# alvinliu0/HumanGaussian

Hardware: AMD Instinct MI355X
Metric: rasterize fwd+bwd Gaussians/sec @1024^2, 100k pts (higher is better)
Workload: dtype f32

## Files before the change

### humangaussian_amd/csrc/api.hip

```cpp
#include "hgs_common.h"
#include <stdio.h>
#include <stdlib.h>
#include <string.h>
#include <algorithm>
#include <atomic>
#include <mutex>

#ifdef HGS_TIMELINE
__device__ unsigned long long hgs_tl[HGS_TL_KERNELS][HGS_TL_SLOTS][4];
#endif
#include "preprocess.hip"
#include "binning.hip"
#include "render_fwd.hip"
#include "knn.hip"
#include "mesh.hip"
#include "fields.hip"
#include "bookkeeping.hip"
#include "optim.hip"
#include "lbs.hip"
#include "pose.hip"
#include "step_images.hip"

extern "C" __global__ void hgs_k_render_bwd(View, Layout, const hgs_status*, const SortRec*, const float*,
                                            const float*, const float*, const float*, const float*,
                                            const float*, const float*, float*, uint32_t);
extern "C" __global__ void hgs_k_pair_reduce_em(View, Layout, const hgs_status*, const SortRec*, const float*, float*, uint32_t, uint32_t);
extern "C" __global__ void hgs_k_pair_reduce_ch(View, Layout, const hgs_status*, const SortRec*, const float*, float*, uint32_t, uint32_t);

namespace {

#ifdef HGS_KNOBS
inline int hgs_knob(const char* name, int dflt) { const char* e = getenv(name); return (e && atoi(e) > 0) ? atoi(e) : dflt; }
#else
inline int hgs_knob(const char*, int dflt) { return dflt; }
#endif

#define HGS_CHUNK_ROWS_MIN_VIEWS 3
#ifndef HGS_PRE_BWD_VPAR_MIN_VIEWS
#define HGS_PRE_BWD_VPAR_MIN_VIEWS 2
#endif
constexpr size_t ALIGN = 256;
struct Carver {
  size_t off = 0;
  size_t take(size_t bytes) { const size_t o = off; off = hgs_align_up(off + bytes, ALIGN); return o; }
};
struct ScanShape { unsigned blocks; size_t bsum_bytes; };
inline ScanShape scan_shape(size_t n, size_t elem) {
  const size_t nb = (n + HGS_SCAN_BLOCK - 1) / HGS_SCAN_BLOCK;
  return {(unsigned)nb, (nb + 1) * elem};
}
constexpr size_t HGS_LDS_BINS_MAX = 16384;
#define HGS_BIN_WGS_PER_VIEW_MAX 512
#define HGS_BIN_WGS_TOTAL_MAX 1024
constexpr int HGS_MAX_BIN_WGS_PER_VIEW = HGS_BIN_WGS_PER_VIEW_MAX;
constexpr int HGS_BIN_WGS_TOTAL = HGS_BIN_WGS_TOTAL_MAX;

struct GeomCarve {
  size_t geom, tile_n, tile_start, tile_order, tile_rec, cell_info, items_part, fwd_cells,
      hist, tile_gbase, tile_count, chunk_sums, chunk_base, ctr, status, total;
};

inline int grid_dim(int pixels) { return (pixels + HGS_TILE - 1) / HGS_TILE; }

inline void bin_shape(int B, int P, int& nblk, int& cpw, int& nwg) {
  nblk = (P + HGS_BLOCK - 1) / HGS_BLOCK;
  int want = HGS_BIN_WGS_TOTAL / (B > 0 ? B : 1);
  if (want > HGS_MAX_BIN_WGS_PER_VIEW) want = HGS_MAX_BIN_WGS_PER_VIEW;
  if (want < 1) want = 1;
  cpw = (nblk + want - 1) / want;
  if (cpw < 1) cpw = 1;
  nwg = (nblk + cpw - 1) / cpw;
}

GeomCarve carve_geom(int B, int P, int H, int W) {
  const size_t T = (size_t)grid_dim(W) * grid_dim(H);
  const size_t TT = T * (size_t)B;
  int nblk, cpw, nwg;
  bin_shape(B, P, nblk, cpw, nwg);
  const bool lds = T <= HGS_LDS_BINS_MAX;
  GeomCarve c;
  Carver cv;
  c.geom = cv.take((size_t)B * P * sizeof(GeomRec));
  c.tile_n = cv.take(TT * 4);
  c.tile_start = cv.take(TT * 4);
  c.tile_order = cv.take(TT * 4);
  c.tile_rec = cv.take(TT * 16);
  c.cell_info = cv.take(TT * 16 * sizeof(CellInfo));
  const size_t dcap = hgs_die_cells((int)TT);
  c.items_part = cv.take(HGS_NXCD * 2 * dcap * sizeof(uint4));
  c.fwd_cells = cv.take((size_t)HGS_NXCD * HGS_NFC * dcap * 4);
  c.hist = cv.take(lds ? (size_t)B * nwg * T * 4 : 0);
  c.tile_gbase = cv.take(lds ? (size_t)HGS_ROW_GROUPS * TT * 4 : 0);
  c.tile_count = cv.take(lds ? 0 : TT * 4);
  c.chunk_sums = cv.take((size_t)B * nblk * 4);
  c.chunk_base = cv.take((size_t)B * nblk * 4);
  c.ctr = cv.take(sizeof(Counters));
  c.status = cv.take(sizeof(hgs_status));
  c.total = cv.off;
  return c;
}

struct BinCarve { size_t keys, recs, cell_list, entpair, cstate, items_full, total; };

BinCarve carve_bin(int64_t cap) {
  BinCarve c;
  Carver cv;
  const size_t C = (size_t)(cap > 0 ? cap : 0);
  const size_t NP = C * HGS_PAIRS_PER_ENTRY;
  c.keys = cv.take(C * 8);
  c.recs = cv.take(C * sizeof(SortRec));
  c.cell_list = cv.take(NP * 8);
  c.entpair = cv.take(C * 8);
  c.cstate = cv.take((NP / HGS_SEGLEN + 1) * HGS_CSTATE_FLOATS * sizeof(float));
  c.items_full = cv.take(HGS_NXCD * (NP / HGS_SEGLEN + 1) * sizeof(uint4));
  c.total = cv.off;
  return c;
}

Layout make_layout(void* geom, void* bin, void* img, int B, int P, int H, int W, int64_t cap) {
  const GeomCarve g = carve_geom(B, P, H, W);
  const BinCarve b = carve_bin(cap);
  char* gp = static_cast<char*>(geom);
  char* bp = static_cast<char*>(bin);
  Layout L;
  L.geom = reinterpret_cast<GeomRec*>(gp + g.geom);
  L.tile_n = reinterpret_cast<uint32_t*>(gp + g.tile_n);
  L.tile_start = reinterpret_cast<uint32_t*>(gp + g.tile_start);
  L.tile_order = reinterpret_cast<uint32_t*>(gp + g.tile_order);
  L.tile_rec = reinterpret_cast<uint4*>(gp + g.tile_rec);
  L.cell_info = reinterpret_cast<CellInfo*>(gp + g.cell_info);
  L.items_part = reinterpret_cast<uint4*>(gp + g.items_part);
  L.fwd_cells = reinterpret_cast<uint32_t*>(gp + g.fwd_cells);
  L.hist = reinterpret_cast<uint32_t*>(gp + g.hist);
  L.tile_gbase = reinterpret_cast<uint32_t*>(gp + g.tile_gbase);
  L.tile_count = reinterpret_cast<uint32_t*>(gp + g.tile_count);
  L.chunk_sums = reinterpret_cast<uint32_t*>(gp + g.chunk_sums);
  L.chunk_base = reinterpret_cast<uint32_t*>(gp + g.chunk_base);
  L.ctr = reinterpret_cast<Counters*>(gp + g.ctr);
  L.keys = bp ? reinterpret_cast<unsigned long long*>(bp + b.keys) : nullptr;
  L.recs = bp ? reinterpret_cast<SortRec*>(bp + b.recs) : nullptr;
  L.cell_list = bp ? reinterpret_cast<uint2*>(bp + b.cell_list) : nullptr;
  L.entpair = bp ? reinterpret_cast<uint2*>(bp + b.entpair) : nullptr;
  L.cstate = bp ? reinterpret_cast<float*>(bp + b.cstate) : nullptr;
  L.items_full = bp ? reinterpret_cast<uint4*>(bp + b.items_full) : nullptr;
  L.full_cap = (uint32_t)((size_t)(cap > 0 ? cap : 0) * HGS_PAIRS_PER_ENTRY / HGS_SEGLEN + 1);
  L.n_contrib = static_cast<uint32_t*>(img);
  return L;
}

View make_view(const hgs_settings* s, int B, int P, int M, int64_t cap, int max_tile_hint = 0, int act = 0) {
  View v;
  v.act = act;
  v.pairchunks = B >= HGS_CHUNK_ROWS_MIN_VIEWS ? 1 : 0;
  for (int b = 0; b < HGS_MAX_VIEWS; ++b) {
    const hgs_settings& sb = s[b < B ? b : 0];
    Cam& c = v.cam[b];
    c.viewmatrix = sb.viewmatrix;
    c.projmatrix = sb.projmatrix;
    c.campos = sb.campos;
    c.bg = sb.bg;
    c.tanfovx = sb.tanfovx;
    c.tanfovy = sb.tanfovy;
    c.focal_x = (float)sb.image_width / (2.0f * sb.tanfovx);
    c.focal_y = (float)sb.image_height / (2.0f * sb.tanfovy);
  }
  v.scale_modifier = s->scale_modifier;
  v.W = s->image_width;
  v.H = s->image_height;
  v.grid_x = grid_dim(v.W);
  v.grid_y = grid_dim(v.H);
  v.T = v.grid_x * v.grid_y;
  v.B = B;
  v.TT = B * v.T;
  v.P = P;
  v.M = M;
  v.D = s->sh_degree;
  v.lds_bins = (size_t)v.T <= HGS_LDS_BINS_MAX ? 1 : 0;
  bin_shape(B, P, v.nblk, v.cpw, v.nwg);
  if (!v.lds_bins) { v.cpw = 1; v.nwg = v.nblk; }
  v.entry_capacity = (uint32_t)(cap < 0 ? 0 : (cap > 0xffffffffll ? 0xffffffffll : cap));
  v.max_tile_hint = max_tile_hint;
  return v;
}

inline int hip_rc(hipError_t e) { return e == hipSuccess ? HGS_OK : -(1000 + (int)e); }

inline hipError_t box_init(void* hdr, size_t hdr_bytes, uint32_t* bmin, hipStream_t stream) {
  const hipError_t e = hipMemsetAsync(hdr, 0, hdr_bytes, stream);
  return e != hipSuccess ? e : hipMemsetAsync(bmin, 0xff, 3 * sizeof(uint32_t), stream);
}

#define HGS_LAUNCH_CHECK()                       \
  do {                                           \
    hipError_t e__ = hipGetLastError();          \
    if (e__ != hipSuccess) return hip_rc(e__);   \
  } while (0)

#define HGS_STAGE(k)                                                              \
  do {                                                                            \
    if (stage_events && stage_events[k]) {                                        \
      hipError_t e__ = hipEventRecord(static_cast<hipEvent_t>(stage_events[k]), stream); \
      if (e__ != hipSuccess) return hip_rc(e__);                                  \
    }                                                                             \
  } while (0)

struct SideStream {
  std::mutex mu;
  hipStream_t s = nullptr;
  hipEvent_t fork = nullptr, join = nullptr;
  bool tried = false, ok = false;
};

struct DeviceState {
  std::atomic<int> cus;
  SideStream side;
  std::atomic<int> lds_raised[HGS_PRE_BWD_ROWS];
};
DeviceState g_devices[64];
DeviceState* device_state(hipStream_t stream) {
  int dev = 0;
  if (hipStreamGetDevice(stream, &dev) != hipSuccess || dev < 0 || dev >= 64) { (void)hipGetLastError(); return nullptr; }
  return &g_devices[dev];
}
struct DeviceCurrent {
  int dev, cur = 0;
  bool ok, switched;
  explicit DeviceCurrent(const DeviceState* ds)
      : dev((int)(ds - g_devices)), ok(hipGetDevice(&cur) == hipSuccess), switched(ok && cur != dev) {
    if (switched) ok = hipSetDevice(dev) == hipSuccess;
  }
  ~DeviceCurrent() { if (switched) (void)hipSetDevice(cur); }
};

int cu_count(DeviceState* ds) {
  if (!ds) return 256;
  int cus = ds->cus.load(std::memory_order_relaxed);
  if (cus > 0) return cus;
  if (hipDeviceGetAttribute(&cus, hipDeviceAttributeMultiprocessorCount, (int)(ds - g_devices)) != hipSuccess || cus < 1) cus = 256;
  ds->cus.store(cus, std::memory_order_relaxed);
  return cus;
}

SideStream* side_stream(DeviceState* ds) {
  if (!ds) return nullptr;
  SideStream& t = ds->side;
  std::lock_guard<std::mutex> lk(t.mu);
  if (!t.tried) {
    t.tried = true;
    DeviceCurrent on(ds);
    t.ok = on.ok && hipStreamCreateWithFlags(&t.s, hipStreamNonBlocking) == hipSuccess &&
           hipEventCreateWithFlags(&t.fork, hipEventDisableTiming) == hipSuccess &&
           hipEventCreateWithFlags(&t.join, hipEventDisableTiming) == hipSuccess;
    if (!t.ok) (void)hipGetLastError();
  }
  return t.ok ? &t : nullptr;
}

bool pre_bwd_lds_raised(DeviceState* ds, int row) {
  if (!ds) return false;
  int st = ds->lds_raised[row].load(std::memory_order_relaxed);
  if (st == 0) {
    const PreBwdForm& form = hgs_pre_bwd_forms.row[row];
    DeviceCurrent on(ds);
    if (on.ok && hipFuncSetAttribute(reinterpret_cast<const void*>(form.kernel), hipFuncAttributeMaxDynamicSharedMemorySize, 160 * 1024) == hipSuccess) {
      st = 1;
    } else {
      (void)hipGetLastError();
      st = -1;
      fprintf(stderr, "libhgs_rast: cannot raise the dynamic LDS limit of %s on device %d: "
                      "batches that need more than 64 KB take the (slower) loop form\n", form.name, on.dev);
    }
    ds->lds_raised[row].store(st, std::memory_order_relaxed);
  }
  return st > 0;
}

bool settings_ok(const hgs_settings* s) {
  return s && s->image_height > 0 && s->image_width > 0 && s->bg && s->viewmatrix &&
         s->projmatrix && s->campos && s->sh_degree >= 0 && s->sh_degree <= 3 &&
         s->image_width <= 16 * 65535 && s->image_height <= 16 * 65535;
}

bool batch_ok(const hgs_settings* s, int B) {
  if (!s || B < 1 || B > HGS_MAX_VIEWS) return false;
  for (int b = 0; b < B; ++b) {
    if (!settings_ok(s + b)) return false;
    if (s[b].image_height != s[0].image_height || s[b].image_width != s[0].image_width ||
        s[b].sh_degree != s[0].sh_degree || s[b].scale_modifier != s[0].scale_modifier)
      return false;
  }
  return (size_t)B * grid_dim(s->image_width) * grid_dim(s->image_height) < (1u << 30);
}

}

#ifdef HGS_TIMELINE
extern "C" int hgs_debug_timeline_read(int kernel_id, void* host_dst) {
  if (kernel_id < 0 || kernel_id >= HGS_TL_KERNELS) return -1;
  const size_t bytes = sizeof(unsigned long long) * HGS_TL_SLOTS * 4, off = bytes * (size_t)kernel_id;
  if (hipDeviceSynchronize() != hipSuccess) return -2;
  if (hipMemcpyFromSymbol(host_dst, HIP_SYMBOL(hgs_tl), bytes, off, hipMemcpyDeviceToHost) != hipSuccess) return -3;
  void* p = nullptr;
  if (hipGetSymbolAddress(&p, HIP_SYMBOL(hgs_tl)) != hipSuccess) return -4;
  return hipMemset(static_cast<char*>(p) + off, 0, bytes) == hipSuccess ? 0 : -5;
}
#endif
// ... 5 lines not shown
  if (P == 0) return HGS_OK;
  if (!points || !mean_dist2) return HGS_EINVAL;
  hipStream_t stream = static_cast<hipStream_t>(stream_);
  hipLaunchKernelGGL(hgs_k_knn3, dim3((P + 255) / 256), dim3(256), 0, stream, (int)P, points, mean_dist2,
                     static_cast<const KnnGrid*>(nullptr));
  HGS_LAUNCH_CHECK();
  return HGS_OK;
}

namespace {
struct KnnCarve { size_t grid, cell_of, count, cursor, bsum, sorted, total; uint32_t nc_max; };
KnnCarve carve_knn(int32_t P) {
  KnnCarve c;
  const size_t n = (size_t)(P > 0 ? P : 0);
  const size_t want = std::max<size_t>(64, 2 * n);
  c.nc_max = (uint32_t)std::min<size_t>(want, HGS_KNN_MAX_CELLS);
  Carver cv;
  c.grid = cv.take(sizeof(KnnGrid));
  c.cell_of = cv.take(n * 4);
  c.count = cv.take(((size_t)c.nc_max + 1) * 4);
  c.cursor = cv.take((size_t)c.nc_max * 4);
  c.bsum = cv.take(scan_shape((size_t)c.nc_max + 1, 4).bsum_bytes);
  c.sorted = cv.take(n * 16);
  c.total = cv.off;
  return c;
}
}

size_t hgs_knn_scratch_bytes(int32_t P) { return carve_knn(P).total; }

int hgs_knn_mean_dist2_grid(int32_t P, const float* points, float* mean_dist2, void* scratch, void* stream_) {
  if (P < 0) return HGS_EINVAL;
  if (P == 0) return HGS_OK;
  if (!points || !mean_dist2 || !scratch) return HGS_EINVAL;
  hipStream_t stream = static_cast<hipStream_t>(stream_);
  const KnnCarve c = carve_knn(P);
  char* sp = static_cast<char*>(scratch);
  KnnGrid* G = reinterpret_cast<KnnGrid*>(sp + c.grid);
  uint32_t* cell_of = reinterpret_cast<uint32_t*>(sp + c.cell_of);
  uint32_t* count = reinterpret_cast<uint32_t*>(sp + c.count);
  uint32_t* cursor = reinterpret_cast<uint32_t*>(sp + c.cursor);
  uint32_t* bsum = reinterpret_cast<uint32_t*>(sp + c.bsum);
  float4* sorted = reinterpret_cast<float4*>(sp + c.sorted);
  hipError_t e = box_init(G, sizeof(KnnGrid), G->bmin, stream);
  if (e == hipSuccess) e = hipMemsetAsync(count, 0, ((size_t)c.nc_max + 1) * 4, stream);
  if (e != hipSuccess) return hip_rc(e);
  const unsigned gp = (unsigned)((P + 255) / 256), gc = scan_shape(c.nc_max, 4).blocks;
  hipLaunchKernelGGL(hgs_k_knn_bbox, dim3(gp), dim3(256), 0, stream, (int)P, points, G);
  hipLaunchKernelGGL(hgs_k_knn_grid_setup, dim3(1), dim3(64), 0, stream, (int)P, c.nc_max, G);
  hipLaunchKernelGGL(hgs_k_knn_count, dim3(gp), dim3(256), 0, stream, (int)P, points, (const KnnGrid*)G, cell_of, count);
  hipLaunchKernelGGL(hgs_k_knn_scan1, dim3(gc), dim3(1024), 0, stream, (const KnnGrid*)G, (const uint32_t*)count, bsum);
  hipLaunchKernelGGL(hgs_k_knn_scan2, dim3(1), dim3(1024), 0, stream, (const KnnGrid*)G, bsum);
  hipLaunchKernelGGL(hgs_k_knn_scan3, dim3(gc), dim3(1024), 0, stream, (int)P, G, count, cursor, (const uint32_t*)bsum);
  hipLaunchKernelGGL(hgs_k_knn_scatter, dim3(gp), dim3(256), 0, stream, (int)P, points, (const uint32_t*)cell_of, cursor, sorted);
  hipLaunchKernelGGL(hgs_k_knn_search, dim3(gp), dim3(256), 0, stream, (int)P, (const KnnGrid*)G, (const uint32_t*)count,
                     (const float4*)sorted, mean_dist2);
  hipLaunchKernelGGL(hgs_k_knn3, dim3(gp), dim3(256), 0, stream, (int)P, points, mean_dist2, (const KnnGrid*)G);
  HGS_LAUNCH_CHECK();
  return HGS_OK;
}

int hgs_reduce_view_packs_acc(int32_t world, int64_t P, int32_t F, const float* gathered, const float* acc_in,
                              float* out, void* stream_) {
  if (world < 1 || P < 0 || F < 1) return HGS_EINVAL;
  if (P == 0) return HGS_OK;
  if (!gathered || !out) return HGS_EINVAL;
  hipStream_t stream = static_cast<hipStream_t>(stream_);
  const long long n = (long long)P * F;
  hipLaunchKernelGGL(hgs_k_reduce_view_packs, dim3((unsigned)((n + 255) / 256)), dim3(256), 0, stream,
                     (int)world, n, (int)F, gathered, acc_in, out);
  HGS_LAUNCH_CHECK();
  return HGS_OK;
}

int hgs_reduce_view_packs_unpack(int32_t world, int64_t P, int32_t M, const float* gathered, const float* acc_in,
                                 float* g_means3D, float* g_means2D, float* g_sh, float* g_opac, float* g_scales,
                                 float* g_rot, int32_t* radii, void* stream_) {
  if (world < 1 || P < 0 || M < 0) return HGS_EINVAL;
  if (P == 0) return HGS_OK;
  if (!gathered || !g_means3D || !g_means2D || (M > 0 && !g_sh) || !g_opac || !g_scales || !g_rot || !radii) return HGS_EINVAL;
  hipStream_t stream = static_cast<hipStream_t>(stream_);
  const int F = 15 + 3 * M;
  const long long n = (long long)P * F;
  hipLaunchKernelGGL(hgs_k_reduce_view_packs_unpack, dim3((unsigned)((n + 255) / 256)), dim3(256), 0, stream,
                     (int)world, n, (int)F, (int)M, gathered, acc_in, g_means3D, g_means2D, g_sh, g_opac, g_scales, g_rot, radii);
  HGS_LAUNCH_CHECK();
  return HGS_OK;
}

int hgs_reduce_view_packs(int32_t world, int64_t P, int32_t F, const float* gathered, float* out,
                          void* stream_) {
  return hgs_reduce_view_packs_acc(world, P, F, gathered, nullptr, out, stream_);
}

int hgs_pack_view_contribution(int32_t P, int32_t M, const float* g_means3D, const float* g_means2D,
                               const float* g_sh, const float* g_opac, const float* g_scales,
                               const float* g_rot, const int32_t* radii, float* out, void* stream_) {
  if (P < 0 || M < 0) return HGS_EINVAL;
  if (P == 0) return HGS_OK;
  if (!g_means3D || !g_means2D || (M > 0 && !g_sh) || !g_opac || !g_scales || !g_rot || !radii || !out)
    return HGS_EINVAL;
  hipStream_t stream = static_cast<hipStream_t>(stream_);
  const long long n = (long long)P * (15 + 3 * M);
  hipLaunchKernelGGL(hgs_k_pack_view_contribution, dim3((unsigned)((n + 255) / 256)), dim3(256), 0, stream,
                     (int)P, (int)M, g_means3D, g_means2D, g_sh, g_opac, g_scales, g_rot, radii, out);
  HGS_LAUNCH_CHECK();
  return HGS_OK;
}

int hgs_abi_version(void) { return 17; }

size_t hgs_geom_bytes_batch(int32_t B, int32_t P, int32_t H, int32_t W) {
  if (B < 1 || B > HGS_MAX_VIEWS || P < 0 || H <= 0 || W <= 0) return 0;
  return carve_geom(B, P, H, W).total;
}
size_t hgs_geom_bytes(int32_t P, int32_t H, int32_t W) { return hgs_geom_bytes_batch(1, P, H, W); }
size_t hgs_bin_bytes(int64_t entry_capacity) { return carve_bin(entry_capacity).total; }
size_t hgs_img_bytes_batch(int32_t B, int32_t H, int32_t W) {
  if (B < 1 || B > HGS_MAX_VIEWS || H <= 0 || W <= 0) return 0;
  return hgs_align_up((size_t)B * H * W * 4, ALIGN);
}
size_t hgs_img_bytes(int32_t H, int32_t W) { return hgs_img_bytes_batch(1, H, W); }
size_t hgs_bwd_scratch_bytes(int64_t R) {
  return hgs_align_up((size_t)(R > 0 ? R : 0) * (HGS_ROW_FLOATS + HGS_PAIRS_PER_ENTRY * HGS_PROW_FLOATS) * sizeof(float), ALIGN);
}
size_t hgs_bwd_scratch_bytes_pairs(int64_t R, int64_t pairs) {
  if (R <= 0) return 0;
  if (pairs <= 0 || pairs > R * HGS_PAIRS_PER_ENTRY) return hgs_bwd_scratch_bytes(R);
  return hgs_align_up(((size_t)R * HGS_ROW_FLOATS + (size_t)pairs * HGS_PROW_FLOATS) * sizeof(float), ALIGN);
}

int hgs_forward_batch_act(const hgs_settings* s, int32_t B, int32_t P, int32_t M, const float* means3D,
                          const float* shs, const float* colors_precomp, const float* opacities,
                          const float* scales, const float* rotations, const float* cov3D_precomp,
                          float* out_color, float* out_depth, float* out_alpha, int32_t* radii,
                          void* geom, void* bin, int64_t entry_capacity, void* img,
                          int32_t store_bwd_state, int32_t max_tile_entries_hint, hgs_status* status_host,
                          int32_t status_host_mapped, void* status_event, void* const* stage_events,
                          int32_t activation_flags, void* stream_) {
  return hgs_forward_batch_act_leaf(s, B, P, M, means3D, shs, colors_precomp, opacities, scales, rotations, cov3D_precomp,
                                    out_color, out_depth, out_alpha, radii, geom, bin, entry_capacity, img, store_bwd_state,
                                    max_tile_entries_hint, status_host, status_host_mapped, status_event, stage_events,
                                    activation_flags, nullptr, stream_);
}

int hgs_forward_batch_act_leaf(const hgs_settings* s, int32_t B, int32_t P, int32_t M, const float* means3D,
                               const float* shs, const float* colors_precomp, const float* opacities,
                               const float* scales, const float* rotations, const float* cov3D_precomp,
                               float* out_color, float* out_depth, float* out_alpha, int32_t* radii,
                               void* geom, void* bin, int64_t entry_capacity, void* img,
                               int32_t store_bwd_state, int32_t max_tile_entries_hint, hgs_status* status_host,
                               int32_t status_host_mapped, void* status_event, void* const* stage_events,
                               int32_t activation_flags, float* means2D_leaf, void* stream_) {
  if (activation_flags & ~(7 | HGS_GRAD_SCALE_TRUE_DERIVATIVE | HGS_ANTIALIAS)) return HGS_EINVAL;
  if (!batch_ok(s, B) || P < 0 || !out_color || !out_depth || !out_alpha || !geom || !img ||
      entry_capacity < 0)
    return HGS_EINVAL;
  if (P > 0) {
    if (!means3D || !opacities || !radii) return HGS_EINVAL;
    if ((shs != nullptr) == (colors_precomp != nullptr)) return HGS_ESHAPE;
    const bool has_sr = scales != nullptr && rotations != nullptr;
    if ((scales != nullptr) != (rotations != nullptr)) return HGS_ESHAPE;
    if (has_sr == (cov3D_precomp != nullptr)) return HGS_ESHAPE;
    if (shs && M < (s->sh_degree + 1) * (s->sh_degree + 1)) return HGS_ESHAPE;
    if (entry_capacity > 0 && !bin) return HGS_EINVAL;
    if ((int64_t)B * P >= (1ll << 31) || P >= (1 << 28)) return HGS_EINVAL;
  }
  if (entry_capacity > HGS_MAX_ENTRY_CAPACITY) return HGS_EINVAL;
  hipStream_t stream = static_cast<hipStream_t>(stream_);
  DeviceState* const ds = device_state(stream);
  const int ncu = cu_count(ds);
  const bool aa = (activation_flags & HGS_ANTIALIAS) != 0;
  const View v = make_view(s, B, P, M, entry_capacity, max_tile_entries_hint > 0 ? max_tile_entries_hint : 0,
                           activation_flags & 7);
  const Layout L = make_layout(geom, bin, img, B, P, v.H, v.W, entry_capacity);
  hgs_status* status_dev =
      reinterpret_cast<hgs_status*>(static_cast<char*>(geom) + carve_geom(B, P, v.H, v.W).status);

  HGS_STAGE(0);
  hipError_t e = hipSuccess;
  if (v.nblk == 0) {
    e = hipMemsetAsync(L.ctr, 0, sizeof(Counters), stream);
    if (e != hipSuccess) return hip_rc(e);
  }
  const size_t lds_bytes = (size_t)v.T * 4;
  if (!v.lds_bins) {
    e = hipMemsetAsync(L.tile_count, 0, (size_t)v.TT * 4, stream);
    if (e != hipSuccess) return hip_rc(e);
  }
  if (v.nblk > 0) {
    if (v.lds_bins)
      hipLaunchKernelGGL(aa ? hgs_k_preprocess_fwd_aa : hgs_k_preprocess_fwd, dim3(v.B * v.nwg), dim3(HGS_BLOCK), lds_bytes,
                         stream, v, L, means3D, shs, colors_precomp, opacities, scales, rotations,
                         cov3D_precomp, radii, means2D_leaf);
    else
      hipLaunchKernelGGL(aa ? hgs_k_preprocess_fwd_ga_aa : hgs_k_preprocess_fwd_ga, dim3(v.B * v.nblk), dim3(HGS_BLOCK), 0,
                         stream, v, L, means3D, shs, colors_precomp, opacities, scales, rotations,
                         cov3D_precomp, radii, means2D_leaf);
    HGS_LAUNCH_CHECK();
  }
  HGS_STAGE(1);
  const unsigned bpv = (unsigned)((v.T + HGS_TILES_PER_WG - 1) / HGS_TILES_PER_WG);
  hipLaunchKernelGGL(hgs_k_tiles, dim3(bpv * (unsigned)v.B), dim3(64 * HGS_ROW_GROUPS), 0, stream, v, L);
  HGS_LAUNCH_CHECK();
  HGS_STAGE(2);
  const unsigned order_wgs = (unsigned)((v.TT + HGS_BLOCK - 1) / HGS_BLOCK);
  hgs_status* status_mapped = status_host_mapped ? status_host : nullptr;
  const unsigned nbin = entry_capacity > 0 ? (unsigned)(v.B * (v.lds_bins ? v.nwg : v.nblk)) : 0u;
  if (v.lds_bins && nbin)
    hipLaunchKernelGGL(hgs_k_fill, dim3(nbin + order_wgs), dim3(HGS_BLOCK), lds_bytes, stream, v, L, status_dev,
                       status_mapped, (int)nbin);
  else
    hipLaunchKernelGGL(hgs_k_fill_ga, dim3(nbin + order_wgs), dim3(HGS_BLOCK), 0, stream, v, L, status_dev,
                       status_mapped, (int)nbin);
  HGS_LAUNCH_CHECK();
  if (status_host && !status_host_mapped) {
    e = hipMemcpyAsync(status_host, status_dev, sizeof(hgs_status), hipMemcpyDeviceToHost, stream);
    if (e != hipSuccess) return hip_rc(e);
  }
  if (status_event) {
    e = hipEventRecord(static_cast<hipEvent_t>(status_event), stream);
    if (e != hipSuccess) return hip_rc(e);
  }
  if (entry_capacity > 0) {
    HGS_STAGE(3);
    auto class_grid = [&](int64_t lo) {
      const int64_t g = entry_capacity / lo + 1;
      return (unsigned)(g < v.TT ? g : v.TT);
    };
    const int hint = v.max_tile_hint;
    const bool need_huge = hint <= 0 || hint > 16384, need_large = hint <= 0 || hint > HGS_SORT_LDS_MAX;
    const bool expect_long = hint <= 0 || hint > HGS_SORT_LDS_MAX + HGS_SORT_LDS_MAX / 2 + 64;
    SideStream* side = ((need_huge || need_large) && expect_long) ? side_stream(ds) : nullptr;
    {
      std::unique_lock<std::mutex> side_lk;
      hipStream_t s2 = stream;
      if (side) {
        side_lk = std::unique_lock<std::mutex>(side->mu);
        e = hipEventRecord(side->fork, stream);
        if (e == hipSuccess) e = hipStreamWaitEvent(side->s, side->fork, 0);
        if (e != hipSuccess) return hip_rc(e);
        s2 = side->s;
      }
      if (need_huge) {
        hipLaunchKernelGGL(hgs_k_sort_huge, dim3(class_grid(16384)), dim3(1024), 0, s2, v, L, status_dev);
        HGS_LAUNCH_CHECK();
      }
      if (need_large) {
        hipLaunchKernelGGL(hgs_k_sort_large, dim3(class_grid(HGS_SORT_LDS_MAX)), dim3(1024), 0, s2, v, L, status_dev);
        HGS_LAUNCH_CHECK();
      }
      if (side) {
        e = hipEventRecord(side->join, side->s);
        if (e != hipSuccess) return hip_rc(e);
      }
      const unsigned sort_wgs = std::min<unsigned>(class_grid(1), (unsigned)(hgs_knob("HGS_SORT_WGS_PER_CU", 3) * ncu));
      hipLaunchKernelGGL(v.pairchunks ? hgs_k_sort_lds_ch : hgs_k_sort_lds, dim3(sort_wgs), dim3(HGS_SORT_NT), 0, stream, v, L,
                         status_dev);
      HGS_LAUNCH_CHECK();
      if (side) {
        e = hipStreamWaitEvent(stream, side->join, 0);
        if (e != hipSuccess) return hip_rc(e);
      }
    }
  } else {
    HGS_STAGE(3);
  }
  HGS_STAGE(4);
  {
    const int64_t cells = std::min<int64_t>((int64_t)16 * v.TT, (int64_t)HGS_PAIRS_PER_ENTRY * entry_capacity);
    const int64_t fwd_blocks = (int64_t)hgs_knob("HGS_FWD_BLOCKS_PER_CU", 4) * ncu;
    const unsigned cell_blocks = (unsigned)std::max<int64_t>(4, std::min<int64_t>(fwd_blocks, (cells + 3) / 4) & ~int64_t(3));
    const unsigned bg_blocks = (unsigned)v.TT;
    hipLaunchKernelGGL(store_bwd_state ? hgs_k_render_fwd_store : hgs_k_render_fwd_nostore, dim3(cell_blocks + bg_blocks),
                       dim3(HGS_FWD_THREADS), 0, stream, v, L, cell_blocks, status_dev, status_mapped, L.recs, L.cstate,
                       out_color, out_depth, out_alpha);
  }
  HGS_LAUNCH_CHECK();
  HGS_STAGE(5);
  return HGS_OK;
}

int hgs_forward_batch(const hgs_settings* s, int32_t B, int32_t P, int32_t M, const float* means3D,
                      const float* shs, const float* colors_precomp, const float* opacities,
                      const float* scales, const float* rotations, const float* cov3D_precomp,
                      float* out_color, float* out_depth, float* out_alpha, int32_t* radii,
                      void* geom, void* bin, int64_t entry_capacity, void* img,
                      int32_t store_bwd_state, int32_t max_tile_entries_hint, hgs_status* status_host,
                      int32_t status_host_mapped, void* status_event, void* const* stage_events,
                      void* stream_) {
  return hgs_forward_batch_act(s, B, P, M, means3D, shs, colors_precomp, opacities, scales, rotations, cov3D_precomp,
                               out_color, out_depth, out_alpha, radii, geom, bin, entry_capacity, img, store_bwd_state,
                               max_tile_entries_hint, status_host, status_host_mapped, status_event, stage_events, 0,
                               stream_);
}

int hgs_forward(const hgs_settings* s, int32_t P, int32_t M, const float* means3D,
                const float* shs, const float* colors_precomp, const float* opacities,
                const float* scales, const float* rotations, const float* cov3D_precomp,
                float* out_color, float* out_depth, float* out_alpha, int32_t* radii,
                void* geom, void* bin, int64_t entry_capacity, void* img,
                int32_t store_bwd_state, int32_t max_tile_entries_hint, hgs_status* status_host,
                int32_t status_host_mapped, void* status_event, void* const* stage_events,
                void* stream_) {
  return hgs_forward_batch(s, 1, P, M, means3D, shs, colors_precomp, opacities, scales, rotations,
                           cov3D_precomp, out_color, out_depth, out_alpha, radii, geom, bin, entry_capacity,
                           img, store_bwd_state, max_tile_entries_hint, status_host, status_host_mapped,
                           status_event, stage_events, stream_);
}

}

namespace {
int backward_impl(const hgs_settings* s, int32_t B, int32_t P, int32_t M, const float* means3D,
                           const float* shs, const float* colors_precomp, const float* opacities,
                           const float* scales, const float* rotations, const float* cov3D_precomp,
                           const int32_t* radii, const float* out_color, const float* out_depth,
                           const float* out_alpha, const float* dL_dout_color,
                           const float* dL_dout_depth, const float* dL_dout_alpha, const void* geom,
                           const void* bin, const void* img, const hgs_status* status,
                           int64_t entry_capacity, void* bwd_scratch, float* dL_dmeans3D, float* dL_dmeans2D, float* dL_dshs,
                           float* dL_dcolors_precomp, float* dL_dopacities, float* dL_dscales,
                           float* dL_drotations, float* dL_dcov3D_precomp, void* const* stage_events,
                           int32_t activation_flags, float* pack, int32_t pack_F, void* stream_) {
  (void)radii;
  if (activation_flags & ~(7 | HGS_GRAD_SCALE_TRUE_DERIVATIVE | HGS_ANTIALIAS)) return HGS_EINVAL;
  if ((activation_flags & (HGS_ACT_OPACITY_SIGMOID | HGS_ANTIALIAS)) && P > 0 && !opacities) return HGS_EINVAL;
  if (!batch_ok(s, B) || P < 0 || !geom || !img || entry_capacity < 0 || entry_capacity > HGS_MAX_ENTRY_CAPACITY) return HGS_EINVAL;
  if (status && status->overflow) return HGS_EINVAL;
  if (status && (int64_t)status->reserved[0] != entry_capacity) return HGS_EINVAL;
  if (P == 0) return HGS_OK;
  if (!means3D || !out_color || !out_depth || !out_alpha) return HGS_EINVAL;
  if ((shs != nullptr) == (colors_precomp != nullptr)) return HGS_ESHAPE;
  if ((scales != nullptr) != (rotations != nullptr)) return HGS_ESHAPE;
  if ((scales != nullptr) == (cov3D_precomp != nullptr)) return HGS_ESHAPE;
  if (shs && !dL_dshs) return HGS_EINVAL;
  const bool maybe_entries = status ? status->num_rendered > 0 : entry_capacity > 0;
  if (maybe_entries && (!bin || !bwd_scratch)) return HGS_EINVAL;
  hipStream_t stream = static_cast<hipStream_t>(stream_);
  DeviceState* const ds = device_state(stream);
  const int64_t cap = entry_capacity;
  const View v = make_view(s, B, P, M, cap, 0, activation_flags);
  const Layout L = make_layout(const_cast<void*>(geom), const_cast<void*>(bin),
                               const_cast<void*>(img), B, P, v.H, v.W, cap);
  const hgs_status* status_dev = reinterpret_cast<const hgs_status*>(
      static_cast<const char*>(geom) + carve_geom(B, P, v.H, v.W).status);
  const int64_t X = status ? (int64_t)status->num_rendered : cap;
  const int64_t worst = X * HGS_PAIRS_PER_ENTRY;
  const int64_t pc = (status && status->num_pairs > 0 && (int64_t)status->num_pairs < worst) ? (int64_t)status->num_pairs : worst;
  const uint32_t pair_cap = (uint32_t)(pc > 0xffffffffll ? 0xffffffffll : pc);
  float* rows = static_cast<float*>(bwd_scratch);
  float* pair_rows = rows + (size_t)X * HGS_ROW_FLOATS;
  HGS_STAGE(0);
  if (maybe_entries) {
    const int resident = hgs_knob("HGS_BWD_WAVES_PER_CU", 12) * cu_count(ds);
    hipLaunchKernelGGL(hgs_k_render_bwd, dim3((unsigned)std::max(HGS_NXCD, resident / HGS_BWD_BLOCK_WAVES / HGS_NXCD * HGS_NXCD)), dim3(64 * HGS_BWD_BLOCK_WAVES), 0, stream, v, L, status_dev, L.recs, L.cstate,
                       out_color, out_depth, out_alpha, dL_dout_color, dL_dout_depth, dL_dout_alpha, pair_rows, pair_cap);
    HGS_LAUNCH_CHECK();
    HGS_STAGE(1);
    if (X > 0) {
      const uint32_t R_host = status ? status->num_rendered : 0xffffffffu;
      hipLaunchKernelGGL(v.pairchunks ? hgs_k_pair_reduce_ch : hgs_k_pair_reduce_em, dim3((unsigned)((X + 255) / 256)), dim3(256), 0,
                         stream, v, L, status_dev, L.recs, pair_rows, rows, pair_cap, R_host);
      HGS_LAUNCH_CHECK();
    }
  }
  if (!maybe_entries) HGS_STAGE(1);
  HGS_STAGE(2);
  const int deg = shs ? v.D : 0;
  const int nc = (deg + 1) * (deg + 1);
  const int aa = (activation_flags & HGS_ANTIALIAS) ? 1 : 0;
  const unsigned thr_p = 64u * (unsigned)v.B;
  const size_t lds_p = (size_t)(23 + 3 * nc) * thr_p * sizeof(float);
  const int row_p = hgs_pre_bwd_row(aa, 2, deg);
  const bool vpar_ok = v.B >= HGS_PRE_BWD_VPAR_MIN_VIEWS && thr_p <= (unsigned)hgs_pre_bwd_forms.row[row_p].threads &&
                       (lds_p <= 65536 || pre_bwd_lds_raised(ds, row_p));
  const int mode = v.B == 1 ? 1 : (vpar_ok ? 2 : 0);
  const PreBwdForm& form = hgs_pre_bwd_forms.row[hgs_pre_bwd_row(aa, mode, deg)];
  const unsigned grid = mode == 2 ? (unsigned)((v.P + 63) / 64) : (unsigned)v.nblk, threads = mode == 2 ? thr_p : HGS_BLOCK;
  const size_t lds = mode == 2 ? lds_p : (mode == 1 ? hgs_pre_bwd_stage_bytes(M, deg, shs != nullptr && dL_dshs != nullptr) : 0);
  hipLaunchKernelGGL(form.kernel, dim3(grid), dim3(threads), lds, stream, v, L, status_dev, rows, means3D, shs,
                     colors_precomp, opacities, scales, rotations, cov3D_precomp, dL_dmeans3D, dL_dmeans2D,
                     dL_dshs, dL_dcolors_precomp, dL_dopacities, dL_dscales, dL_drotations,
                     dL_dcov3D_precomp, pack, (int)pack_F);
  HGS_LAUNCH_CHECK();
  HGS_STAGE(3);
  return HGS_OK;
}
}

extern "C" {

int hgs_backward_batch_act(const hgs_settings* s, int32_t B, int32_t P, int32_t M, const float* means3D,
                           const float* shs, const float* colors_precomp, const float* opacities,
                           const float* scales, const float* rotations, const float* cov3D_precomp,
                           const int32_t* radii, const float* out_color, const float* out_depth,
                           const float* out_alpha, const float* dL_dout_color,
                           const float* dL_dout_depth, const float* dL_dout_alpha, const void* geom,
                           const void* bin, const void* img, const hgs_status* status,
                           int64_t entry_capacity, void* bwd_scratch, float* dL_dmeans3D, float* dL_dmeans2D, float* dL_dshs,
                           float* dL_dcolors_precomp, float* dL_dopacities, float* dL_dscales,
                           float* dL_drotations, float* dL_dcov3D_precomp, void* const* stage_events,
                           int32_t activation_flags, void* stream_) {
  return backward_impl(s, B, P, M, means3D, shs, colors_precomp, opacities, scales, rotations, cov3D_precomp, radii, out_color,
                       out_depth, out_alpha, dL_dout_color, dL_dout_depth, dL_dout_alpha, geom, bin, img, status,
                       entry_capacity, bwd_scratch, dL_dmeans3D, dL_dmeans2D, dL_dshs, dL_dcolors_precomp, dL_dopacities,
                       dL_dscales, dL_drotations, dL_dcov3D_precomp, stage_events, activation_flags, nullptr, 0, stream_);
}

int hgs_backward_batch_packed(const hgs_settings* s, int32_t B, int32_t P, int32_t M, const float* means3D,
                              const float* shs, const float* opacities, const float* scales, const float* rotations,
                              const int32_t* radii, const float* out_color, const float* out_depth, const float* out_alpha,
                              const float* dL_dout_color, const float* dL_dout_depth, const float* dL_dout_alpha,
                              const void* geom, const void* bin, const void* img, const hgs_status* status,
                              int64_t entry_capacity, void* bwd_scratch, float* pack, float* dL_dmeans2D_views,
                              void* const* stage_events, int32_t activation_flags, void* stream_) {
  if (!pack || !shs || !scales || !rotations || M < 1) return P == 0 ? HGS_OK : HGS_EINVAL;
  float* marker = pack;
  return backward_impl(s, B, P, M, means3D, shs, nullptr, opacities, scales, rotations, nullptr, radii, out_color, out_depth,
                       out_alpha, dL_dout_color, dL_dout_depth, dL_dout_alpha, geom, bin, img, status, entry_capacity,
                       bwd_scratch, marker, dL_dmeans2D_views, marker, nullptr, marker, marker, marker, nullptr, stage_events,
                       activation_flags, pack, 15 + 3 * M, stream_);
}

int hgs_backward_batch(const hgs_settings* s, int32_t B, int32_t P, int32_t M, const float* means3D,
                       const float* shs, const float* colors_precomp, const float* opacities,
                       const float* scales, const float* rotations, const float* cov3D_precomp,
                       const int32_t* radii, const float* out_color, const float* out_depth,
                       const float* out_alpha, const float* dL_dout_color,
                       const float* dL_dout_depth, const float* dL_dout_alpha, const void* geom,
                       const void* bin, const void* img, const hgs_status* status,
                       int64_t entry_capacity, void* bwd_scratch, float* dL_dmeans3D, float* dL_dmeans2D, float* dL_dshs,
                       float* dL_dcolors_precomp, float* dL_dopacities, float* dL_dscales,
                       float* dL_drotations, float* dL_dcov3D_precomp, void* const* stage_events,
                       void* stream_) {
  return hgs_backward_batch_act(s, B, P, M, means3D, shs, colors_precomp, opacities, scales, rotations, cov3D_precomp,
                                radii, out_color, out_depth, out_alpha, dL_dout_color, dL_dout_depth, dL_dout_alpha,
                                geom, bin, img, status, entry_capacity, bwd_scratch, dL_dmeans3D, dL_dmeans2D, dL_dshs,
                                dL_dcolors_precomp, dL_dopacities, dL_dscales, dL_drotations, dL_dcov3D_precomp,
                                stage_events, 0, stream_);
}

int hgs_backward(const hgs_settings* s, int32_t P, int32_t M, const float* means3D,
                 const float* shs, const float* colors_precomp, const float* opacities,
                 const float* scales, const float* rotations, const float* cov3D_precomp,
                 const int32_t* radii, const float* out_color, const float* out_depth,
                 const float* out_alpha, const float* dL_dout_color,
                 const float* dL_dout_depth, const float* dL_dout_alpha, const void* geom,
                 const void* bin, const void* img, const hgs_status* status,
                 int64_t entry_capacity, void* bwd_scratch, float* dL_dmeans3D, float* dL_dmeans2D, float* dL_dshs,
                 float* dL_dcolors_precomp, float* dL_dopacities, float* dL_dscales,
                 float* dL_drotations, float* dL_dcov3D_precomp, void* const* stage_events,
                 void* stream_) {
  return hgs_backward_batch(s, 1, P, M, means3D, shs, colors_precomp, opacities, scales, rotations,
                            cov3D_precomp, radii, out_color, out_depth, out_alpha, dL_dout_color,
                            dL_dout_depth, dL_dout_alpha, geom, bin, img, status, entry_capacity, bwd_scratch,
                            dL_dmeans3D, dL_dmeans2D, dL_dshs, dL_dcolors_precomp, dL_dopacities, dL_dscales,
                            dL_drotations, dL_dcov3D_precomp, stage_events, stream_);
}

int hgs_densify_stats(int32_t B, int32_t P, const float* dL_dmeans2D, const int32_t* radii, const uint8_t* keep,
                      float* xyz_gradient_accum, float* denom, float* max_radii2D, int32_t* radii_max,
                      uint8_t* visibility, void* stream_) {
  if (B < 1 || P < 0) return HGS_EINVAL;
  if (P == 0) return HGS_OK;
  if (!dL_dmeans2D || !radii || !xyz_gradient_accum || !denom || !max_radii2D) return HGS_EINVAL;
  hipStream_t stream = static_cast<hipStream_t>(stream_);
  hipLaunchKernelGGL(hgs_k_densify_stats, dim3((P + 255) / 256), dim3(256), 0, stream, (int)B, (int)P, dL_dmeans2D,
                     radii, keep, xyz_gradient_accum, denom, max_radii2D, radii_max, visibility);
  HGS_LAUNCH_CHECK();
  return HGS_OK;
}

int hgs_densify_masks(int32_t P, const float* xyz_gradient_accum, const float* denom, const float* scales,
                      int32_t scales_are_log, const float* opacity, int32_t opacity_is_logit,
                      const float* max_radii2D, float grad_threshold, float percent_dense, float extent,
                      float min_opacity, float max_screen_size, float size_thresh, uint8_t* clone_mask,
                      uint8_t* split_mask, uint8_t* prune_mask, uint32_t* counts, void* stream_) {
  if (P < 0) return HGS_EINVAL;
  hipStream_t stream = static_cast<hipStream_t>(stream_);
  if (counts) {
    hipError_t e = hipMemsetAsync(counts, 0, 3 * sizeof(uint32_t), stream);
    if (e != hipSuccess) return hip_rc(e);
  }
  if (P == 0) return HGS_OK;
  if (!xyz_gradient_accum || !denom || !scales || !opacity || (max_screen_size > 0.0f && !max_radii2D)) return HGS_EINVAL;
  hipLaunchKernelGGL(hgs_k_densify_masks, dim3((P + 255) / 256), dim3(256), 0, stream, (int)P, xyz_gradient_accum, denom,
                     scales, (int)scales_are_log, opacity, (int)opacity_is_logit, max_radii2D, grad_threshold,
                     percent_dense, extent, min_opacity, max_screen_size, size_thresh, clone_mask, split_mask, prune_mask,
                     counts);
  HGS_LAUNCH_CHECK();
  return HGS_OK;
}

size_t hgs_compact_scratch_bytes(int32_t P) {
  return hgs_align_up(scan_shape((size_t)(P > 0 ? P : 0), 4).bsum_bytes, ALIGN);
}

int hgs_compact_index(int32_t P, const uint8_t* keep, int32_t* src_of_dst, uint32_t* num_kept, void* scratch,
                      void* stream_) {
  if (P < 0 || !num_kept) return HGS_EINVAL;
  hipStream_t stream = static_cast<hipStream_t>(stream_);
  if (P == 0) {
    hipError_t e = hipMemsetAsync(num_kept, 0, 4, stream);
    return e == hipSuccess ? HGS_OK : hip_rc(e);
  }
  if (!keep || !src_of_dst || !scratch) return HGS_EINVAL;
  const int nb = (int)scan_shape((size_t)P, 4).blocks;
  uint32_t* blocks = static_cast<uint32_t*>(scratch);
  hipLaunchKernelGGL(hgs_k_keep_count, dim3(nb), dim3(1024), 0, stream, (int)P, keep, blocks);
  hipLaunchKernelGGL(hgs_k_keep_scan, dim3(1), dim3(1024), 0, stream, nb, blocks, num_kept);
  hipLaunchKernelGGL(hgs_k_keep_index, dim3(nb), dim3(1024), 0, stream, (int)P, keep, blocks, src_of_dst);
  HGS_LAUNCH_CHECK();
  return HGS_OK;
}

int hgs_gather_rows(int64_t n_out, int32_t row_floats, const int32_t* src_of_dst, const float* src, float* dst,
                    void* stream_) {
  if (n_out < 0 || row_floats < 1) return HGS_EINVAL;
  if (n_out == 0) return HGS_OK;
  if (!src_of_dst || !src || !dst) return HGS_EINVAL;
  hipStream_t stream = static_cast<hipStream_t>(stream_);
  const long long n = (long long)n_out * row_floats;
  hipLaunchKernelGGL(hgs_k_gather_rows, dim3((unsigned)((n + 255) / 256)), dim3(256), 0, stream, n, (int)row_floats,
                     src_of_dst, src, dst);
  HGS_LAUNCH_CHECK();
  return HGS_OK;
}

int hgs_reanchor(int32_t P, const float* vertices, const int32_t* faces, const int32_t* mapping_face,
                 const float* mapping_uvw, const float* mapping_dist, float* xyz, void* stream_) {
  if (P < 0) return HGS_EINVAL;
  if (P == 0) return HGS_OK;
  if (!vertices || !faces || !mapping_face || !mapping_uvw || !mapping_dist || !xyz) return HGS_EINVAL;
// ... 457 lines not shown
```

### humangaussian_amd/csrc/binning.hip

```cpp
#include "hgs_common.h"

extern "C" __global__ void __launch_bounds__(64 * HGS_ROW_GROUPS)
hgs_k_tiles(View v, Layout L) {
  __shared__ uint32_t gt[HGS_ROW_GROUPS][HGS_TILES_PER_WG];
  __shared__ uint32_t start_s[HGS_TILES_PER_WG];
  __shared__ uint32_t cls_s[HGS_NCLS];
  const int tid = threadIdx.x, tl = tid & 63;
  const int rg = __builtin_amdgcn_readfirstlane(tid >> 6);
  const int bpv = (v.T + HGS_TILES_PER_WG - 1) / HGS_TILES_PER_WG;
  const int b = (int)blockIdx.x / bpv;
  const int t = ((int)blockIdx.x % bpv) * HGS_TILES_PER_WG + tl;
  const bool valid = t < v.T;
  const size_t g = (size_t)b * v.T + t;
  if (tid < HGS_NCLS) cls_s[tid] = 0;
  uint32_t run = 0;
  if (v.lds_bins) {
    const int rpg = (v.nwg + HGS_ROW_GROUPS - 1) / HGS_ROW_GROUPS;
    const int r0 = rg * rpg, r1 = min(v.nwg, r0 + rpg);
    if (valid) {
      uint32_t* col = L.hist + (size_t)b * v.nwg * v.T + t;
      constexpr int BR = 16;
      for (int r = r0; r < r1; r += BR) {
        uint32_t c[BR];
#pragma unroll
        for (int k = 0; k < BR; ++k) c[k] = (r + k < r1) ? col[(size_t)(r + k) * v.T] : 0u;
#pragma unroll
        for (int k = 0; k < BR; ++k) {
          if (r + k < r1 && c[k]) col[(size_t)(r + k) * v.T] = run;
          run += c[k];
        }
      }
    }
  } else if (rg == 0 && valid) {
    run = L.tile_count[g];
    L.tile_count[g] = 0;
  }
  gt[rg][tl] = run;
  __syncthreads();
  uint32_t gbase = 0;
#pragma unroll
  for (int k = 0; k < HGS_ROW_GROUPS; ++k) gbase += (k < rg) ? gt[k][tl] : 0u;
  if (rg == 0) {
    uint32_t n = 0;
#pragma unroll
    for (int k = 0; k < HGS_ROW_GROUPS; ++k) n += gt[k][tl];
    if (!valid) n = 0;
    const uint32_t i0 = hgs_wave_incl_scan(n);
    unsigned long long b_eb = 0;
    if (tl == 63 && i0) b_eb = atomicAdd(&L.ctr->alloc_eb, (unsigned long long)i0);
    const uint32_t s0 = (uint32_t)__builtin_amdgcn_readlane((int)(uint32_t)b_eb, 63);
    const uint32_t start = s0 + i0 - n;
    start_s[tl] = start;
    if (valid) {
      L.tile_n[g] = n;
      L.tile_start[g] = start;
    }
    const unsigned long long eb = __ballot(valid && n == 0);
    if (tl == 0 && eb) atomicAdd(&cls_s[0], (uint32_t)__popcll(eb));
    if (valid && n) atomicAdd(&cls_s[32 - __clz(n)], 1u);
    const uint32_t mx = hgs_wave_max_u32(n);
    if (tl == 0 && mx) atomicMax(&L.ctr->max_n, mx);
  }
  __syncthreads();
  if (v.lds_bins && valid) L.tile_gbase[(size_t)rg * v.TT + g] = start_s[tl] + gbase;
  if (tid < HGS_NCLS && cls_s[tid]) atomicAdd(&L.ctr->cls_hist[tid].v, cls_s[tid]);

}

__device__ __forceinline__ uint32_t overflow_from_counters(const View& v, const Layout& L) {
  const uint32_t R = (uint32_t)L.ctr->alloc_eb;
  uint32_t o = (R > v.entry_capacity) ? 1u : 0u;
  if (v.max_tile_hint > 0 && L.ctr->max_n > (uint32_t)v.max_tile_hint) o |= 2u;
  return o;
}

__device__ __forceinline__ void place_tiles(const View& v, const Layout& L, int blk, int nblks,
                                            hgs_status* __restrict__ status,
                                            hgs_status* __restrict__ status_host) {
  __shared__ uint32_t cls_base[HGS_NCLS];
  __shared__ uint32_t cls_cnt[HGS_NCLS];
  const int tid = threadIdx.x, lane = tid & 63;
  if (tid < HGS_NCLS) cls_cnt[tid] = L.ctr->cls_hist[tid].v;
  __syncthreads();
  if (tid == 0) {
    uint32_t acc = 0;
    for (int c = HGS_NCLS - 1; c >= 0; --c) { cls_base[c] = acc; acc += cls_cnt[c]; }
  }
  if (blk == 0 && tid == 64) {
    const unsigned long long a_eb = L.ctr->alloc_eb;
    hgs_status st;
    st.num_rendered = (uint32_t)a_eb;
    st.active_tiles = (uint32_t)v.TT - cls_cnt[0];
    st.num_pairs = 0;
    st.bwd_groups = 0;
    st.overflow = overflow_from_counters(v, L);
    st.reserved[0] = v.entry_capacity;
    st.reserved[1] = L.ctr->max_n;
    st.reserved[2] = 1;
    *status = st;
    if (status_host) {
      volatile uint32_t* hs = reinterpret_cast<volatile uint32_t*>(status_host);
      const uint32_t* sw = reinterpret_cast<const uint32_t*>(&st);
      for (int k = 0; k < 7; ++k) hs[k] = sw[k];
      __threadfence_system();
      hs[7] = 1u;
      __threadfence_system();
    }
  }
  if (tid >= 128 && tid < 192) {
    const int nchunk = v.B * v.nblk;
    const int per_wg = (nchunk + nblks - 1) / nblks;
    const int c_begin = blk * per_wg, c_end = min(nchunk, c_begin + per_wg);
    for (int c0 = c_begin; c0 < c_end; c0 += 64) {
      const int c = c0 + lane;
      const uint32_t sum = (c < c_end) ? L.chunk_sums[c] : 0u;
      const uint32_t inc = hgs_wave_incl_scan(sum);
      uint32_t base = 0;
      if (lane == 63 && inc) base = atomicAdd(&L.ctr->entry_alloc, inc);
      base = (uint32_t)__builtin_amdgcn_readlane((int)base, 63);
      if (c < c_end) L.chunk_base[c] = base + inc - sum;
    }
  }
  __syncthreads();
  const int g = blk * HGS_BLOCK + tid;
  const bool valid = g < v.TT;
  const uint32_t n = valid ? L.tile_n[g] : 0u;
  const int c = (valid && n) ? 32 - __clz(n) : 0;
  int leader_of = 0;
  uint32_t rank = 0, cnt = 0;
  unsigned long long todo = __ballot(valid);
  while (todo) {
    const int leader = (int)__builtin_ctzll(todo);
    const int cl = __builtin_amdgcn_readlane(c, leader);
    const unsigned long long same = __ballot(valid && c == cl);
    if (valid && c == cl) {
      leader_of = leader;
      rank = __builtin_amdgcn_mbcnt_hi((uint32_t)(same >> 32), __builtin_amdgcn_mbcnt_lo((uint32_t)same, 0u));
      cnt = (uint32_t)__popcll(same);
    }
    todo &= ~same;
  }
  uint32_t base = 0;
  if (valid && lane == leader_of) base = atomicAdd(&L.ctr->cls_cur[c].v, cnt);
  base = (uint32_t)__shfl((int)base, leader_of, 64);
  const uint32_t pos = cls_base[c] + base + rank;
  if (!valid) return;
  L.tile_order[pos] = (uint32_t)g;
  L.tile_rec[pos] = make_uint4((uint32_t)g, n, L.tile_start[g], 0u);
}

extern "C" __global__ void __launch_bounds__(HGS_BLOCK)
hgs_k_fill(View v, Layout L, hgs_status* __restrict__ status, hgs_status* __restrict__ status_host, int nbin) {
  extern __shared__ __attribute__((aligned(16))) uint32_t lds_cur[];
  if ((int)blockIdx.x >= nbin) {
    place_tiles(v, L, (int)blockIdx.x - nbin, (int)gridDim.x - nbin, status, status_host);
    return;
  }
  if (overflow_from_counters(v, L)) return;
  const int b = (int)blockIdx.x / v.nwg, lw = (int)blockIdx.x % v.nwg;
  const uint32_t* __restrict__ base_row = L.hist + (size_t)blockIdx.x * v.T;
  const int rpg = (v.nwg + HGS_ROW_GROUPS - 1) / HGS_ROW_GROUPS;
  const uint32_t* __restrict__ grp_row = L.tile_gbase + (size_t)(lw / rpg) * v.TT + (size_t)b * v.T;
  for (int t = threadIdx.x; t < v.T; t += HGS_BLOCK) lds_cur[t] = grp_row[t] + base_row[t];
  __syncthreads();
  const GeomRec* __restrict__ geom = L.geom + (size_t)b * v.P;
  for (int c = 0; c < v.cpw; ++c) {
    const int chunk = lw * v.cpw + c;
    if (chunk >= v.nblk) break;
    const int i = chunk * HGS_BLOCK + threadIdx.x;
    if (i >= v.P) continue;
    const uint4 q2 = reinterpret_cast<const uint4*>(&geom[i])[2];
    const uint32_t depth_bits = q2.y, lo = q2.z, hi = q2.w;
    const int minx = lo & 0xffffu, miny = lo >> 16, maxx = hi & 0xffffu, maxy = hi >> 16;
    const unsigned long long key_hi = (unsigned long long)depth_bits << 32;
    for (int ty = miny; ty < maxy; ++ty)
      for (int tx = minx; tx < maxx; ++tx) {
        const uint32_t slot = atomicAdd(&lds_cur[ty * v.grid_x + tx], 1u);
        L.keys[slot] = key_hi | (uint32_t)i;
      }
  }
}

extern "C" __global__ void __launch_bounds__(HGS_BLOCK)
hgs_k_fill_ga(View v, Layout L, hgs_status* __restrict__ status, hgs_status* __restrict__ status_host, int nbin) {
  if ((int)blockIdx.x >= nbin) {
    place_tiles(v, L, (int)blockIdx.x - nbin, (int)gridDim.x - nbin, status, status_host);
    return;
  }
  if (overflow_from_counters(v, L)) return;
  const int b = (int)blockIdx.x / v.nblk, chunk = (int)blockIdx.x % v.nblk;
  const int i = chunk * HGS_BLOCK + threadIdx.x;
  if (i >= v.P) return;
  const uint4 q2 = reinterpret_cast<const uint4*>(&L.geom[(size_t)b * v.P + i])[2];
  const uint32_t depth_bits = q2.y, lo = q2.z, hi = q2.w;
  const int minx = lo & 0xffffu, miny = lo >> 16, maxx = hi & 0xffffu, maxy = hi >> 16;
  const unsigned long long key_hi = (unsigned long long)depth_bits << 32;
  for (int ty = miny; ty < maxy; ++ty)
    for (int tx = minx; tx < maxx; ++tx) {
      const size_t g = (size_t)b * v.T + ty * v.grid_x + tx;
      const uint32_t slot = L.tile_start[g] + atomicAdd(&L.tile_count[g], 1u);
      L.keys[slot] = key_hi | (uint32_t)i;
    }
}

namespace {

#define HGS_EMIT_RECORD(MASK, G0, G1, G2, OFFSET, CHUNK_BASE, K, TAGGED, CHUNK_ROWS)                                     \
  {                                                                                                                      \
    const uint4 g0 = (G0), g1 = (G1), g2 = (G2);                                                                         \
    const int minx = g2.z & 0xffffu, miny = g2.z >> 16, maxx = g2.w & 0xffffu;                                           \
    const uint32_t entry = (CHUNK_BASE) + (OFFSET) + (uint32_t)((ty - miny) * (maxx - minx) + (tx - minx));              \
    const float mx = __uint_as_float(g0.x), my = __uint_as_float(g0.y);                                                  \
    const float ca = __uint_as_float(g0.z), cb = __uint_as_float(g0.w), cc = __uint_as_float(g1.x);                      \
    MASK = hgs_cell_mask(mx, my, ca, cb, cc, __uint_as_float(g1.y), x0, y0);                                             \
    uint4* dst = reinterpret_cast<uint4*>(&L.recs[start + (K)]);                                                         \
    const float qa = -0.5f * ca * HGS_LOG2E, qb = -cb * HGS_LOG2E, qc = -0.5f * cc * HGS_LOG2E;                          \
    dst[0] = make_uint4(g0.x, g0.y, __float_as_uint(qa), __float_as_uint(qb));                                           \
    dst[1] = make_uint4(__float_as_uint(qc), g1.y, g1.z, g1.w);                                                          \
    dst[2] = make_uint4(g2.x, g2.y, entry, (TAGGED) ? hgs_rec_tag(MASK, (K), n, (CHUNK_ROWS)) : 0u);                     \
    L.entpair[start + (K)].x = hgs_entpair_x(entry, (uint32_t)__popc(MASK));                                             \
  }

struct CellAlloc {
  uint32_t len, nfull, rem, nst, i_len, i_st, i_full, pcls, fcls, frank, die;
  unsigned long long b1, b2, b3, got;
};

__device__ __forceinline__ void hgs_alloc_cell_ranges_issue(const Layout& L, uint32_t order_pos, uint32_t len_of_lane, CellAlloc& a) {
  const int lane = (int)threadIdx.x & 63;
  a.die = order_pos % HGS_NXCD;
  const bool cl = lane < 16;
  a.len = cl ? len_of_lane : 0u;
  a.nfull = a.len / HGS_SEGLEN; a.rem = a.len % HGS_SEGLEN;
  const uint32_t nseg = a.nfull + (a.rem ? 1u : 0u);
  a.nst = nseg ? nseg - 1u : 0u;
  a.i_len = hgs_wave_incl_scan(a.len); a.i_st = hgs_wave_incl_scan(a.nst); a.i_full = hgs_wave_incl_scan(a.nfull);
  a.pcls = a.rem ? hgs_item_class(a.rem) : 0u;
  a.b1 = __ballot(a.pcls == 1u); a.b2 = __ballot(a.pcls == 2u); a.b3 = __ballot(a.pcls == 3u);
  const uint32_t t_len = (uint32_t)__builtin_amdgcn_readlane((int)a.i_len, 63);
  const uint32_t t_st = (uint32_t)__builtin_amdgcn_readlane((int)a.i_st, 63);
  const uint32_t t_full = (uint32_t)__builtin_amdgcn_readlane((int)a.i_full, 63);
  a.fcls = hgs_cell_class(a.len);
  unsigned long long fb_ = 0;
  a.frank = 0;
#pragma unroll
  for (int c = 0; c < HGS_NFC; ++c) {
    const unsigned long long bc = __ballot(cl && a.len && a.fcls == (uint32_t)c);
    if (lane == 3 + c) fb_ = bc;
    if (a.fcls == (uint32_t)c) a.frank = (uint32_t)__popcll(bc & ((1ull << lane) - 1ull));
  }
  const unsigned long long add = lane == 0 ? ((unsigned long long)t_len | ((unsigned long long)t_st << 32))
                               : lane == 1 ? ((unsigned long long)t_full | ((unsigned long long)__popcll(a.b1) << 32))
                               : lane == 2 ? ((unsigned long long)__popcll(a.b2) | ((unsigned long long)__popcll(a.b3) << 32))
                                           : (unsigned long long)__popcll(fb_);
  a.got = 0;
  unsigned long long* ctr = lane == 0 ? &L.ctr->alloc_ps : &L.ctr->sched[a.die][min(lane, 2 + HGS_NFC) - 1];
  if (lane < 3 + HGS_NFC && add) a.got = atomicAdd(ctr, add);
}

__device__ __forceinline__ void hgs_alloc_cell_ranges_finish(const View& v, const Layout& L, int g, const CellAlloc& a,
                                                             uint32_t* cell_base, uint32_t& pair_base_out) {
  int lane = (int)threadIdx.x & 63;
  asm volatile("" : "+v"(lane));
  const bool cl = lane < 16;
  const uint32_t fpos = (uint32_t)__shfl((int)(uint32_t)a.got, 3 + (int)a.fcls, 64) + a.frank;
  const uint32_t got_lo = (uint32_t)a.got, got_hi = (uint32_t)(a.got >> 32);
  const uint32_t pb = (uint32_t)__builtin_amdgcn_readlane((int)got_lo, 0);
  const uint32_t sb = (uint32_t)__builtin_amdgcn_readlane((int)got_hi, 0);
  const uint32_t fb = (uint32_t)__builtin_amdgcn_readlane((int)got_lo, 1);
  const uint32_t p1 = (uint32_t)__builtin_amdgcn_readlane((int)got_hi, 1);
  const uint32_t p2 = (uint32_t)__builtin_amdgcn_readlane((int)got_lo, 2);
  const uint32_t p3 = (uint32_t)__builtin_amdgcn_readlane((int)got_hi, 2);
  if (cl) {
    const uint32_t len = a.len, nfull = a.nfull, rem = a.rem;
    const uint32_t base = pb + a.i_len - len;
    cell_base[lane] = base;
    CellInfo ci;
    ci.base = base; ci.len = len; ci.sbase = sb + a.i_st - a.nst; ci.pbase = pb;
    L.cell_info[(size_t)g * 16 + lane] = ci;
    const uint32_t key = hgs_cell_key((uint32_t)g, (uint32_t)lane);
    const size_t dcap = hgs_die_cells(v.TT);
    if (len) L.fwd_cells[((size_t)a.die * HGS_NFC + a.fcls) * dcap + fpos] = key;
    uint4* full = L.items_full + ((size_t)a.die * L.full_cap + fb + a.i_full - nfull);
    for (uint32_t sgm = 0; sgm < nfull; ++sgm)
      full[sgm] = make_uint4(key, HGS_SEGLEN, base + sgm * HGS_SEGLEN, sgm ? ci.sbase + sgm - 1u : 0xffffffffu);
    if (rem) {
      const unsigned long long below = (1ull << lane) - 1ull;
      uint4* part = L.items_part + (size_t)a.die * 2 * dcap;
      const uint4 it = make_uint4(key, rem, base + nfull * HGS_SEGLEN, nfull ? ci.sbase + nfull - 1u : 0xffffffffu);
      if (a.pcls == 1u) part[p1 + (uint32_t)__popcll(a.b1 & below)] = it;
      else if (a.pcls == 2u) part[dcap - 1 - (p2 + (uint32_t)__popcll(a.b2 & below))] = it;
      else part[dcap + p3 + (uint32_t)__popcll(a.b3 & below)] = it;
    }
  }
  if (lane == 0) pair_base_out = pb;
}

__device__ __forceinline__ void hgs_alloc_cell_ranges(const View& v, const Layout& L, int g, uint32_t order_pos, const uint32_t* cell_tot,
                                                      uint32_t* cell_base, uint32_t& pair_base_out) {
  if (threadIdx.x < 64) {
    CellAlloc a;
    hgs_alloc_cell_ranges_issue(L, order_pos, (threadIdx.x & 63) < 16 ? cell_tot[threadIdx.x & 63] : 0u, a);
    hgs_alloc_cell_ranges_finish(v, L, g, a, cell_base, pair_base_out);
  }
}

template <int MAXCH>
struct GatherLds {
  uint32_t tab[MAXCH][17];
  uint32_t run[17];
  uint32_t cell_tot[16];
  uint32_t cell_base[16];
  uint32_t pair_base;
};

template <int MAXCH>
__device__ __forceinline__ void gather_records(const View& v, const Layout& L, int g, uint32_t order_pos,
                                               uint32_t start, uint32_t n,
                                               unsigned long long* sorted, int nt, GatherLds<MAXCH>& S) {
  const int t = g % v.T;
  const GeomRec* __restrict__ geom = L.geom + (size_t)(g / v.T) * v.P;
  const uint32_t* __restrict__ cbase = L.chunk_base + (size_t)(g / v.T) * v.nblk;
  const int tx = t % v.grid_x, ty = t / v.grid_x;
  const float x0 = (float)(tx * HGS_TILE), y0 = (float)(ty * HGS_TILE);
  const int tid = (int)threadIdx.x, lane = tid & 63;
  const int wv = tid >> 6, nwaves = nt >> 6;
  if (tid < 16) S.cell_tot[tid] = 0;
  if (tid < 17) S.run[tid] = 0;
  __syncthreads();
  constexpr int GU = 4;
  uint32_t mytot = 0;
  for (uint32_t kb0 = 0; kb0 < n; kb0 += (uint32_t)nt * GU) {
    const uint32_t kb = kb0 + threadIdx.x;
    uint32_t idxv[GU];
    uint4 q0[GU], q1[GU], q2[GU];
    uint32_t q3[GU];
#pragma unroll
    for (int u = 0; u < GU; ++u) {
      const uint32_t k = kb + (uint32_t)u * nt;
      idxv[u] = (k < n) ? (uint32_t)sorted[k] : 0u;
    }
#pragma unroll
    for (int u = 0; u < GU; ++u) {
      const uint32_t k = kb + (uint32_t)u * nt;
      if (k < n) {
        const uint4* gp = reinterpret_cast<const uint4*>(&geom[idxv[u]]);
        q0[u] = gp[0]; q1[u] = gp[1]; q2[u] = gp[2]; q3[u] = gp[3].x;
      }
    }
#pragma unroll
    for (int u = 0; u < GU; ++u) {
      const uint32_t k = kb + (uint32_t)u * nt;
      uint32_t mask = 0;
      if (k < n) {
        HGS_EMIT_RECORD(mask, q0[u], q1[u], q2[u], q3[u], cbase[idxv[u] >> 8], k, v.pairchunks, false)
        sorted[k] = (unsigned long long)mask;
      }
#pragma unroll
      for (int c = 0; c < 16; ++c) {
        const unsigned long long bal = __ballot((mask >> c) & 1u);
        if (lane == c) mytot += (uint32_t)__popcll(bal);
      }
    }
  }
  if (lane < 16 && mytot) atomicAdd(&S.cell_tot[lane], mytot);
  __syncthreads();
  hgs_alloc_cell_ranges(v, L, g, order_pos, S.cell_tot, S.cell_base, S.pair_base);
  __syncthreads();
  const uint32_t pair_base = S.pair_base;
  for (uint32_t sc0 = 0; sc0 < n; sc0 += (uint32_t)MAXCH * 64u) {
    const uint32_t nch = min((uint32_t)MAXCH, (n - sc0 + 63u) / 64u);
    for (uint32_t ch = wv; ch < nch; ch += nwaves) {
      const uint32_t k = sc0 + ch * 64u + lane;
      const uint32_t mask = (k < n) ? (uint32_t)sorted[k] : 0u;
      uint32_t mine = 0;
#pragma unroll
      for (int c = 0; c < 16; ++c) {
        const unsigned long long bal = __ballot((mask >> c) & 1u);
        if (lane == c) mine = (uint32_t)__popcll(bal);
      }
      uint32_t tot = mine;
      tot += __builtin_amdgcn_update_dpp(0, (int)tot, HGS_DPP_ROW_SHR(1), 0xf, 0xf, false);
      tot += __builtin_amdgcn_update_dpp(0, (int)tot, HGS_DPP_ROW_SHR(2), 0xf, 0xf, false);
      tot += __builtin_amdgcn_update_dpp(0, (int)tot, HGS_DPP_ROW_SHR(4), 0xf, 0xf, false);
      tot += __builtin_amdgcn_update_dpp(0, (int)tot, HGS_DPP_ROW_SHR(8), 0xf, 0xf, false);
      if (lane < 16) S.tab[ch][lane] = mine;
      if (lane == 15) S.tab[ch][16] = tot;
    }
    __syncthreads();
    for (int col = wv; col < 17; col += nwaves) {
      uint32_t carry = S.run[col];
      for (uint32_t c0 = 0; c0 < nch; c0 += 64u) {
        const uint32_t ch = c0 + lane;
        const uint32_t x = ch < nch ? S.tab[ch][col] : 0u;
        const uint32_t inc = hgs_wave_incl_scan(x);
        if (ch < nch) S.tab[ch][col] = carry + inc - x;
        carry += (uint32_t)__builtin_amdgcn_readlane((int)inc, 63);
      }
      if (lane == 0) S.run[col] = carry;
    }
    __syncthreads();
    for (uint32_t ch = wv; ch < nch; ch += nwaves) {
      const uint32_t k = sc0 + ch * 64u + lane;
      const bool in = k < n;
      const uint32_t mask = in ? (uint32_t)sorted[k] : 0u;
      const uint32_t cnt = (uint32_t)__popc(mask);
      const uint32_t rel = S.tab[ch][16] + hgs_wave_incl_scan(cnt) - cnt;
      if (in) L.entpair[start + k].y = pair_base + rel;
#pragma unroll
      for (int c = 0; c < 16; ++c) {
        const bool bit = (mask >> c) & 1u;
        const unsigned long long bal = __ballot(bit);
        if (bit) {
          const uint32_t rank = S.tab[ch][c] + __builtin_amdgcn_mbcnt_hi((uint32_t)(bal >> 32), __builtin_amdgcn_mbcnt_lo((uint32_t)bal, 0u));
          const uint32_t slot = S.cell_base[c] + rank;
          L.cell_list[slot] = make_uint2(start + k, pair_base + rel + (uint32_t)__popc(mask & ((1u << c) - 1u)));
        }
      }
    }
    __syncthreads();
  }
}

__device__ __forceinline__ uint32_t hgs_spread4(uint32_t nib) {
  return (nib * 0x00204081u) & 0x01010101u;
}
__device__ __forceinline__ uint32_t hgs_bytesum(uint32_t w) { return __builtin_amdgcn_sad_u8(w, 0u, 0u); }

template <int MAXCH>
__device__ __forceinline__ void gather_records_single(const View& v, const Layout& L, int g, uint32_t order_pos,
                                                      uint32_t start, uint32_t n,
                                                      unsigned long long* sorted, int nt, GatherLds<MAXCH>& S) {
  const int t = g % v.T;
  const GeomRec* __restrict__ geom = L.geom + (size_t)(g / v.T) * v.P;
  const uint32_t* __restrict__ cbase = L.chunk_base + (size_t)(g / v.T) * v.nblk;
  const int tx = t % v.grid_x, ty = t / v.grid_x;
  const float x0 = (float)(tx * HGS_TILE), y0 = (float)(ty * HGS_TILE);
  const int tid = (int)threadIdx.x, lane = tid & 63;
  const int wv = tid >> 6, nwaves = nt >> 6;
  const uint32_t nch = (n + 63u) / 64u;
#ifdef HGS_TIMELINE
  const unsigned long long tg0 = wall_clock64();
#define HGS_TG(i) const unsigned long long tg##i = wall_clock64()
#else
#define HGS_TG(i)
#endif
  constexpr int GU = 2;
  for (uint32_t kb0 = 0; kb0 < n; kb0 += (uint32_t)nt * GU) {
    const uint32_t kb = kb0 + threadIdx.x;
    uint32_t idxv[GU];
    uint4 q0[GU], q1[GU], q2[GU];
    uint32_t q3[GU];
#pragma unroll
    for (int u = 0; u < GU; ++u) {
      const uint32_t k = kb + (uint32_t)u * nt;
      idxv[u] = (k < n) ? (uint32_t)sorted[k] : 0u;
    }
#pragma unroll
    for (int u = 0; u < GU; ++u) {
      const uint32_t k = kb + (uint32_t)u * nt;
      if (k < n) {
        const uint4* gp = reinterpret_cast<const uint4*>(&geom[idxv[u]]);
        q0[u] = gp[0]; q1[u] = gp[1]; q2[u] = gp[2]; q3[u] = gp[3].x;
      }
    }
#pragma unroll
    for (int u = 0; u < GU; ++u) {
      const uint32_t k = kb + (uint32_t)u * nt;
      if (kb0 + (uint32_t)u * nt + (uint32_t)(wv * 64) >= n) continue;
      uint32_t mask = 0;
      if (k < n) {
        HGS_EMIT_RECORD(mask, q0[u], q1[u], q2[u], q3[u], cbase[idxv[u] >> 8], k, v.pairchunks, false)
        sorted[k] = (unsigned long long)mask;
      }
      const uint32_t ch = k >> 6;
      uint32_t tot[4];
#pragma unroll
      for (int wd = 0; wd < 4; ++wd) tot[wd] = hgs_wave_incl_scan(hgs_spread4((mask >> (4 * wd)) & 0xfu));
      if (lane == 63) {
        S.tab[ch][0] = tot[0]; S.tab[ch][1] = tot[1]; S.tab[ch][2] = tot[2]; S.tab[ch][3] = tot[3];
        S.tab[ch][16] = hgs_bytesum(tot[0]) + hgs_bytesum(tot[1]) + hgs_bytesum(tot[2]) + hgs_bytesum(tot[3]);
      }
    }
  }
  __syncthreads();
  HGS_TG(1);
  {
    uint32_t pk[(MAXCH + 63) / 64][4];
#pragma unroll
    for (int r = 0; r < (MAXCH + 63) / 64; ++r) {
      const uint32_t ch = (uint32_t)r * 64u + lane;
#pragma unroll
      for (int wd = 0; wd < 4; ++wd) pk[r][wd] = (wv < 5 && ch < nch) ? S.tab[ch][wd] : 0u;
    }
    __syncthreads();
    for (int col = wv; col < 5; col += nwaves) {
      uint32_t carry[4] = {0u, 0u, 0u, 0u};
#pragma unroll
      for (int r = 0; r < (MAXCH + 63) / 64; ++r) {
        const uint32_t ch = (uint32_t)r * 64u + lane;
        if ((uint32_t)r * 64u >= nch) break;
        if (col < 4) {
#pragma unroll
          for (int b = 0; b < 4; ++b) {
            const uint32_t x = (pk[r][col] >> (8 * b)) & 0xffu;
            const uint32_t inc = hgs_wave_incl_scan(x);
            if (ch < nch) S.tab[ch][4 * col + b] = carry[b] + inc - x;
            carry[b] += (uint32_t)__builtin_amdgcn_readlane((int)inc, 63);
          }
        } else {
          const uint32_t x = ch < nch ? S.tab[ch][16] : 0u;
          const uint32_t inc = hgs_wave_incl_scan(x);
          if (ch < nch) S.tab[ch][16] = carry[0] + inc - x;
          carry[0] += (uint32_t)__builtin_amdgcn_readlane((int)inc, 63);
        }
      }
      if (col < 4 && lane < 4) S.cell_tot[4 * col + lane] = lane == 0 ? carry[0] : lane == 1 ? carry[1] : lane == 2 ? carry[2] : carry[3];
    }
  }
  __syncthreads();
  HGS_TG(2);
  hgs_alloc_cell_ranges(v, L, g, order_pos, S.cell_tot, S.cell_base, S.pair_base);
  __syncthreads();
  HGS_TG(3);
  const uint32_t pair_base = S.pair_base;
  for (uint32_t ch = wv; ch < nch; ch += nwaves) {
    const uint32_t k = ch * 64u + lane;
    const bool in = k < n;
    uint32_t mask = in ? (uint32_t)sorted[k] : 0u;
    uint32_t ex[4], before = 0;
#pragma unroll
    for (int wd = 0; wd < 4; ++wd) {
      const uint32_t mine = hgs_spread4((mask >> (4 * wd)) & 0xfu);
      ex[wd] = hgs_wave_incl_scan(mine) - mine;
      before += hgs_bytesum(ex[wd]);
    }
    const uint32_t rel = S.tab[ch][16] + before;
    if (in) L.entpair[start + k].y = pair_base + rel;
    uint32_t r = 0;
    while (mask) {
      const int c = __builtin_ctz(mask);
      mask &= mask - 1u;
      const uint32_t exw = (c < 8) ? (c < 4 ? ex[0] : ex[1]) : (c < 12 ? ex[2] : ex[3]);
      const uint32_t slot = S.cell_base[c] + S.tab[ch][c] + ((exw >> (8 * (c & 3))) & 0xffu);
      L.cell_list[slot] = make_uint2(start + k, pair_base + rel + r);
      ++r;
    }
  }
#ifdef HGS_TIMELINE
  if (threadIdx.x == 0 && blockIdx.x < HGS_TL_SLOTS) {
    const unsigned long long tg4 = wall_clock64();
    auto cl = [](unsigned long long d) { return d > 0xffffull ? 0xffffull : d; };
    hgs_tl[2][blockIdx.x][0] = cl(tg1 - tg0) | (cl(tg2 - tg1) << 16) | (cl(tg3 - tg2) << 32) | (cl(tg4 - tg3) << 48);
  }
#endif
}

template <int NT>
__device__ __forceinline__ void bitonic_sort(unsigned long long* keys, uint32_t n) {
  uint32_t npad = 2;
  while (npad < n) npad <<= 1;
  const uint32_t half = npad >> 1;
  for (uint32_t kk = 2; kk <= npad; kk <<= 1) {
    const uint32_t hk = kk >> 1;
    for (uint32_t i = threadIdx.x; i < half; i += NT) {
      const uint32_t blk = i / hk, off = i - blk * hk;
      const uint32_t lo = blk * kk + off, hi = blk * kk + (kk - 1 - off);
      if (hi < n) {
        const unsigned long long a = keys[lo], c = keys[hi];
        if (a > c) { keys[lo] = c; keys[hi] = a; }
      }
    }
    __syncthreads();
    for (uint32_t j = kk >> 2; j > 0; j >>= 1) {
      for (uint32_t i = threadIdx.x; i < half; i += NT) {
        const uint32_t lo = ((i & ~(j - 1)) << 1) | (i & (j - 1));
        const uint32_t hi = lo | j;
        if (hi < n) {
          const unsigned long long a = keys[lo], c = keys[hi];
          if (a > c) { keys[lo] = c; keys[hi] = a; }
        }
      }
      __syncthreads();
    }
  }
}

typedef unsigned long long u64;

}

#define HGS_SORT_LIGHT 16
#define HGS_RANK_BUCKET_MAX 192
#define HGS_RANK_NB_MAX 2048
#define HGS_SORT_NT 256
#define HGS_SORT_WAVES_PER_EU 3
#define HGS_RANK_GU 2

namespace {

#ifdef HGS_TIMELINE
__shared__ unsigned long long hgs_s_tq[8];
#define HGS_TQ(i) { if (threadIdx.x == 0) hgs_s_tq[(i)] = wall_clock64(); }
#else
#define HGS_TQ(i) {}
#endif

__device__ __forceinline__ void lds_barrier() { asm volatile("s_waitcnt lgkmcnt(0)\n\ts_barrier" ::: "memory"); }

struct __attribute__((aligned(16))) RankLds {
  uint32_t hist[HGS_RANK_NB_MAX + 1];
  uint32_t wtot[16];
  uint32_t tot16[8];
  uint32_t dmin, dmax, maxcnt, pad;
};
static_assert(sizeof(uint32_t) * (HGS_RANK_NB_MAX + 1) >= sizeof(uint16_t) * 4096, "the masks of the longest list fit into the histogram");

template <int NT>
__device__ __forceinline__ void bucket_scan(RankLds& R, uint32_t NB) {
  int tid = (int)threadIdx.x;
  asm volatile("" : "+v"(tid));
  const int lane = tid & 63, wv = tid >> 6;
  const uint32_t PER = NB / (uint32_t)NT;
  uint32_t* __restrict__ h = R.hist + (uint32_t)tid * PER;
  uint32_t c[8];
  auto load_counts = [&]() {
#pragma unroll
    for (int i = 0; i < 8; ++i) c[i] = 0u;
    if (PER == 8u) {
      const uint4 a = *reinterpret_cast<const uint4*>(h), b = *reinterpret_cast<const uint4*>(h + 4);
      c[0] = a.x; c[1] = a.y; c[2] = a.z; c[3] = a.w; c[4] = b.x; c[5] = b.y; c[6] = b.z; c[7] = b.w;
    } else if (PER == 4u) {
      const uint4 a = *reinterpret_cast<const uint4*>(h);
      c[0] = a.x; c[1] = a.y; c[2] = a.z; c[3] = a.w;
    } else if (PER == 2u) {
      const uint2 a = *reinterpret_cast<const uint2*>(h);
      c[0] = a.x; c[1] = a.y;
    } else {
      c[0] = h[0];
    }
  };
  load_counts();
  uint32_t sum = 0, mx = 0;
#pragma unroll
  for (int i = 0; i < 8; ++i) { sum += c[i]; mx = max(mx, c[i]); }
  const uint32_t inc = hgs_wave_incl_scan(sum);
  mx = hgs_wave_max_u32(mx);
  if (lane == 63) R.wtot[wv] = inc;
  if (lane == 0 && mx) atomicMax(&R.maxcnt, mx);
  uint32_t base = inc - sum;
  asm volatile("" : "+v"(base));
  lds_barrier();
  load_counts();
#pragma unroll
  for (int w = 0; w < NT / 64; ++w) base += (w < wv) ? R.wtot[w] : 0u;
  uint32_t e[8];
#pragma unroll
  for (int i = 0; i < 8; ++i) { e[i] = base; base += c[i]; }
  if (PER == 8u) {
    *reinterpret_cast<uint4*>(h) = make_uint4(e[0], e[1], e[2], e[3]);
    *reinterpret_cast<uint4*>(h + 4) = make_uint4(e[4], e[5], e[6], e[7]);
  } else if (PER == 4u) {
    *reinterpret_cast<uint4*>(h) = make_uint4(e[0], e[1], e[2], e[3]);
  } else if (PER == 2u) {
    *reinterpret_cast<uint2*>(h) = make_uint2(e[0], e[1]);
  } else {
    h[0] = e[0];
  }
}

template <int NT, bool CH>
__device__ __forceinline__ void cell_lists_from_masks(const View& v, const Layout& L, uint32_t order_pos, uint32_t start, uint32_t n,
                                                      const uint16_t* __restrict__ masks, GatherLds<64>& S, const CellAlloc& ca,
                                                      unsigned long long* tp) {
  const int tid = (int)threadIdx.x, lane = tid & 63, wv = tid >> 6;
  constexpr int nwaves = NT / 64;
  const uint32_t nch = (n + 63u) / 64u;
  for (uint32_t ch = wv; ch < nch; ch += nwaves) {
    const uint32_t k = ch * 64u + lane;
    const uint32_t mask = (k < n) ? (uint32_t)masks[k] : 0u;
    uint32_t tot[4];
#pragma unroll
    for (int wd = 0; wd < 4; ++wd) tot[wd] = hgs_wave_incl_scan(hgs_spread4((mask >> (4 * wd)) & 0xfu));
    if (lane == 63) {
      S.tab[ch][0] = tot[0]; S.tab[ch][1] = tot[1]; S.tab[ch][2] = tot[2]; S.tab[ch][3] = tot[3];
      S.tab[ch][16] = hgs_bytesum(tot[0]) + hgs_bytesum(tot[1]) + hgs_bytesum(tot[2]) + hgs_bytesum(tot[3]);
    }
  }
  lds_barrier();
  {
    uint32_t pk[4];
    const uint32_t ch = (uint32_t)lane;
#pragma unroll
    for (int wd = 0; wd < 4; ++wd) pk[wd] = (ch < nch) ? S.tab[ch][wd] : 0u;
    lds_barrier();
    for (int col = wv; col < 5; col += nwaves) {
      if (col < 4) {
        const uint32_t word = col == 0 ? pk[0] : col == 1 ? pk[1] : col == 2 ? pk[2] : pk[3];
#pragma unroll
        for (int b = 0; b < 4; ++b) {
          const uint32_t x = (word >> (8 * b)) & 0xffu;
          const uint32_t inc = hgs_wave_incl_scan(x);
          if (ch < nch) S.tab[ch][4 * col + b] = inc - x;
        }
      } else {
        const uint32_t x = ch < nch ? S.tab[ch][16] : 0u;
        const uint32_t inc = hgs_wave_incl_scan(x);
        if (ch < nch) S.tab[ch][16] = inc - x;
      }
    }
  }
#ifdef HGS_TIMELINE
  tp[2] = wall_clock64();
#endif
  if (tid < 64) hgs_alloc_cell_ranges_finish(v, L, (int)L.tile_rec[order_pos].x, ca, S.cell_base, S.pair_base);
  lds_barrier();
#ifdef HGS_TIMELINE
  tp[3] = wall_clock64();
#endif
  const uint32_t pair_base = S.pair_base;
  for (uint32_t ch = wv; ch < nch; ch += nwaves) {
    const uint32_t k = ch * 64u + lane;
    const bool in = k < n;
    const uint32_t mask = in ? (uint32_t)masks[k] : 0u;
    uint32_t ex[4], before = 0;
    uint32_t tot[4];
#pragma unroll
    for (int wd = 0; wd < 4; ++wd) {
      const uint32_t mine = hgs_spread4((mask >> (4 * wd)) & 0xfu);
      const uint32_t inc = hgs_wave_incl_scan(mine);
      ex[wd] = inc - mine;
      if (CH) tot[wd] = (uint32_t)__builtin_amdgcn_readlane((int)inc, 63);
      before += hgs_bytesum(ex[wd]);
    }
    const uint32_t rel_chunk = pair_base + S.tab[ch][16];
    const uint32_t rel = rel_chunk + before;
    if (in) L.entpair[start + k].y = CH ? rel_chunk : rel;
    const uint32_t cb = lane < 16 ? S.cell_base[lane] + S.tab[ch][lane] : 0u;
    uint32_t cp = 0;
#pragma unroll
    for (int c = 0; c < 16; ++c) {
      const uint32_t cbase = (uint32_t)__builtin_amdgcn_readlane((int)cb, c);
      if ((mask >> c) & 1u) {
        const uint32_t exc = (ex[c >> 2] >> (8 * (c & 3))) & 0xffu;
        const uint32_t slot = cbase + exc;
        L.cell_list[slot] = make_uint2(start + k, CH ? rel_chunk + cp + exc : rel + (uint32_t)__popc(mask & ((1u << c) - 1u)));
      }
      if (CH) cp += (tot[c >> 2] >> (8 * (c & 3))) & 0xffu;
    }
  }
}

template <int E, int NT>
__device__ __forceinline__ bool rank_keys(const Layout& L, uint32_t start, uint32_t n, uint32_t NB, const u64 (&keyp)[HGS_RANK_GU],
                                          unsigned long long* pairs, RankLds& R) {
  int tid = (int)threadIdx.x;
  asm volatile("" : "+v"(tid));
  const int lane = tid & 63, wv = tid >> 6;
  u64 key[E];
#pragma unroll
  for (int e = 0; e < E; ++e) {
    if (e < HGS_RANK_GU) key[e] = keyp[e];
    else {
      const uint32_t k = (uint32_t)e * NT + (uint32_t)tid;
      const u64 kv = L.keys[start + min(k, n - 1u)];
      key[e] = (k < n) ? kv : ~0ull;
    }
  }
  {
    uint32_t lo = 0xffffffffu, hi = 0u;
#pragma unroll
    for (int e = 0; e < E; ++e) {
      const uint32_t d = (uint32_t)(key[e] >> 32);
      lo = min(lo, d);
      hi = max(hi, key[e] != ~0ull ? d : 0u);
    }
    hi = hgs_wave_max_u32(hi);
    lo = ~hgs_wave_max_u32(~lo);
    lds_barrier();
    if (lane == 0) { atomicMin(&R.dmin, lo); atomicMax(&R.dmax, hi); }
  }
  lds_barrier();
  HGS_TQ(0)
  const float flo = __uint_as_float(R.dmin);
  const float range = __uint_as_float(R.dmax) - flo;
  const float scale = range > 1e-30f ? (float)NB / range : 0.0f;
  uint32_t bp[E];
#pragma unroll
  for (int e = 0; e < E; ++e) {
    bp[e] = 0u;
    if (key[e] != ~0ull) {
      const float x = (__uint_as_float((uint32_t)(key[e] >> 32)) - flo) * scale;
      const uint32_t bkt = (uint32_t)fminf(x, (float)(NB - 1u));
      bp[e] = bkt | (atomicAdd(&R.hist[bkt], 1u) << 12);
    }
  }
  lds_barrier();
  HGS_TQ(1)
  bucket_scan<NT>(R, NB);
  if (tid == 0) R.hist[NB] = n;
  lds_barrier();
  HGS_TQ(2)
  const bool degenerate = R.maxcnt > (uint32_t)HGS_RANK_BUCKET_MAX;
  if (!degenerate) {
    constexpr int EG = E < 8 ? E : 8;
    uint32_t lmax[E / EG];
#pragma unroll
    for (int h = 0; h < E / EG; ++h) lmax[h] = 0u;
#pragma unroll
    for (int e = 0; e < E; ++e) {
      if (key[e] != ~0ull) {
        const uint32_t j0 = R.hist[bp[e] & 0xfffu], j1 = R.hist[(bp[e] & 0xfffu) + 1u];
        pairs[j0 + (bp[e] >> 12)] = key[e];
        bp[e] = j0 | ((j1 - j0) << 12);
        lmax[e / EG] = max(lmax[e / EG], j1 - j0);
      }
    }
    lds_barrier();
    HGS_TQ(3)
#pragma unroll
    for (int h = 0; h < E / EG; ++h) {
      for (uint32_t sidx = 0; sidx < lmax[h]; ++sidx) {
        u64 other[EG];
#pragma unroll
        for (int e = 0; e < EG; ++e) {
          const uint32_t w = bp[h * EG + e];
          const bool on = sidx < ((w >> 12) & 0xffu);
          other[e] = pairs[on ? (w & 0xfffu) + sidx : 0u];
        }
#pragma unroll
        for (int e = 0; e < EG; ++e) {
          const uint32_t w = bp[h * EG + e];
          const bool on = sidx < ((w >> 12) & 0xffu);
          bp[h * EG + e] = w + ((on && other[e] < key[h * EG + e]) ? (1u << 20) : 0u);
        }
      }
    }
#pragma unroll
    for (int e = 0; e < E; ++e) bp[e] = (bp[e] & 0xfffu) + (bp[e] >> 20);
  } else {
#pragma unroll
    for (int e = 0; e < E; ++e) {
      const uint32_t k = (uint32_t)e * NT + (uint32_t)tid;
      if (k < n) pairs[k] = key[e];
    }
    __syncthreads();
    bitonic_sort<NT>(pairs, n);
#pragma unroll
    for (int e = 0; e < E; ++e) {
      const uint32_t k = (uint32_t)e * NT + (uint32_t)tid;
      key[e] = (k < n) ? pairs[k] : ~0ull;
      bp[e] = k;
    }
  }
  lds_barrier();
#pragma unroll
  for (int e = 0; e < E; ++e) {
    const uint32_t k = (uint32_t)e * NT + (uint32_t)tid;
    if (k < n) pairs[k] = (key[e] & 0xffffffffull) | ((u64)bp[e] << 32);
  }
  return degenerate;
}

template <int NT, bool SORTED = false>
__device__ __forceinline__ bool rank_keys_stream(const Layout& L, uint32_t start, uint32_t n, uint32_t NB,
                                                 unsigned long long* pairs, RankLds& R) {
  const int tid = (int)threadIdx.x, lane = tid & 63, wv = tid >> 6;
  constexpr int JB = NT >= 1024 ? 14 : 12;
  constexpr uint32_t JM = (1u << JB) - 1u;
  const unsigned long long* __restrict__ keys = L.keys + start;
  const uint32_t last = n - 1u;
  {
    uint32_t lo = 0xffffffffu, hi = 0u;
#pragma unroll 4
    for (uint32_t k = tid; k < n; k += NT) {
      const uint32_t d = (uint32_t)(keys[k] >> 32);
      lo = min(lo, d); hi = max(hi, d);
    }
    hi = hgs_wave_max_u32(hi);
    lo = ~hgs_wave_max_u32(~lo);
    lds_barrier();
    if (lane == 0) { atomicMin(&R.dmin, lo); atomicMax(&R.dmax, hi); }
  }
  lds_barrier();
  const float flo = __uint_as_float(R.dmin);
  const float range = __uint_as_float(R.dmax) - flo;
  const float scale = range > 1e-30f ? (float)NB / range : 0.0f;
  const float bmax = (float)(NB - 1u);
  auto bucket_of = [&](u64 key) { return (uint32_t)fminf((__uint_as_float((uint32_t)(key >> 32)) - flo) * scale, bmax); };
#pragma unroll 4
  for (uint32_t k = tid; k < n; k += NT) atomicAdd(&R.hist[bucket_of(keys[k])], 1u);
  lds_barrier();
  bucket_scan<NT>(R, NB);
  lds_barrier();
  const bool degenerate = R.maxcnt > (uint32_t)HGS_RANK_BUCKET_MAX;
  uint32_t rk[16];
  if (!degenerate) {
#pragma unroll 4
    for (uint32_t k = tid; k < n; k += NT) {
      const u64 key = keys[k];
      pairs[atomicAdd(&R.hist[bucket_of(key)], 1u)] = key;
    }
    lds_barrier();
#pragma unroll
    for (int e0 = 0; e0 < 16; e0 += 4) {
      if ((uint32_t)e0 * NT >= n) break;
      u64 key[4];
      uint32_t w[4], lmax = 0;
#pragma unroll
      for (int e = 0; e < 4; ++e) {
        const uint32_t k = (uint32_t)(e0 + e) * NT + (uint32_t)tid;
        key[e] = keys[min(k, last)];
      }
#pragma unroll
      for (int e = 0; e < 4; ++e) {
        const uint32_t k = (uint32_t)(e0 + e) * NT + (uint32_t)tid;
        const uint32_t b = bucket_of(key[e]);
        const uint32_t j1 = R.hist[b], j0 = b ? R.hist[b - 1u] : 0u;
        const uint32_t len = k < n ? j1 - j0 : 0u;
        w[e] = j0 | (len << JB);
        lmax = max(lmax, len);
      }
      for (uint32_t sidx = 0; sidx < lmax; ++sidx) {
        u64 other[4];
#pragma unroll
        for (int e = 0; e < 4; ++e) {
          const bool on = sidx < ((w[e] >> JB) & 0xffu);
          other[e] = pairs[on ? (w[e] & JM) + sidx : 0u];
        }
#pragma unroll
        for (int e = 0; e < 4; ++e) {
          const bool on = sidx < ((w[e] >> JB) & 0xffu);
          w[e] += (on && other[e] < key[e]) ? (1u << (JB + 8)) : 0u;
        }
      }
#pragma unroll
      for (int e = 0; e < 4; ++e) rk[e0 + e] = (w[e] & JM) + (w[e] >> (JB + 8));
    }
    lds_barrier();
#pragma unroll
    for (int e = 0; e < 16; ++e) {
      const uint32_t k = (uint32_t)e * NT + (uint32_t)tid;
      if (k < n) {
        if (SORTED) pairs[rk[e]] = keys[k];
        else pairs[k] = (keys[k] & 0xffffffffull) | ((u64)rk[e] << 32);
      }
    }
    if (SORTED) lds_barrier();
  } else {
    for (uint32_t k = tid; k < n; k += NT) pairs[k] = keys[k];
    __syncthreads();
    bitonic_sort<NT>(pairs, n);
    if (!SORTED) {
      for (uint32_t k = tid; k < n; k += NT) pairs[k] = (pairs[k] & 0xffffffffull) | ((u64)k << 32);
      lds_barrier();
    }
  }
  return degenerate;
}

template <int NT, bool CH>
__device__ __forceinline__ void rank_sort_tile(const View& v, const Layout& L, uint32_t order_pos, int g, uint32_t start, uint32_t n,
                                               unsigned long long* pairs, RankLds& R, GatherLds<64>& S, bool& degenerate_out,
                                               unsigned long long* tp) {
  const int tid = (int)threadIdx.x, lane = tid & 63;
  constexpr int GU = HGS_RANK_GU;
  const int t = g % v.T;
  const GeomRec* __restrict__ geom = L.geom + (size_t)(g / v.T) * v.P;
  const uint32_t* __restrict__ cbase = L.chunk_base + (size_t)(g / v.T) * v.nblk;
  const int tx = t % v.grid_x, ty = t / v.grid_x;
  const float x0 = (float)(tx * HGS_TILE), y0 = (float)(ty * HGS_TILE);
  uint32_t NB = 256u;
  while (NB < 2u * n && NB < (uint32_t)HGS_RANK_NB_MAX) NB <<= 1;
  for (uint32_t i = tid; i <= NB; i += NT) R.hist[i] = 0u;
  if (tid < 8) R.tot16[tid] = 0u;
  if (tid == 0) { R.dmin = 0xffffffffu; R.dmax = 0u; R.maxcnt = 0u; }
  u64 keyp[GU];
#pragma unroll
  for (int u = 0; u < GU; ++u) {
    const uint32_t k = (uint32_t)u * NT + (uint32_t)tid;
    const u64 kv = L.keys[start + min(k, n - 1u)];
    keyp[u] = (k < n) ? kv : ~0ull;
  }
  uint4 Aa[GU], Ab[GU], Ac[GU], Ba[GU], Bb[GU], Bc[GU];
  uint32_t Aoff[GU], Acb[GU], Boff[GU], Bcb[GU];
  u64 Apr[GU], Bpr[GU];
#define HGS_RANK_ISSUE(X, u, PR)                                                              \
  {                                                                                           \
    const u64 pr__ = (PR);                                                                    \
    const uint32_t idx__ = pr__ == ~0ull ? 0u : (uint32_t)pr__;                               \
    const uint4* gp__ = reinterpret_cast<const uint4*>(&geom[idx__]);                         \
    X##a[u] = gp__[0]; X##b[u] = gp__[1]; X##c[u] = gp__[2]; X##off[u] = gp__[3].x;           \
    X##cb[u] = cbase[idx__ >> 8];                                                             \
    X##pr[u] = pr__;                                                                          \
  }
  bool degenerate;
  const bool early = n <= 8u * NT;
  if (early) {
#pragma unroll
    for (int u = 0; u < GU; ++u) HGS_RANK_ISSUE(A, u, keyp[u]);
    if (n <= 2u * NT) degenerate = rank_keys<2, NT>(L, start, n, NB, keyp, pairs, R);
    else if (n <= 4u * NT) degenerate = rank_keys<4, NT>(L, start, n, NB, keyp, pairs, R);
    else degenerate = rank_keys<8, NT>(L, start, n, NB, keyp, pairs, R);
  } else {
    degenerate = rank_keys_stream<NT>(L, start, n, NB, pairs, R);
  }
  degenerate_out = degenerate;
#ifdef HGS_TIMELINE
  tp[0] = wall_clock64();
#endif
  uint16_t* __restrict__ masks = reinterpret_cast<uint16_t*>(R.hist);
  uint32_t acc[4] = {0u, 0u, 0u, 0u};
#define HGS_RANK_ROUND(X, r)                       \
  _Pragma("unroll") for (int u = 0; u < GU; ++u) {                                            \
    const uint32_t k__ = ((r) * (uint32_t)GU + (uint32_t)u) * NT + (uint32_t)tid;             \
    HGS_RANK_ISSUE(X, u, (k__ < n) ? pairs[k__] : ~0ull);                                     \
  }
#define HGS_RANK_CONSUME(X)                                                                   \
  _Pragma("unroll") for (int u = 0; u < GU; ++u) {                                            \
    if (X##pr[u] != ~0ull) {                                                                  \
      const uint32_t k = (uint32_t)(X##pr[u] >> 32);                                          \
      uint32_t mask;                                                                          \
      HGS_EMIT_RECORD(mask, X##a[u], X##b[u], X##c[u], X##off[u], X##cb[u], k, CH, true)    \
      masks[k] = (uint16_t)mask;                                                              \
      _Pragma("unroll") for (int wd = 0; wd < 4; ++wd) acc[wd] += hgs_spread4((mask >> (4 * wd)) & 0xfu); \
    }                                                                                         \
  }
  if (degenerate || !early) {
    HGS_RANK_ROUND(A, 0u)
  } else {
#pragma unroll
    for (int u = 0; u < GU; ++u) {
      const uint32_t k = (uint32_t)u * NT + (uint32_t)tid;
      Apr[u] = (k < n) ? pairs[k] : ~0ull;
    }
  }
  const uint32_t per_round = (uint32_t)GU * NT;
  for (uint32_t r = 0; r * per_round < n; r += 2u) {
    const bool hb = (r + 1u) * per_round < n, ha = (r + 2u) * per_round < n;
    if (hb) { HGS_RANK_ROUND(B, r + 1u) }
    HGS_RANK_CONSUME(A)
    if (r < 4u) HGS_TQ(4 + r)
    if (ha) { HGS_RANK_ROUND(A, r + 2u) }
    if (hb) { HGS_RANK_CONSUME(B) }
    if (r < 3u) HGS_TQ(5 + r)
  }
#undef HGS_RANK_ISSUE
#undef HGS_RANK_ROUND
#undef HGS_RANK_CONSUME
  {
    uint32_t w16[8];
#pragma unroll
    for (int wd = 0; wd < 4; ++wd) { w16[2 * wd] = acc[wd] & 0x00ff00ffu; w16[2 * wd + 1] = (acc[wd] >> 8) & 0x00ff00ffu; }
#pragma unroll
    for (int i = 0; i < 8; ++i) w16[i] = hgs_wave_incl_scan(w16[i]);
    if (lane == 63) {
#pragma unroll
      for (int i = 0; i < 8; ++i) if (w16[i]) atomicAdd(&R.tot16[i], w16[i]);
    }
  }
  lds_barrier();
#ifdef HGS_TIMELINE
  tp[1] = wall_clock64();
#endif
  CellAlloc ca;
  if (tid < 64) {
    const int c = lane & 15;
    const uint32_t word = R.tot16[2 * (c >> 2) + (c & 1)];
    hgs_alloc_cell_ranges_issue(L, order_pos, (word >> (16 * ((c >> 1) & 1))) & 0xffffu, ca);
  }
  cell_lists_from_masks<NT, CH>(v, L, order_pos, start, n, masks, S, ca, tp);
}

template <int NT, bool CH>
__device__ __forceinline__ void sort_rank_body(const View& v, const Layout& L, const hgs_status* __restrict__ status,
                                               unsigned long long* pairs, RankLds& R, GatherLds<64>& S) {
  if (status->overflow) return;
  const uint32_t active = status->active_tiles;
  const uint32_t G = gridDim.x, ncu = G / 3u, na = min(active, G);
  const bool remap = HGS_SORT_LIGHT > 0 && G == 3u * ncu && status->reserved[1] >= 768u &&
                     na >= 2u * ncu + 3u * (uint32_t)HGS_SORT_LIGHT;
  for (uint32_t b0 = blockIdx.x; b0 < active; b0 += gridDim.x) {
    uint32_t b = b0;
    if (remap && b0 < na) {
      constexpr uint32_t H = (uint32_t)HGS_SORT_LIGHT;
      if (b0 >= ncu && b0 < ncu + H) b = na - 1u - (b0 - ncu);
      else if (b0 >= 2u * ncu && b0 < 2u * ncu + H) b = na - 1u - H - (b0 - 2u * ncu);
      else if (b0 >= na - 2u * H) { const uint32_t j = na - 1u - b0; b = j < H ? ncu + j : 2u * ncu + (j - H); }
    }
    const uint4 tr = L.tile_rec[b];
    const int g = (int)tr.x;
    const uint32_t n = tr.y, start = tr.z;
    if (n == 0 || n > (uint32_t)HGS_SORT_LDS_MAX) continue;
#ifdef HGS_TIMELINE
    const unsigned long long tp0 = wall_clock64();
#endif
    bool degenerate;
    unsigned long long tp[4] = {0, 0, 0, 0};
    rank_sort_tile<NT, CH>(v, L, b, g, start, n, pairs, R, S, degenerate, tp);
#ifdef HGS_TIMELINE
    if (threadIdx.x == 0 && b < HGS_TL_SLOTS) {
      const unsigned long long tpe = wall_clock64();
      auto cl = [](unsigned long long d) { return d > 0xffffull ? 0xffffull : d; };
      hgs_tl[5][b][0] = tp0;
      hgs_tl[5][b][1] = tpe;
      hgs_tl[5][b][2] = degenerate ? 1 : 0;
      hgs_tl[5][b][3] = ((unsigned long long)1 << 32) | n;
      hgs_tl[2][b][0] = cl(tp[0] - tp0) | (cl(tp[1] - tp[0]) << 16) | (cl(tp[2] - tp[1]) << 32) | (cl(tp[3] - tp[2]) << 48);
      hgs_tl[2][b][1] = cl(tpe - tp[3]);
      hgs_tl[2][b][2] = cl(hgs_s_tq[0] - tp0) | (cl(hgs_s_tq[1] - hgs_s_tq[0]) << 16) | (cl(hgs_s_tq[2] - hgs_s_tq[1]) << 32) | (cl(hgs_s_tq[3] - hgs_s_tq[2]) << 48);
      hgs_tl[2][b][3] = cl(hgs_s_tq[4] - tp[0]) | (cl(hgs_s_tq[5] - tp[0]) << 16) | (cl(hgs_s_tq[6] - tp[0]) << 32) | (cl(hgs_s_tq[7] - tp[0]) << 48);
    }
#endif
    lds_barrier();
  }
}
#undef HGS_EMIT_RECORD
}

static_assert(16 * HGS_SORT_NT >= 4096, "the rank sort takes every list of the LDS class");
#define HGS_SORT_LDS_KERNEL(NAME, CH)                                                                                  \
  extern "C" __global__ void __launch_bounds__(HGS_SORT_NT) __attribute__((amdgpu_waves_per_eu(HGS_SORT_WAVES_PER_EU, HGS_SORT_WAVES_PER_EU))) \
  NAME(View v, Layout L, const hgs_status* __restrict__ status) {                                                      \
    __shared__ unsigned long long pairs[4096];                                                                         \
    __shared__ GatherLds<64> S;                                                                                        \
    __shared__ RankLds R;                                                                                              \
    HGS_TL_BEGIN();                                                                                                    \
    sort_rank_body<HGS_SORT_NT, CH>(v, L, status, pairs, R, S);                                                        \
    HGS_TL_END(3, 0u);                                                                                                 \
  }
HGS_SORT_LDS_KERNEL(hgs_k_sort_lds, false)
HGS_SORT_LDS_KERNEL(hgs_k_sort_lds_ch, true)

extern "C" __global__ void __launch_bounds__(1024)
hgs_k_sort_large(View v, Layout L, const hgs_status* __restrict__ status) {
  __shared__ unsigned long long keys[16384];
  __shared__ GatherLds<256> S;
  if (status->overflow) return;
  const uint32_t b = blockIdx.x;
  if (b >= status->active_tiles) return;
  const int t = (int)L.tile_order[b];
  const uint32_t start = L.tile_start[t];
  const uint32_t n = L.tile_n[t];
  if (n <= (uint32_t)HGS_SORT_LDS_MAX || n > 16384u) return;
  {
    __shared__ RankLds R;
    const uint32_t NB = (uint32_t)HGS_RANK_NB_MAX;
    for (uint32_t i = threadIdx.x; i <= NB; i += 1024) R.hist[i] = 0u;
    if (threadIdx.x == 0) { R.dmin = 0xffffffffu; R.dmax = 0u; R.maxcnt = 0u; }
    rank_keys_stream<1024, true>(L, start, n, NB, keys, R);
    __syncthreads();
  }
  gather_records_single<256>(v, L, t, b, start, n, keys, 1024, S);
}

extern "C" __global__ void __launch_bounds__(1024)
hgs_k_sort_huge(View v, Layout L, const hgs_status* __restrict__ status) {
  if (status->overflow) return;
  const uint32_t b = blockIdx.x;
  if (b >= status->active_tiles) return;
  const int t = (int)L.tile_order[b];
  const uint32_t start = L.tile_start[t];
  const uint32_t n = L.tile_n[t];
  if (n <= 16384u) return;
  __shared__ GatherLds<256> S;
  bitonic_sort<1024>(L.keys + start, n);
  gather_records<256>(v, L, t, b, start, n, L.keys + start, 1024, S);
}
```

### humangaussian_amd/csrc/entryrec.h

```cpp
#pragma once
#include <stddef.h>
#include <stdint.h>

#include "../../include/hgs_rast.h"
#include "cellmask.h"

struct __attribute__((aligned(16))) SortRec {
  float mx, my;
  float qa, qb, qc;
  float op, r, g, b, depth;
  uint32_t entry;
  uint32_t tag;
};
#define HGS_REC_WORDS ((uint32_t)(sizeof(SortRec) / sizeof(uint32_t)))
#define HGS_REC_F4 ((int)(sizeof(SortRec) / 16))
#define HGS_REC_TAG_WORD ((uint32_t)(offsetof(SortRec, tag) / sizeof(uint32_t)))
static_assert(sizeof(SortRec) == 48, "a record is three 16 B words");
static_assert(offsetof(SortRec, entry) == 40 && offsetof(SortRec, tag) == 44, "entry id and tag close the record's third word");

#define HGS_CHUNK_RECS 64u
#define HGS_TAG_MASK_BITS 16
#define HGS_TAG_POS_SHIFT 16
#define HGS_TAG_COUNT_SHIFT 22
#define HGS_TAG_ROWS_SHIFT 28
#define HGS_TAG_CHUNK_BITS 6
#define HGS_TAG_CHUNK_FIELD ((1u << HGS_TAG_CHUNK_BITS) - 1u)
static_assert(HGS_TAG_MASK_BITS == HGS_CELLS_PER_TILE, "one mask bit per cell");
static_assert(HGS_CHUNK_RECS == 1u << HGS_TAG_CHUNK_BITS, "position and count - 1 of a 64-record chunk fit their 6-bit fields");
static_assert(HGS_TAG_POS_SHIFT >= HGS_TAG_MASK_BITS && HGS_TAG_COUNT_SHIFT >= HGS_TAG_POS_SHIFT + HGS_TAG_CHUNK_BITS &&
              HGS_TAG_ROWS_SHIFT >= HGS_TAG_COUNT_SHIFT + HGS_TAG_CHUNK_BITS && HGS_TAG_ROWS_SHIFT < 32,
              "the four tag fields do not overlap");

HGS_HD uint32_t hgs_rec_tag(uint32_t mask, uint32_t k, uint32_t n, bool chunk_rows) {
  const uint32_t left = n - (k & ~(HGS_CHUNK_RECS - 1u));
  return (mask & 0xffffu) | ((k & (HGS_CHUNK_RECS - 1u)) << HGS_TAG_POS_SHIFT) |
         (((left < HGS_CHUNK_RECS ? left : HGS_CHUNK_RECS) - 1u) << HGS_TAG_COUNT_SHIFT) | (chunk_rows ? 1u << HGS_TAG_ROWS_SHIFT : 0u);
}
HGS_HD uint32_t hgs_tag_mask(uint32_t tag) { return tag & 0xffffu; }
HGS_HD uint32_t hgs_tag_pos(uint32_t tag) { return (tag >> HGS_TAG_POS_SHIFT) & HGS_TAG_CHUNK_FIELD; }
HGS_HD uint32_t hgs_tag_count(uint32_t tag) { return ((tag >> HGS_TAG_COUNT_SHIFT) & HGS_TAG_CHUNK_FIELD) + 1u; }
HGS_HD bool hgs_tag_chunk_rows(uint32_t tag) { return ((tag >> HGS_TAG_ROWS_SHIFT) & 1u) != 0u; }

#define HGS_PAIRS_PER_ENTRY 16
#define HGS_ENTRY_BITS 27
#define HGS_ENTRY_MASK ((1u << HGS_ENTRY_BITS) - 1u)
static_assert(HGS_MAX_ENTRY_CAPACITY == 1ll << HGS_ENTRY_BITS, "the ABI's capacity limit is what the entry field holds");
static_assert(HGS_PAIRS_PER_ENTRY < (1 << (32 - HGS_ENTRY_BITS)), "the pair count fits above the entry id");
static_assert(HGS_PAIRS_PER_ENTRY == HGS_CELLS_PER_TILE, "an entry has at most one pair per cell");

HGS_HD uint32_t hgs_entpair_x(uint32_t entry, uint32_t pairs) { return entry | (pairs << HGS_ENTRY_BITS); }
HGS_HD uint32_t hgs_entpair_entry(uint32_t x) { return x & HGS_ENTRY_MASK; }
HGS_HD uint32_t hgs_entpair_pairs(uint32_t x) { return x >> HGS_ENTRY_BITS; }

#define HGS_CELL_KEY_BITS 4
static_assert(HGS_CELLS_PER_TILE == 1 << HGS_CELL_KEY_BITS, "the cell index is the key's low bits");
HGS_HD uint32_t hgs_cell_key(uint32_t g, uint32_t c) { return g * (uint32_t)HGS_CELLS_PER_TILE + c; }
HGS_HD int hgs_cell_key_tile(uint32_t key) { return (int)(key >> HGS_CELL_KEY_BITS); }
HGS_HD int hgs_cell_key_cell(uint32_t key) { return (int)(key & ((1u << HGS_CELL_KEY_BITS) - 1u)); }
```

### humangaussian_amd/csrc/hgs_common.h

```cpp
#pragma once
#include <hip/hip_runtime.h>
#include <stdint.h>

#include "../../include/hgs_rast.h"
#include "cellmask.h"
#include "entryrec.h"

#define HGS_TILE 16
#define HGS_TILE_PIX 256
#define HGS_BLOCK 256
#define HGS_ROW_GROUPS 16
#define HGS_TILES_PER_WG 64
#define HGS_RB 16
#define HGS_ROW_F4 (HGS_RB * HGS_REC_F4 + 1)
#define HGS_BWD_BLOCK_WAVES 12
#define HGS_SEGLEN 128
#define HGS_NEAR_Z 0.2f
#define HGS_ALPHA_MIN (1.0f / 255.0f)
#define HGS_ALPHA_MAX 0.99f
#define HGS_T_EPS 0.0001f
#define HGS_CSTATE_FLOATS (6 * 16)
#define HGS_ROW_FLOATS 12
#define HGS_GROW_F4 (HGS_ROW_FLOATS / 4)
#define HGS_PROW_FLOATS 10
#define HGS_PROW_F2 (HGS_PROW_FLOATS / 2)
#define HGS_SORT_LDS_MAX 4096
#define HGS_NCLS 33
#define HGS_NXCD 8
#define HGS_NFC 11

struct __attribute__((aligned(16))) GeomRec {
  float mx, my;
  float ca, cb, cc;
  float op;
  float r, g, b;
  float depth;
  uint32_t rect_lo;
  uint32_t rect_hi;
  uint32_t offset;
  int32_t radius;
  uint32_t clamped;
  uint32_t flags;
};

#define HGS_LOG2E 1.4426950408889634f

struct __attribute__((aligned(16))) CellInfo {
  uint32_t base;
  uint32_t len;
  uint32_t sbase;
  uint32_t pbase;
};

struct __attribute__((aligned(128))) CounterLine { uint32_t v; };
struct __attribute__((aligned(128))) Counters {
  unsigned long long alloc_eb;
  __attribute__((aligned(128))) uint32_t entry_alloc;
  __attribute__((aligned(128))) uint32_t max_n;
  CounterLine cls_hist[HGS_NCLS];
  CounterLine cls_cur[HGS_NCLS];
  __attribute__((aligned(128))) unsigned long long alloc_ps;
  __attribute__((aligned(128))) unsigned long long sched[HGS_NXCD][16];
};
static_assert(2 + HGS_NFC <= 16, "a die's row of work counters is one 128 B line");

__host__ __device__ __forceinline__ uint32_t hgs_item_class(uint32_t cnt) {
  return cnt >= HGS_SEGLEN ? 0u : (cnt >= (2u * HGS_SEGLEN + 2u) / 3u ? 1u : (cnt >= (HGS_SEGLEN + 2u) / 3u ? 2u : 3u));
}

__host__ __device__ __forceinline__ uint32_t hgs_cell_class(uint32_t len) {
  const uint32_t nb = (len + HGS_RB - 1) / HGS_RB;
  return nb >= 33u ? 0u : nb >= 25u ? 1u : nb >= 17u ? 2u : nb >= 13u ? 3u : nb >= 9u ? 4u : nb >= 7u ? 5u : nb >= 5u ? 6u : 11u - nb;
}

struct Layout {
  GeomRec* geom;
  uint32_t* tile_n;
  uint32_t* tile_start;
  uint32_t* tile_order;
  uint4* tile_rec;
  uint32_t* hist;
  uint32_t* tile_gbase;
  uint32_t* tile_count;
  uint32_t* chunk_sums;
  uint32_t* chunk_base;
  CellInfo* cell_info;
  uint32_t* fwd_cells;
  uint4* items_part;
  Counters* ctr;
  unsigned long long* keys;
  SortRec* recs;
  uint2* cell_list;
  uint2* entpair;
  float* cstate;
  uint32_t full_cap;
  uint4* items_full;
  uint32_t* n_contrib;
};

__host__ __device__ __forceinline__ size_t hgs_die_cells(int TT) { return (size_t)16 * (size_t)((TT + HGS_NXCD - 1) / HGS_NXCD); }

struct Cam {
  const float* viewmatrix;
  const float* projmatrix;
  const float* campos;
  const float* bg;
  float tanfovx, tanfovy, focal_x, focal_y;
};

struct View {
  Cam cam[HGS_MAX_VIEWS];
  float scale_modifier;
  int32_t W, H, grid_x, grid_y, T;
  int32_t B, TT;
  int32_t P, M, D, nblk;
  int32_t cpw, nwg, lds_bins;
  uint32_t entry_capacity;
  int32_t max_tile_hint;
  int32_t act;
  int32_t pairchunks;
};

static inline size_t hgs_align_up(size_t v, size_t a) { return (v + a - 1) / a * a; }

__device__ __forceinline__ int hgs_cell_of(int w, int j) { return (((w >> 1) << 1) + (j >> 1)) * 4 + ((w & 1) << 1) + (j & 1); }
#define HGS_FWD_THREADS 256

__device__ __forceinline__ bool hgs_eval_alpha(float dx, float dy, float qa, float qb,
                                               float qc, float op, float& G, float& alpha,
                                               float& m2, float& m3) {
  m2 = __builtin_fmaf(qa, dx, qb * dy);
  m3 = qc * dy;
  const float p2 = __builtin_fmaf(dx, m2, m3 * dy);
  G = __builtin_amdgcn_exp2f(p2);
  const float og = op * G;
  alpha = fminf(HGS_ALPHA_MAX, og);
  return (p2 <= 0.0f) && (og >= HGS_ALPHA_MIN);
}

#define HGS_DPP_ROW_SHR(n) (0x110 + (n))
#define HGS_DPP_ROW_BCAST15 0x142
#define HGS_DPP_ROW_BCAST31 0x143
#define HGS_DPP_QUAD_PERM(a, b, c, d) ((a) | ((b) << 2) | ((c) << 4) | ((d) << 6))
#define HGS_DPP_ROW_MIRROR 0x140
#define HGS_DPP_ROW_HALF_MIRROR 0x141
#define HGS_DPP_ROW_ROR(n) (0x120 + (n))

__device__ __forceinline__ uint32_t hgs_wave_incl_scan(uint32_t v) {
  int x = (int)v;
  x += __builtin_amdgcn_update_dpp(0, x, HGS_DPP_ROW_SHR(1), 0xf, 0xf, false);
  x += __builtin_amdgcn_update_dpp(0, x, HGS_DPP_ROW_SHR(2), 0xf, 0xf, false);
  x += __builtin_amdgcn_update_dpp(0, x, HGS_DPP_ROW_SHR(4), 0xf, 0xf, false);
  x += __builtin_amdgcn_update_dpp(0, x, HGS_DPP_ROW_SHR(8), 0xf, 0xf, false);
  x += __builtin_amdgcn_update_dpp(0, x, HGS_DPP_ROW_BCAST15, 0xa, 0xf, false);
  x += __builtin_amdgcn_update_dpp(0, x, HGS_DPP_ROW_BCAST31, 0xc, 0xf, false);
  return (uint32_t)x;
}

__device__ __forceinline__ uint32_t hgs_wave_max_u32(uint32_t v) {
  int x = (int)v;
  x = (int)max((uint32_t)x, (uint32_t)__builtin_amdgcn_update_dpp(0, x, HGS_DPP_ROW_SHR(1), 0xf, 0xf, false));
  x = (int)max((uint32_t)x, (uint32_t)__builtin_amdgcn_update_dpp(0, x, HGS_DPP_ROW_SHR(2), 0xf, 0xf, false));
  x = (int)max((uint32_t)x, (uint32_t)__builtin_amdgcn_update_dpp(0, x, HGS_DPP_ROW_SHR(4), 0xf, 0xf, false));
  x = (int)max((uint32_t)x, (uint32_t)__builtin_amdgcn_update_dpp(0, x, HGS_DPP_ROW_SHR(8), 0xf, 0xf, false));
  x = (int)max((uint32_t)x, (uint32_t)__builtin_amdgcn_update_dpp(0, x, HGS_DPP_ROW_BCAST15, 0xa, 0xf, false));
  x = (int)max((uint32_t)x, (uint32_t)__builtin_amdgcn_update_dpp(0, x, HGS_DPP_ROW_BCAST31, 0xc, 0xf, false));
  return (uint32_t)__builtin_amdgcn_readlane(x, 63);
}

template <int NT>
__device__ __forceinline__ uint32_t hgs_block_excl_scan(uint32_t v, uint32_t* wtot,
                                                        uint32_t& total) {
  const int lane = threadIdx.x & 63, w = threadIdx.x >> 6;
  const uint32_t incl = hgs_wave_incl_scan(v);
  __syncthreads();
  if (lane == 63) wtot[w] = incl;
  __syncthreads();
  uint32_t base = 0, tot = 0;
#pragma unroll
  for (int k = 0; k < NT / 64; ++k) {
    const uint32_t t = wtot[k];
    if (k < w) base += t;
    tot += t;
  }
  total = tot;
  return base + incl - v;
}

#include "gridscan.h"

#ifdef HGS_TIMELINE
#define HGS_TL_KERNELS 6
#define HGS_TL_SLOTS (1 << 17)
#define HGS_TL_BEGIN() const unsigned long long tl_t0__ = wall_clock64()
#define HGS_TL_END(KID, TAG)                                                                        \
  do {                                                                                              \
    const unsigned long long tl_t1__ = wall_clock64();                                              \
    const uint32_t tl_slot__ = blockIdx.x * (blockDim.x >> 6) + (threadIdx.x >> 6);                 \
    if ((threadIdx.x & 63) == 0 && tl_slot__ < HGS_TL_SLOTS) {                                      \
      const uint32_t hw__ = __builtin_amdgcn_s_getreg((31 << 11) | 4);                              \
      const uint32_t xcc__ = __builtin_amdgcn_s_getreg((31 << 11) | 20);                            \
      hgs_tl[KID][tl_slot__][0] = tl_t0__;                                                          \
      hgs_tl[KID][tl_slot__][1] = tl_t1__;                                                          \
      hgs_tl[KID][tl_slot__][2] = ((unsigned long long)xcc__ << 32) | hw__;                         \
      hgs_tl[KID][tl_slot__][3] = (unsigned long long)(TAG);                                        \
    }                                                                                               \
  } while (0)
#define HGS_TLI_DECL() unsigned long long tli_max__ = 0, tli_t__ = 0; uint32_t tli_it__ = 0, tli_n__ = 0
#define HGS_TLI_BEGIN() tli_t__ = wall_clock64()
#define HGS_TLI_END(IT, CLS)                                                                        \
  do {                                                                                              \
    const unsigned long long d__ = wall_clock64() - tli_t__;                                        \
    ++tli_n__;                                                                                      \
    if (d__ > tli_max__) { tli_max__ = d__; tli_it__ = ((uint32_t)(IT) << 4) | (uint32_t)((CLS) + 1); } \
  } while (0)
#define HGS_TLI_TAG() ((tli_max__ << 40) | ((unsigned long long)tli_n__ << 28) | (tli_it__ & 0xfffffffu))
#else
#define HGS_TL_BEGIN() do {} while (0)
#define HGS_TL_END(KID, TAG) do {} while (0)
#define HGS_TLI_DECL() do {} while (0)
#define HGS_TLI_BEGIN() do {} while (0)
#define HGS_TLI_END(IT, CLS) do {} while (0)
#define HGS_TLI_TAG() 1u
#endif
```

### humangaussian_amd/csrc/preprocess.hip

```cpp
#include "hgs_common.h"

namespace {

__device__ __constant__ const float SH_C0 = 0.28209479177387814f;
__device__ __constant__ const float SH_C1 = 0.4886025119029199f;
__device__ __constant__ const float SH_C2[5] = {1.0925484305920792f, -1.0925484305920792f,
                                                0.31539156525252005f, -1.0925484305920792f,
                                                0.5462742152960396f};
__device__ __constant__ const float SH_C3[7] = {-0.5900435899266435f, 2.890611442640554f,
                                                -0.4570457994644658f, 0.3731763325901154f,
                                                -0.4570457994644658f, 1.445305721320277f,
                                                -0.5900435899266435f};

struct Cov3 { float c0, c1, c2, c3, c4, c5; };

struct RotScale {
  float R00, R01, R02, R10, R11, R12, R20, R21, R22;
  float sx, sy, sz;
};

__device__ __forceinline__ float act_opacity(float raw, int act) {
  return (act & HGS_ACT_OPACITY_SIGMOID) ? 1.0f / (1.0f + expf(-raw)) : raw;
}
__device__ __forceinline__ void act_scale(const float* __restrict__ scales, int i, int act, float& s0, float& s1, float& s2) {
// ... 260 lines not shown
    rec.g = colors_precomp[3 * i + 1];
    rec.b = colors_precomp[3 * i + 2];
  } else {
    const float* cp = cam.campos;
    const float ddx = x - cp[0], ddy = y - cp[1], ddz = z - cp[2];
    const float n = sqrtf(ddx * ddx + ddy * ddy + ddz * ddz);
    float col[3];
    if (sh_block_vectorisable(v.M)) {
      float sh48[48];
      load_sh_block(shs + (size_t)i * v.M * 3, v.M, sh48);
      eval_sh(v.D, sh48, ddx / n, ddy / n, ddz / n, col);
    } else {
      eval_sh(v.D, shs + (size_t)i * v.M * 3, ddx / n, ddy / n, ddz / n, col);
    }
    uint32_t cl = 0;
#pragma unroll
    for (int ch = 0; ch < 3; ++ch) {
      col[ch] = col[ch] + 0.5f;
      if (col[ch] < 0.0f) { cl |= (1u << ch); col[ch] = 0.0f; }
    }
    rec.r = col[0]; rec.g = col[1]; rec.b = col[2];
    rec.clamped = cl;
  }
  return (uint32_t)tight_area;
}

__device__ __forceinline__ void store_geom(GeomRec* dstp, const GeomRec& rec) {
  uint4* dst = reinterpret_cast<uint4*>(dstp);
  const uint4* src = reinterpret_cast<const uint4*>(&rec);
  dst[0] = src[0]; dst[1] = src[1]; dst[2] = src[2]; dst[3] = src[3];
}

}

__device__ __forceinline__ uint32_t chunk_prefix(uint32_t tt, uint32_t* wtot, uint32_t* chunk_sum) {
  uint32_t total;
  const uint32_t ex = hgs_block_excl_scan<HGS_BLOCK>(tt, wtot, total);
  if (threadIdx.x == 0) *chunk_sum = total;
  return ex;
}

__device__ __forceinline__ void zero_counters(const Layout& L) {
  if (blockIdx.x == 0)
    for (uint32_t i = threadIdx.x; i < sizeof(Counters) / 4; i += blockDim.x) reinterpret_cast<uint32_t*>(L.ctr)[i] = 0u;
}

template <bool AA>
__device__ __forceinline__ void preprocess_fwd_body(
    const View& v, const Layout& L, const float* __restrict__ means3D, const float* __restrict__ shs,
    const float* __restrict__ colors_precomp, const float* __restrict__ opacities, const float* __restrict__ scales,
    const float* __restrict__ rotations, const float* __restrict__ cov3D_precomp, int32_t* __restrict__ radii,
    float* __restrict__ zero_leaf) {
  extern __shared__ __attribute__((aligned(16))) uint32_t lds_hist[];
  __shared__ uint32_t wtot[HGS_BLOCK / 64];
  zero_counters(L);
  const int b = (int)blockIdx.x / v.nwg, lw = (int)blockIdx.x % v.nwg;
  const Cam cam = v.cam[b];
  for (int t = threadIdx.x; t < v.T; t += HGS_BLOCK) lds_hist[t] = 0u;
  __syncthreads();
  const int gxm = v.grid_x;
  for (int c = 0; c < v.cpw; ++c) {
    const int chunk = lw * v.cpw + c;
    if (chunk >= v.nblk) break;
    const int i = chunk * HGS_BLOCK + threadIdx.x;
    uint32_t tt = 0;
    if (i < v.P) {
      GeomRec rec;
      tt = preprocess_one<AA>(v, cam, i, means3D, shs, colors_precomp, opacities, scales, rotations,
                              cov3D_precomp, rec);
      radii[(size_t)b * v.P + i] = rec.radius;
      if (zero_leaf) {
        float* z = zero_leaf + ((size_t)b * v.P + i) * 3;
        z[0] = 0.0f; z[1] = 0.0f; z[2] = 0.0f;
      }
      store_geom(&L.geom[(size_t)b * v.P + i], rec);
      if (tt) {
        const int minx = rec.rect_lo & 0xffffu, miny = rec.rect_lo >> 16;
        const int maxx = rec.rect_hi & 0xffffu, maxy = rec.rect_hi >> 16;
        for (int ty = miny; ty < maxy; ++ty)
          for (int tx = minx; tx < maxx; ++tx) atomicAdd(&lds_hist[ty * gxm + tx], 1u);
      }
    }
    const uint32_t off = chunk_prefix(tt, wtot, &L.chunk_sums[(size_t)b * v.nblk + chunk]);
    if (i < v.P && tt) L.geom[(size_t)b * v.P + i].offset = off;
  }
  __syncthreads();
  uint32_t* row = L.hist + (size_t)blockIdx.x * v.T;
  for (int t = threadIdx.x; t < v.T; t += HGS_BLOCK) row[t] = lds_hist[t];
}

template <bool AA>
__device__ __forceinline__ void preprocess_fwd_ga_body(
    const View& v, const Layout& L, const float* __restrict__ means3D, const float* __restrict__ shs,
    const float* __restrict__ colors_precomp, const float* __restrict__ opacities, const float* __restrict__ scales,
    const float* __restrict__ rotations, const float* __restrict__ cov3D_precomp, int32_t* __restrict__ radii,
    float* __restrict__ zero_leaf) {
  __shared__ uint32_t wtot[HGS_BLOCK / 64];
  zero_counters(L);
  const int b = (int)blockIdx.x / v.nblk, chunk = (int)blockIdx.x % v.nblk;
  const Cam cam = v.cam[b];
  const int i = chunk * HGS_BLOCK + threadIdx.x;
  uint32_t tt = 0;
  if (i < v.P) {
    GeomRec rec;
    tt = preprocess_one<AA>(v, cam, i, means3D, shs, colors_precomp, opacities, scales, rotations,
                            cov3D_precomp, rec);
    radii[(size_t)b * v.P + i] = rec.radius;
    if (zero_leaf) {
      float* z = zero_leaf + ((size_t)b * v.P + i) * 3;
      z[0] = 0.0f; z[1] = 0.0f; z[2] = 0.0f;
    }
    store_geom(&L.geom[(size_t)b * v.P + i], rec);
    if (tt) {
      const int minx = rec.rect_lo & 0xffffu, miny = rec.rect_lo >> 16;
      const int maxx = rec.rect_hi & 0xffffu, maxy = rec.rect_hi >> 16;
      uint32_t* cnt = L.tile_count + (size_t)b * v.T;
      for (int ty = miny; ty < maxy; ++ty)
        for (int tx = minx; tx < maxx; ++tx) atomicAdd(&cnt[ty * v.grid_x + tx], 1u);
    }
  }
  const uint32_t off = chunk_prefix(tt, wtot, &L.chunk_sums[blockIdx.x]);
  if (i < v.P && tt) L.geom[(size_t)b * v.P + i].offset = off;
}

#define HGS_PRE_FWD_KERNEL(NAME, BODY, AA)                                                                       \
  extern "C" __global__ void __launch_bounds__(HGS_BLOCK) NAME(                                                  \
      View v, Layout L, const float* __restrict__ means3D, const float* __restrict__ shs,                        \
      const float* __restrict__ colors_precomp, const float* __restrict__ opacities,                             \
      const float* __restrict__ scales, const float* __restrict__ rotations,                                     \
      const float* __restrict__ cov3D_precomp, int32_t* __restrict__ radii, float* __restrict__ zero_leaf) {     \
    BODY<AA>(v, L, means3D, shs, colors_precomp, opacities, scales, rotations, cov3D_precomp, radii, zero_leaf);   \
  }
HGS_PRE_FWD_KERNEL(hgs_k_preprocess_fwd, preprocess_fwd_body, false)
HGS_PRE_FWD_KERNEL(hgs_k_preprocess_fwd_ga, preprocess_fwd_ga_body, false)
HGS_PRE_FWD_KERNEL(hgs_k_preprocess_fwd_aa, preprocess_fwd_body, true)
HGS_PRE_FWD_KERNEL(hgs_k_preprocess_fwd_ga_aa, preprocess_fwd_ga_body, true)

namespace {

template <int DEG, int MODE, int AA>
__device__ __forceinline__ void preprocess_bwd_body(
    const View& v, const Layout& L, const hgs_status* __restrict__ status,
    const float* __restrict__ grad_rows, const float* __restrict__ means3D,
    const float* __restrict__ shs, const float* __restrict__ colors_precomp,
    const float* __restrict__ opacities_raw,
    const float* __restrict__ scales, const float* __restrict__ rotations,
    const float* __restrict__ cov3D_precomp, float* __restrict__ dL_dmeans3D,
    float* __restrict__ dL_dmeans2D, float* __restrict__ dL_dshs, float* __restrict__ dL_dcolors,
    float* __restrict__ dL_dopac, float* __restrict__ dL_dscales, float* __restrict__ dL_drots,
    float* __restrict__ dL_dcov3D, float* __restrict__ pack, int pack_F) {
  constexpr int NC = (DEG + 1) * (DEG + 1);
  constexpr bool SINGLE = MODE != 0;
  constexpr bool VPAR = MODE == 2;
  constexpr int NV = 23 + 3 * NC;
  extern __shared__ float red[];
  int i = blockIdx.x * HGS_BLOCK + threadIdx.x, bview = 0, il = threadIdx.x;
  if (VPAR) {
    il = (int)threadIdx.x & 63;
    bview = __builtin_amdgcn_readfirstlane((int)threadIdx.x >> 6);
    i = blockIdx.x * 64 + il;
  }
  const bool mine = (i < v.P) && (bview < v.B);
  const bool staged = MODE == 1 && DEG > 0 && dL_dshs != nullptr && shs != nullptr && hgs_sh_staged(v.M) &&
                      (int)(blockIdx.x + 1) * HGS_BLOCK <= v.P && pack == nullptr;
  if (staged) {
    stage_sh_chunk(shs, v.M, (int)blockIdx.x * HGS_BLOCK, HGS_BLOCK, red);
    __syncthreads();
  }
  if (!VPAR && !mine) return;
  if (!mine) i = 0;
  if (bview >= v.B) bview = 0;
  const bool ok = status->overflow == 0;
  const bool aa = AA == 1 || (AA == 2 && (v.act & HGS_ANTIALIAS) != 0);

  float x, y, z;
  Cov3 s;
  RotScale rs;
  float4 q = make_float4(0.f, 0.f, 0.f, 0.f);
  float q_inv_norm = 1.0f;
  const bool want_sh = dL_dshs != nullptr && shs != nullptr;
  float sh48[48];
  auto load_inputs = [&]() {
    x = means3D[3 * i + 0]; y = means3D[3 * i + 1]; z = means3D[3 * i + 2];
    if (cov3D_precomp) {
      const float* c = cov3D_precomp + 6 * (size_t)i;
      s.c0 = c[0]; s.c1 = c[1]; s.c2 = c[2]; s.c3 = c[3]; s.c4 = c[4]; s.c5 = c[5];
    } else {
      rs = make_rotscale(scales, rotations, i, v.scale_modifier, v.act);
      s = cov3d_from(rs);
      q = act_rotation(rotations, i, v.act, q_inv_norm);
    }
    if (DEG > 0 && want_sh) {
      if (staged) {
        load_sh_row_lds(red + (int)threadIdx.x * (hgs_sh_row_f4(v.M) * 4), v.M, sh48);
      } else if (sh_block_vectorisable(v.M)) {
        load_sh_block(shs + (size_t)i * v.M * 3, v.M, sh48);
      } else {
        const float* shp = shs + (size_t)i * v.M * 3;
#pragma unroll
        for (int k = 3; k < 48; ++k) sh48[k] = (k < 3 * NC) ? shp[k] : 0.f;
      }
    }
  };
  if (SINGLE) load_inputs();

  float a_mean[3] = {0.f, 0.f, 0.f}, a_sc[3] = {0.f, 0.f, 0.f}, a_rot[4] = {0.f, 0.f, 0.f, 0.f};
  float a_cov[6] = {0.f, 0.f, 0.f, 0.f, 0.f, 0.f}, a_col[3] = {0.f, 0.f, 0.f}, a_op = 0.f;
  float a_sh[3 * NC];
#pragma unroll
  for (int k = 0; k < 3 * NC; ++k) a_sh[k] = 0.f;
  float a_m2x = 0.f, a_m2y = 0.f, a_rad = 0.f;

  const int b_begin = VPAR ? bview : 0;
  const int b_end = SINGLE ? b_begin + 1 : v.B;
  for (int b = b_begin; b < b_end; ++b) {
    if (!SINGLE) {
      asm volatile("" ::: "memory");
      load_inputs();
    }
    const Cam cam = v.cam[b];
    const float* __restrict__ V = cam.viewmatrix;
    const float* __restrict__ PM = cam.projmatrix;
    const GeomRec g = L.geom[(size_t)b * v.P + i];
    float gmx = 0.f, gmy = 0.f;
    if ((g.radius > 0) && ok && mine) {
      float gA = 0.f, gB = 0.f, gC = 0.f, gop = 0.f, gr = 0.f, gg = 0.f, gb = 0.f, gdep = 0.f;
      const int rw = (int)(g.rect_hi & 0xffffu) - (int)(g.rect_lo & 0xffffu);
      const int rh = (int)(g.rect_hi >> 16) - (int)(g.rect_lo >> 16);
      const int tt = rw * rh;
      const float4* rows = reinterpret_cast<const float4*>(grad_rows) +
                           HGS_GROW_F4 * (size_t)(L.chunk_base[(size_t)b * v.nblk + (i >> 8)] + g.offset);
#define HGS_ROWS_UNROLL_MANY 4
      constexpr int RU = SINGLE ? 1 : HGS_ROWS_UNROLL_MANY;
      for (int k0 = 0; k0 < tt; k0 += RU) {
        float4 r0[RU], r1[RU], r2[RU];
#pragma unroll
        for (int u = 0; u < RU; ++u) {
          const int k = min(k0 + u, tt - 1);
          r0[u] = rows[HGS_GROW_F4 * k + 0]; r1[u] = rows[HGS_GROW_F4 * k + 1]; r2[u] = rows[HGS_GROW_F4 * k + 2];
        }
#pragma unroll
        for (int u = 0; u < RU; ++u) {
          if (k0 + u < tt) {
            gmx += r0[u].x; gmy += r0[u].y; gA += r0[u].z; gB += r0[u].w;
            gC += r1[u].x; gop += r1[u].y; gr += r1[u].z; gg += r1[u].w;
            gb += r2[u].x; gdep += r2[u].y;
          }
        }
      }
      if (!aa) a_op += gop;
      a_col[0] += gr; a_col[1] += gg; a_col[2] += gb;

      Proj2D pj;
      view_point(V, x, y, z, pj.tx0, pj.ty0, pj.tz);
      project_cov(cam, V, s, pj);

      const float a = pj.a, bq_ = pj.b, c = pj.c;
      const float inv2 = 1.0f / (pj.det * pj.det);
      float dLa = inv2 * (-c * c * gA + bq_ * c * gB - bq_ * bq_ * gC);
      float dLb = inv2 * (2.0f * bq_ * c * gA - (pj.det + 2.0f * bq_ * bq_) * gB + 2.0f * a * bq_ * gC);
      float dLc = inv2 * (-bq_ * bq_ * gA + a * bq_ * gB - a * a * gC);
      if (aa) {
        const float ratio = aa_ratio(pj), rho = aa_rho(ratio);
        a_op += gop * rho;
        if (ratio > HGS_AA_MIN_RATIO) {
          const float k = gop * act_opacity(opacities_raw[i], v.act) / (2.0f * rho * pj.det);
          dLa += k * (pj.c0 - ratio * c);
          dLc += k * (pj.a0 - ratio * a);
          dLb += -2.0f * k * bq_ * (1.0f - ratio);
        }
      }

      const float M0[3] = {pj.M00, pj.M01, pj.M02}, M1[3] = {pj.M10, pj.M11, pj.M12};
      float dcov[6];
      dcov[0] = dLa * M0[0] * M0[0] + dLb * M0[0] * M1[0] + dLc * M1[0] * M1[0];
      dcov[3] = dLa * M0[1] * M0[1] + dLb * M0[1] * M1[1] + dLc * M1[1] * M1[1];
      dcov[5] = dLa * M0[2] * M0[2] + dLb * M0[2] * M1[2] + dLc * M1[2] * M1[2];
      dcov[1] = 2.f * dLa * M0[0] * M0[1] + dLb * (M0[0] * M1[1] + M0[1] * M1[0]) + 2.f * dLc * M1[0] * M1[1];
      dcov[2] = 2.f * dLa * M0[0] * M0[2] + dLb * (M0[0] * M1[2] + M0[2] * M1[0]) + 2.f * dLc * M1[0] * M1[2];
      dcov[4] = 2.f * dLa * M0[1] * M0[2] + dLb * (M0[1] * M1[2] + M0[2] * M1[1]) + 2.f * dLc * M1[1] * M1[2];
#pragma unroll
      for (int k = 0; k < 6; ++k) a_cov[k] += dcov[k];

      const float u[3] = {pj.u0, pj.u1, pj.u2}, w[3] = {pj.w0, pj.w1, pj.w2};
      float dM0[3], dM1[3];
#pragma unroll
      for (int k = 0; k < 3; ++k) {
        dM0[k] = 2.f * dLa * u[k] + dLb * w[k];
        dM1[k] = 2.f * dLc * w[k] + dLb * u[k];
      }
      const float dJ00 = dM0[0] * V[0] + dM0[1] * V[4] + dM0[2] * V[8];
      const float dJ02 = dM0[0] * V[2] + dM0[1] * V[6] + dM0[2] * V[10];
      const float dJ11 = dM1[0] * V[1] + dM1[1] * V[5] + dM1[2] * V[9];
      const float dJ12 = dM1[0] * V[2] + dM1[1] * V[6] + dM1[2] * V[10];
      const float tzi = 1.0f / pj.tz, tz2 = tzi * tzi, tz3 = tz2 * tzi;
      const float fx = cam.focal_x, fy = cam.focal_y;
      float dt[3];
      dt[0] = pj.clx ? 0.f : -fx * tz2 * dJ02;
      dt[1] = pj.cly ? 0.f : -fy * tz2 * dJ12;
      dt[2] = -fx * tz2 * dJ00 - fy * tz2 * dJ11 + 2.f * fx * pj.tx * tz3 * dJ02 +
              2.f * fy * pj.ty * tz3 * dJ12;
      dt[2] += gdep;
      float dmean[3] = {0.f, 0.f, 0.f};
#pragma unroll
      for (int bq = 0; bq < 3; ++bq)
        dmean[bq] += V[4 * bq + 0] * dt[0] + V[4 * bq + 1] * dt[1] + V[4 * bq + 2] * dt[2];

      const float dpx = gmx * 0.5f * (float)v.W, dpy = gmy * 0.5f * (float)v.H;
      const float hx = PM[0] * x + PM[4] * y + PM[8] * z + PM[12];
      const float hy = PM[1] * x + PM[5] * y + PM[9] * z + PM[13];
      const float hw = PM[3] * x + PM[7] * y + PM[11] * z + PM[15];
      const float pw = 1.0f / (hw + 0.0000001f);
      const float dhx = dpx * pw, dhy = dpy * pw;
      const float dhw = -(dpx * hx + dpy * hy) * pw * pw;
#pragma unroll
      for (int bq = 0; bq < 3; ++bq)
        dmean[bq] += PM[4 * bq + 0] * dhx + PM[4 * bq + 1] * dhy + PM[4 * bq + 3] * dhw;

      if (!cov3D_precomp) {
        const float G00 = dcov[0], G11 = dcov[3], G22 = dcov[5];
        const float G01 = 0.5f * dcov[1], G02 = 0.5f * dcov[2], G12 = 0.5f * dcov[4];
        const float Lm[3][3] = {{rs.R00 * rs.sx, rs.R01 * rs.sy, rs.R02 * rs.sz},
                                {rs.R10 * rs.sx, rs.R11 * rs.sy, rs.R12 * rs.sz},
                                {rs.R20 * rs.sx, rs.R21 * rs.sy, rs.R22 * rs.sz}};
        const float Gm[3][3] = {{G00, G01, G02}, {G01, G11, G12}, {G02, G12, G22}};
        const float Rm[3][3] = {{rs.R00, rs.R01, rs.R02}, {rs.R10, rs.R11, rs.R12},
                                {rs.R20, rs.R21, rs.R22}};
        const float sv[3] = {rs.sx, rs.sy, rs.sz};
        float D[3][3];
#pragma unroll
        for (int k = 0; k < 3; ++k) {
          float ds = 0.f;
#pragma unroll
          for (int ii = 0; ii < 3; ++ii) {
            const float dLik = 2.f * (Gm[ii][0] * Lm[0][k] + Gm[ii][1] * Lm[1][k] + Gm[ii][2] * Lm[2][k]);
            ds += dLik * Rm[ii][k];
            D[ii][k] = dLik * sv[k];
          }
          a_sc[k] += (v.act & HGS_GRAD_SCALE_TRUE_DERIVATIVE) ? ds * v.scale_modifier : ds;
        }
        const float r = q.x, qx = q.y, qy = q.z, qz = q.w;
        a_rot[0] += 2.f * (-qz * D[0][1] + qy * D[0][2] + qz * D[1][0] - qx * D[1][2] - qy * D[2][0] + qx * D[2][1]);
        a_rot[1] += 2.f * (qy * D[0][1] + qz * D[0][2] + qy * D[1][0] - 2.f * qx * D[1][1] - r * D[1][2] +
                           qz * D[2][0] + r * D[2][1] - 2.f * qx * D[2][2]);
        a_rot[2] += 2.f * (-2.f * qy * D[0][0] + qx * D[0][1] + r * D[0][2] + qx * D[1][0] + qz * D[1][2] -
                           r * D[2][0] + qz * D[2][1] - 2.f * qy * D[2][2]);
        a_rot[3] += 2.f * (-2.f * qz * D[0][0] - r * D[0][1] + qx * D[0][2] + r * D[1][0] - 2.f * qz * D[1][1] +
                           qy * D[1][2] + qx * D[2][0] + qy * D[2][1]);
      }

      if (want_sh) {
        float draw[3];
        draw[0] = (g.clamped & 1u) ? 0.f : gr;
        draw[1] = (g.clamped & 2u) ? 0.f : gg;
        draw[2] = (g.clamped & 4u) ? 0.f : gb;
        const float* cp = cam.campos;
        const float ox = x - cp[0], oy = y - cp[1], oz = z - cp[2];
        const float n = sqrtf(ox * ox + oy * oy + oz * oz);
        const float dx = ox / n, dy = oy / n, dz = oz / n;
        float basis[NC];
        basis[0] = SH_C0;
        float ddir[3] = {0.f, 0.f, 0.f};
        if constexpr (DEG > 0) {
          basis[1] = -SH_C1 * dy; basis[2] = SH_C1 * dz; basis[3] = -SH_C1 * dx;
#pragma unroll
          for (int ch = 0; ch < 3; ++ch) {
            ddir[0] += draw[ch] * (-SH_C1 * sh48[9 + ch]);
            ddir[1] += draw[ch] * (-SH_C1 * sh48[3 + ch]);
            ddir[2] += draw[ch] * (SH_C1 * sh48[6 + ch]);
          }
        }
        if constexpr (DEG > 1) {
          const float xx = dx * dx, yy = dy * dy, zz = dz * dz;
          const float xy = dx * dy, yz = dy * dz, xz = dx * dz;
          basis[4] = SH_C2[0] * xy; basis[5] = SH_C2[1] * yz;
          basis[6] = SH_C2[2] * (2.f * zz - xx - yy);
          basis[7] = SH_C2[3] * xz; basis[8] = SH_C2[4] * (xx - yy);
#pragma unroll
          for (int ch = 0; ch < 3; ++ch) {
            const float s4 = sh48[12 + ch], s5 = sh48[15 + ch], s6 = sh48[18 + ch], s7 = sh48[21 + ch], s8 = sh48[24 + ch];
            ddir[0] += draw[ch] * (SH_C2[0] * dy * s4 + SH_C2[2] * -2.f * dx * s6 + SH_C2[3] * dz * s7 + SH_C2[4] * 2.f * dx * s8);
            ddir[1] += draw[ch] * (SH_C2[0] * dx * s4 + SH_C2[1] * dz * s5 + SH_C2[2] * -2.f * dy * s6 + SH_C2[4] * -2.f * dy * s8);
            ddir[2] += draw[ch] * (SH_C2[1] * dy * s5 + SH_C2[2] * 4.f * dz * s6 + SH_C2[3] * dx * s7);
          }
          if constexpr (DEG > 2) {
            basis[9] = SH_C3[0] * dy * (3.f * xx - yy);
            basis[10] = SH_C3[1] * xy * dz;
            basis[11] = SH_C3[2] * dy * (4.f * zz - xx - yy);
            basis[12] = SH_C3[3] * dz * (2.f * zz - 3.f * xx - 3.f * yy);
            basis[13] = SH_C3[4] * dx * (4.f * zz - xx - yy);
            basis[14] = SH_C3[5] * dz * (xx - yy);
            basis[15] = SH_C3[6] * dx * (xx - 3.f * yy);
#pragma unroll
            for (int ch = 0; ch < 3; ++ch) {
              const float s9 = sh48[27 + ch], s10 = sh48[30 + ch], s11 = sh48[33 + ch], s12 = sh48[36 + ch];
              const float s13 = sh48[39 + ch], s14 = sh48[42 + ch], s15 = sh48[45 + ch];
              ddir[0] += draw[ch] * (SH_C3[0] * s9 * 6.f * xy + SH_C3[1] * s10 * yz + SH_C3[2] * s11 * -2.f * xy +
                                     SH_C3[3] * s12 * -6.f * xz + SH_C3[4] * s13 * (4.f * zz - 3.f * xx - yy) +
                                     SH_C3[5] * s14 * 2.f * xz + SH_C3[6] * s15 * 3.f * (xx - yy));
              ddir[1] += draw[ch] * (SH_C3[0] * s9 * 3.f * (xx - yy) + SH_C3[1] * s10 * xz +
                                     SH_C3[2] * s11 * (4.f * zz - xx - 3.f * yy) + SH_C3[3] * s12 * -6.f * yz +
// ... 50 lines not shown
    const int nthr = (int)blockDim.x;
#pragma unroll
    for (int k = 0; k < NV; ++k) red[k * nthr + threadIdx.x] = vals[k];
    __syncthreads();
    if (bview != 0 || !mine) return;
#pragma unroll
    for (int k = 0; k < NV; ++k) vals[k] = 0.f;
#pragma unroll 1
    for (int bb = 0; bb < v.B; ++bb) {
      const float* col = red + bb * 64 + il;
#pragma unroll
      for (int k = 0; k < NV - 1; ++k) vals[k] += col[k * nthr];
      vals[NV - 1] = fmaxf(vals[NV - 1], col[(NV - 1) * nthr]);
    }
    {
      int vi = 0;
#pragma unroll
      for (int k = 0; k < 3; ++k) a_mean[k] = vals[vi++];
#pragma unroll
      for (int k = 0; k < 3; ++k) a_sc[k] = vals[vi++];
#pragma unroll
      for (int k = 0; k < 4; ++k) a_rot[k] = vals[vi++];
#pragma unroll
      for (int k = 0; k < 6; ++k) a_cov[k] = vals[vi++];
#pragma unroll
      for (int k = 0; k < 3; ++k) a_col[k] = vals[vi++];
      a_op = vals[vi++];
#pragma unroll
      for (int k = 0; k < 3 * NC; ++k) a_sh[k] = vals[vi++];
      a_m2x = vals[vi++]; a_m2y = vals[vi++]; a_rad = vals[vi++];
    }
  }
  if (pack) {
    float* __restrict__ row = pack + (size_t)i * pack_F;
    row[0] = a_mean[0]; row[1] = a_mean[1]; row[2] = a_mean[2];
    row[3] = a_m2x; row[4] = a_m2y; row[5] = 0.f;
    if (dL_dshs) {
#pragma unroll
      for (int k = 0; k < 3 * NC; ++k)
        if (k < 3 * v.M) row[6 + k] = a_sh[k];
      for (int k = 3 * NC; k < 3 * v.M; ++k) row[6 + k] = 0.f;
    }
    float* __restrict__ tail = row + 6 + 3 * v.M;
    float gop = a_op;
    if (v.act & HGS_ACT_OPACITY_SIGMOID) {
      const float y = act_opacity(opacities_raw[i], v.act);
      gop = gop * ((1.0f - y) * y);
    }
    tail[0] = gop;
    if (dL_dscales) {
      if (v.act & HGS_ACT_SCALE_EXP) {
        float s0, s1, s2;
        act_scale(scales, i, v.act, s0, s1, s2);
        a_sc[0] *= s0; a_sc[1] *= s1; a_sc[2] *= s2;
      }
      tail[1] = a_sc[0]; tail[2] = a_sc[1]; tail[3] = a_sc[2];
    }
    if (dL_drots) {
      if (!SINGLE && !cov3D_precomp) q = act_rotation(rotations, i, v.act, q_inv_norm);
      if (v.act & HGS_ACT_ROTATION_NORMALIZE) {
        const float dot = q.x * a_rot[0] + q.y * a_rot[1] + q.z * a_rot[2] + q.w * a_rot[3];
        a_rot[0] = (a_rot[0] - q.x * dot) * q_inv_norm;
        a_rot[1] = (a_rot[1] - q.y * dot) * q_inv_norm;
        a_rot[2] = (a_rot[2] - q.z * dot) * q_inv_norm;
        a_rot[3] = (a_rot[3] - q.w * dot) * q_inv_norm;
      }
      tail[4] = a_rot[0]; tail[5] = a_rot[1]; tail[6] = a_rot[2]; tail[7] = a_rot[3];
    }
    tail[8] = a_rad;
    return;
  }

  if (dL_dshs && staged) {
    float* row = red + (int)threadIdx.x * (hgs_sh_row_f4(v.M) * 4);
#pragma unroll
    for (int k = 0; k < 3 * NC; ++k)
      if (k < 3 * v.M) row[k] = a_sh[k];
    for (int k = 3 * NC; k < 3 * v.M; ++k) row[k] = 0.f;
    __syncthreads();
    unstage_sh_chunk(dL_dshs, v.M, (int)blockIdx.x * HGS_BLOCK, red);
  } else if (dL_dshs) {
    float* out = dL_dshs + (size_t)i * v.M * 3;
    if (sh_block_vectorisable(v.M)) {
      float4* o4 = reinterpret_cast<float4*>(out);
      const int nq = (v.M * 3) >> 2;
#pragma unroll
      for (int qd = 0; qd < 12; ++qd)
        if (qd < nq) {
          float4 t;
          t.x = (4 * qd + 0 < 3 * NC) ? a_sh[(4 * qd + 0) % (3 * NC)] : 0.f;
          t.y = (4 * qd + 1 < 3 * NC) ? a_sh[(4 * qd + 1) % (3 * NC)] : 0.f;
          t.z = (4 * qd + 2 < 3 * NC) ? a_sh[(4 * qd + 2) % (3 * NC)] : 0.f;
          t.w = (4 * qd + 3 < 3 * NC) ? a_sh[(4 * qd + 3) % (3 * NC)] : 0.f;
          o4[qd] = t;
        }
    } else {
#pragma unroll
      for (int k = 0; k < 3 * NC; ++k)
        if (k < 3 * v.M) out[k] = a_sh[k];
      for (int k = 3 * NC; k < 3 * v.M; ++k) out[k] = 0.f;
    }
  }
  if (dL_dmeans3D) {
    dL_dmeans3D[3 * i + 0] = a_mean[0]; dL_dmeans3D[3 * i + 1] = a_mean[1]; dL_dmeans3D[3 * i + 2] = a_mean[2];
  }
  if (dL_dcolors) {
    dL_dcolors[3 * i + 0] = a_col[0]; dL_dcolors[3 * i + 1] = a_col[1]; dL_dcolors[3 * i + 2] = a_col[2];
  }
  if (dL_dopac) {
    float g = a_op;
    if (v.act & HGS_ACT_OPACITY_SIGMOID) {
      const float y = act_opacity(opacities_raw[i], v.act);
      g = g * ((1.0f - y) * y);
    }
    dL_dopac[i] = g;
  }
  if (dL_dscales) {
    if (v.act & HGS_ACT_SCALE_EXP) {
      float s0, s1, s2;
      act_scale(scales, i, v.act, s0, s1, s2);
      a_sc[0] *= s0; a_sc[1] *= s1; a_sc[2] *= s2;
    }
    dL_dscales[3 * i + 0] = a_sc[0]; dL_dscales[3 * i + 1] = a_sc[1]; dL_dscales[3 * i + 2] = a_sc[2];
  }
  if (dL_drots) {
    if (!SINGLE && !cov3D_precomp) q = act_rotation(rotations, i, v.act, q_inv_norm);
    if (v.act & HGS_ACT_ROTATION_NORMALIZE) {
      const float dot = q.x * a_rot[0] + q.y * a_rot[1] + q.z * a_rot[2] + q.w * a_rot[3];
      a_rot[0] = (a_rot[0] - q.x * dot) * q_inv_norm;
      a_rot[1] = (a_rot[1] - q.y * dot) * q_inv_norm;
      a_rot[2] = (a_rot[2] - q.z * dot) * q_inv_norm;
      a_rot[3] = (a_rot[3] - q.w * dot) * q_inv_norm;
    }
    reinterpret_cast<float4*>(dL_drots)[i] = make_float4(a_rot[0], a_rot[1], a_rot[2], a_rot[3]);
  }
  if (dL_dcov3D) {
    float* o = dL_dcov3D + 6 * (size_t)i;
#pragma unroll
    for (int k = 0; k < 6; ++k) o[k] = a_cov[k];
  }
}

}

#define HGS_PRE_BWD_FORMS(X)                                                                                              \
  X(0, 0, 0, hgs_k_preprocess_bwd_d0, HGS_BLOCK)                             \
  X(1, 0, 0, hgs_k_preprocess_bwd_d1, HGS_BLOCK)                                                                          \
  X(2, 0, 0, hgs_k_preprocess_bwd_d2, HGS_BLOCK)                                                                          \
  X(3, 0, 2, hgs_k_preprocess_bwd_d3, HGS_BLOCK)            \
  X(0, 1, 0, hgs_k_preprocess_bwd_s0, HGS_BLOCK)                                                             \
  X(1, 1, 0, hgs_k_preprocess_bwd_s1, HGS_BLOCK)                                                                          \
  X(2, 1, 0, hgs_k_preprocess_bwd_s2, HGS_BLOCK)                                                                          \
  X(3, 1, 0, hgs_k_preprocess_bwd_s3, HGS_BLOCK)                                                                          \
  X(0, 2, 0, hgs_k_preprocess_bwd_p0, 1024)                \
  X(1, 2, 0, hgs_k_preprocess_bwd_p1, 1024)                 \
  X(2, 2, 0, hgs_k_preprocess_bwd_p2, 512)                                                                                \
  X(3, 2, 0, hgs_k_preprocess_bwd_p3, 512)                                                                                \
       \
  X(0, 0, 1, hgs_k_preprocess_bwd_d0_aa, HGS_BLOCK)                                                                       \
  X(1, 0, 1, hgs_k_preprocess_bwd_d1_aa, HGS_BLOCK)                                                                       \
  X(2, 0, 1, hgs_k_preprocess_bwd_d2_aa, HGS_BLOCK)                                                                       \
  X(0, 1, 1, hgs_k_preprocess_bwd_s0_aa, HGS_BLOCK)                                                                       \
  X(1, 1, 1, hgs_k_preprocess_bwd_s1_aa, HGS_BLOCK)                                                                       \
  X(2, 1, 1, hgs_k_preprocess_bwd_s2_aa, HGS_BLOCK)                                                                       \
  X(3, 1, 1, hgs_k_preprocess_bwd_s3_aa, HGS_BLOCK)                                                                       \
  X(0, 2, 1, hgs_k_preprocess_bwd_p0_aa, 1024)                                                                            \
  X(1, 2, 1, hgs_k_preprocess_bwd_p1_aa, 1024)                                                                            \
  X(2, 2, 1, hgs_k_preprocess_bwd_p2_aa, 512)                                                                             \
  X(3, 2, 1, hgs_k_preprocess_bwd_p3_aa, 512)

#define HGS_PRE_BWD_KERNEL(DEG, MODE, AA, NAME, THREADS)                                                 \
  extern "C" __global__ void __launch_bounds__(THREADS) NAME(                                       \
      View v, Layout L, const hgs_status* __restrict__ status, const float* __restrict__ grad_rows, \
      const float* __restrict__ means3D, const float* __restrict__ shs,                             \
      const float* __restrict__ colors_precomp, const float* __restrict__ opacities_raw,            \
      const float* __restrict__ scales,                                                             \
      const float* __restrict__ rotations, const float* __restrict__ cov3D_precomp,                 \
      float* __restrict__ dL_dmeans3D, float* __restrict__ dL_dmeans2D, float* __restrict__ dL_dshs, \
      float* __restrict__ dL_dcolors, float* __restrict__ dL_dopac, float* __restrict__ dL_dscales,  \
      float* __restrict__ dL_drots, float* __restrict__ dL_dcov3D, float* __restrict__ pack, int pack_F) { \
    preprocess_bwd_body<DEG, MODE, AA>(v, L, status, grad_rows, means3D, shs, colors_precomp, opacities_raw, scales, \
                             rotations, cov3D_precomp, dL_dmeans3D, dL_dmeans2D, dL_dshs,           \
                             dL_dcolors, dL_dopac, dL_dscales, dL_drots, dL_dcov3D, pack, pack_F);  \
  }
HGS_PRE_BWD_FORMS(HGS_PRE_BWD_KERNEL)
#undef HGS_PRE_BWD_KERNEL

namespace {
using PreBwdKernel = void (*)(View, Layout, const hgs_status*, const float*, const float*, const float*, const float*,
                              const float*, const float*, const float*, const float*, float*, float*, float*, float*,
                              float*, float*, float*, float*, float*, int);
struct PreBwdForm { PreBwdKernel kernel; const char* name; int threads; };
constexpr int HGS_PRE_BWD_ROWS = 24;
constexpr int hgs_pre_bwd_row(int aa, int mode, int deg) { return deg + 4 * mode + 12 * aa; }
struct PreBwdForms { PreBwdForm row[HGS_PRE_BWD_ROWS]; };
__host__ constexpr PreBwdForms hgs_make_pre_bwd_forms() {
  PreBwdForms t{};
#define HGS_PRE_BWD_ROW(DEG, MODE, AA, NAME, THREADS)                                      \
  if (AA != 1) t.row[hgs_pre_bwd_row(0, MODE, DEG)] = PreBwdForm{NAME, #NAME, THREADS};    \
  if (AA != 0) t.row[hgs_pre_bwd_row(1, MODE, DEG)] = PreBwdForm{NAME, #NAME, THREADS};
  HGS_PRE_BWD_FORMS(HGS_PRE_BWD_ROW)
#undef HGS_PRE_BWD_ROW
  return t;
}
constexpr PreBwdForms hgs_pre_bwd_forms = hgs_make_pre_bwd_forms();
__host__ constexpr bool hgs_pre_bwd_forms_complete() {
  for (int r = 0; r < HGS_PRE_BWD_ROWS; ++r)
    if (hgs_pre_bwd_forms.row[r].kernel == nullptr) return false;
  return true;
}
static_assert(hgs_pre_bwd_forms_complete(), "a (filter, mode, degree) combination without a kernel");
#define HGS_PRE_BWD_CHECK(DEG, MODE, AA, NAME, THREADS)                                                              \
  static_assert(MODE != 2 || ((THREADS) % 64 == 0 && (THREADS) <= 1024), #NAME ": a wave per view, <= 1024 threads"); \
  static_assert(MODE != 2 || (23 + 3 * (DEG + 1) * (DEG + 1)) * (THREADS) * 4 <= 160 * 1024, #NAME ": exchange buffer > LDS");
HGS_PRE_BWD_FORMS(HGS_PRE_BWD_CHECK)
#undef HGS_PRE_BWD_CHECK
}

extern "C" __global__ void __launch_bounds__(HGS_BLOCK)
hgs_k_mark_visible(const float* __restrict__ V, int P, const float* __restrict__ means3D,
                   uint8_t* __restrict__ present) {
  const int i = blockIdx.x * HGS_BLOCK + threadIdx.x;
  if (i >= P) return;
  const float x = means3D[3 * i + 0], y = means3D[3 * i + 1], z = means3D[3 * i + 2];
  const float tz = V[2] * x + V[6] * y + V[10] * z + V[14];
  present[i] = tz > HGS_NEAR_Z ? 1 : 0;
}
```

### include/hgs_rast.h

```cpp
#ifndef HGS_RAST_H
#define HGS_RAST_H

#include <stddef.h>
#include <stdint.h>

#ifdef __cplusplus
extern "C" {
#endif

#define HGS_MAX_VIEWS 16
#define HGS_MAX_ENTRY_CAPACITY (1ll << 27)

#define HGS_OK 0
#define HGS_EINVAL (-1)
#define HGS_ESHAPE (-2)

typedef struct hgs_settings {
  int32_t image_height;
  int32_t image_width;
  float tanfovx;
  float tanfovy;
  const float* bg;
  float scale_modifier;
  const float* viewmatrix;
  const float* projmatrix;
  int32_t sh_degree;
  const float* campos;
  int32_t prefiltered;
  int32_t debug;
} hgs_settings;

typedef struct hgs_status {
  uint32_t num_rendered;
  uint32_t active_tiles;
  uint32_t num_pairs;
  uint32_t bwd_groups;
  uint32_t overflow;
  uint32_t reserved[3];
} hgs_status;

size_t hgs_geom_bytes(int32_t P, int32_t image_height, int32_t image_width);
size_t hgs_bin_bytes(int64_t entry_capacity);
size_t hgs_img_bytes(int32_t image_height, int32_t image_width);
size_t hgs_bwd_scratch_bytes(int64_t num_rendered);
size_t hgs_bwd_scratch_bytes_pairs(int64_t num_rendered, int64_t num_pairs);
size_t hgs_geom_bytes_batch(int32_t B, int32_t P, int32_t image_height, int32_t image_width);
size_t hgs_img_bytes_batch(int32_t B, int32_t image_height, int32_t image_width);

#define HGS_FWD_STAGES 6
#define HGS_BWD_STAGES 4

int hgs_forward(const hgs_settings* s, int32_t P, int32_t M,
                const float* means3D, const float* shs, const float* colors_precomp,
                const float* opacities, const float* scales, const float* rotations,
                const float* cov3D_precomp,
                float* out_color, float* out_depth, float* out_alpha, int32_t* radii,
                void* geom, void* bin, int64_t entry_capacity, void* img,
                int32_t store_bwd_state, int32_t max_tile_entries_hint,
                hgs_status* status_host, int32_t status_host_mapped, void* status_event,
                void* const* stage_events, void* stream);

int hgs_forward_batch(const hgs_settings* views, int32_t B, int32_t P, int32_t M,
                      const float* means3D, const float* shs, const float* colors_precomp,
                      const float* opacities, const float* scales, const float* rotations,
                      const float* cov3D_precomp,
                      float* out_color, float* out_depth, float* out_alpha, int32_t* radii,
                      void* geom, void* bin, int64_t entry_capacity, void* img,
                      int32_t store_bwd_state, int32_t max_tile_entries_hint,
                      hgs_status* status_host, int32_t status_host_mapped, void* status_event,
                      void* const* stage_events, void* stream);

int hgs_backward_batch(const hgs_settings* views, int32_t B, int32_t P, int32_t M,
                       const float* means3D, const float* shs, const float* colors_precomp,
                       const float* opacities, const float* scales, const float* rotations,
                       const float* cov3D_precomp, const int32_t* radii,
                       const float* out_color, const float* out_depth, const float* out_alpha,
                       const float* dL_dout_color, const float* dL_dout_depth,
                       const float* dL_dout_alpha,
                       const void* geom, const void* bin, const void* img,
                       const hgs_status* status, int64_t entry_capacity, void* bwd_scratch,
                       float* dL_dmeans3D, float* dL_dmeans2D, float* dL_dshs,
                       float* dL_dcolors_precomp, float* dL_dopacities, float* dL_dscales,
                       float* dL_drotations, float* dL_dcov3D_precomp,
                       void* const* stage_events, void* stream);

#define HGS_ACT_OPACITY_SIGMOID 1
#define HGS_ACT_SCALE_EXP 2
#define HGS_ACT_ROTATION_NORMALIZE 4
#define HGS_GRAD_SCALE_TRUE_DERIVATIVE 8
#define HGS_ANTIALIAS 16
int hgs_forward_batch_act(const hgs_settings* views, int32_t B, int32_t P, int32_t M,
                          const float* means3D, const float* shs, const float* colors_precomp,
                          const float* opacities, const float* scales, const float* rotations,
                          const float* cov3D_precomp,
                          float* out_color, float* out_depth, float* out_alpha, int32_t* radii,
                          void* geom, void* bin, int64_t entry_capacity, void* img,
                          int32_t store_bwd_state, int32_t max_tile_entries_hint,
                          hgs_status* status_host, int32_t status_host_mapped, void* status_event,
                          void* const* stage_events, int32_t activation_flags, void* stream);
int hgs_forward_batch_act_leaf(const hgs_settings* views, int32_t B, int32_t P, int32_t M,
                               const float* means3D, const float* shs, const float* colors_precomp,
                               const float* opacities, const float* scales, const float* rotations,
                               const float* cov3D_precomp,
                               float* out_color, float* out_depth, float* out_alpha, int32_t* radii,
                               void* geom, void* bin, int64_t entry_capacity, void* img,
                               int32_t store_bwd_state, int32_t max_tile_entries_hint,
                               hgs_status* status_host, int32_t status_host_mapped, void* status_event,
                               void* const* stage_events, int32_t activation_flags, float* means2D_leaf, void* stream);
int hgs_backward_batch_act(const hgs_settings* views, int32_t B, int32_t P, int32_t M,
                           const float* means3D, const float* shs, const float* colors_precomp,
                           const float* opacities, const float* scales, const float* rotations,
                           const float* cov3D_precomp, const int32_t* radii,
                           const float* out_color, const float* out_depth, const float* out_alpha,
                           const float* dL_dout_color, const float* dL_dout_depth,
                           const float* dL_dout_alpha,
                           const void* geom, const void* bin, const void* img,
                           const hgs_status* status, int64_t entry_capacity, void* bwd_scratch,
                           float* dL_dmeans3D, float* dL_dmeans2D, float* dL_dshs,
                           float* dL_dcolors_precomp, float* dL_dopacities, float* dL_dscales,
                           float* dL_drotations, float* dL_dcov3D_precomp,
                           void* const* stage_events, int32_t activation_flags, void* stream);

int hgs_backward(const hgs_settings* s, int32_t P, int32_t M,
                 const float* means3D, const float* shs, const float* colors_precomp,
                 const float* opacities, const float* scales, const float* rotations,
                 const float* cov3D_precomp, const int32_t* radii,
                 const float* out_color, const float* out_depth, const float* out_alpha,
                 const float* dL_dout_color, const float* dL_dout_depth,
                 const float* dL_dout_alpha,
                 const void* geom, const void* bin, const void* img,
                 const hgs_status* status, int64_t entry_capacity, void* bwd_scratch,
                 float* dL_dmeans3D, float* dL_dmeans2D, float* dL_dshs,
                 float* dL_dcolors_precomp, float* dL_dopacities, float* dL_dscales,
                 float* dL_drotations, float* dL_dcov3D_precomp,
                 void* const* stage_events, void* stream);

int hgs_mark_visible(const hgs_settings* s, int32_t P, const float* means3D,
                     uint8_t* present, void* stream);

int hgs_knn_mean_dist2(int32_t P, const float* points, float* mean_dist2, void* stream);
size_t hgs_knn_scratch_bytes(int32_t P);
int hgs_knn_mean_dist2_grid(int32_t P, const float* points, float* mean_dist2, void* scratch, void* stream);

int hgs_reduce_view_packs(int32_t world, int64_t P, int32_t F, const float* gathered, float* out,
                          void* stream);
int hgs_reduce_view_packs_acc(int32_t world, int64_t P, int32_t F, const float* gathered, const float* acc_in,
                              float* out, void* stream);

int hgs_pack_view_contribution(int32_t P, int32_t M, const float* g_means3D, const float* g_means2D,
                               const float* g_sh, const float* g_opac, const float* g_scales,
                               const float* g_rot, const int32_t* radii, float* out, void* stream);

int hgs_backward_batch_packed(const hgs_settings* views, int32_t B, int32_t P, int32_t M, const float* means3D,
                              const float* shs, const float* opacities, const float* scales, const float* rotations,
                              const int32_t* radii, const float* out_color, const float* out_depth, const float* out_alpha,
                              const float* dL_dout_color, const float* dL_dout_depth, const float* dL_dout_alpha,
                              const void* geom, const void* bin, const void* img, const hgs_status* status,
                              int64_t entry_capacity, void* bwd_scratch, float* pack, float* dL_dmeans2D_views,
                              void* const* stage_events, int32_t activation_flags, void* stream);
int hgs_reduce_view_packs_unpack(int32_t world, int64_t P, int32_t M, const float* gathered, const float* acc_in,
                                 float* g_means3D, float* g_means2D, float* g_sh, float* g_opac, float* g_scales,
                                 float* g_rot, int32_t* radii, void* stream);

int hgs_densify_stats(int32_t B, int32_t P, const float* dL_dmeans2D, const int32_t* radii, const uint8_t* keep,
                      float* xyz_gradient_accum, float* denom, float* max_radii2D, int32_t* radii_max,
                      uint8_t* visibility, void* stream);

int hgs_densify_masks(int32_t P, const float* xyz_gradient_accum, const float* denom, const float* scales,
                      int32_t scales_are_log, const float* opacity, int32_t opacity_is_logit,
                      const float* max_radii2D, float grad_threshold, float percent_dense, float extent,
                      float min_opacity, float max_screen_size, float size_thresh, uint8_t* clone_mask,
                      uint8_t* split_mask, uint8_t* prune_mask, uint32_t* counts, void* stream);

size_t hgs_compact_scratch_bytes(int32_t P);
int hgs_compact_index(int32_t P, const uint8_t* keep, int32_t* src_of_dst, uint32_t* num_kept, void* scratch,
                      void* stream);
int hgs_gather_rows(int64_t n_out, int32_t row_floats, const int32_t* src_of_dst, const float* src, float* dst,
                    void* stream);

int hgs_reanchor(int32_t P, const float* vertices, const int32_t* faces, const int32_t* mapping_face,
                 const float* mapping_uvw, const float* mapping_dist, float* xyz, void* stream);

#define HGS_ADAM_MAX_TENSORS 16
typedef struct hgs_adam_tensor {
  float* param;
  const float* grad;
  float* exp_avg;
  float* exp_avg_sq;
  int64_t rows;
  int32_t row_floats;
  float step_size, bc2_sqrt, w1, beta2, w2, eps;
} hgs_adam_tensor;
typedef struct hgs_adam_args {
  int32_t num_tensors;
  int64_t visible_rows;
  const uint8_t* visible;
  hgs_adam_tensor t[HGS_ADAM_MAX_TENSORS];
  uint32_t block_start[HGS_ADAM_MAX_TENSORS + 1];
} hgs_adam_args;
int hgs_adam_step(const hgs_adam_args* args, void* stream);

#define HGS_LBS_MAX_JOINTS 64
#define HGS_LBS_FRAME_TILE 8
typedef struct hgs_lbs_args {
  int32_t V, J, F, K;
  int32_t weight_width;
  int32_t posedirs_stride;
  const float* v_shaped;
  const float* J_rest;
  const int32_t* parents;
  const float* posedirs;
  const int32_t* weight_joint;
  const float* weight_value;
  const float* poses;
  const float* transl;
  float centre[3];
  float scale;
  void* workspace;
  float* vertices;
  float* joints;
} hgs_lbs_args;
size_t hgs_lbs_workspace_bytes(int32_t J, int32_t F);
int hgs_lbs_pose(const hgs_lbs_args* args, void* stream);

#define HGS_POSE_OPENPOSE 0
#define HGS_POSE_HUMANSD 1
#define HGS_POSE_MAX_LIMBS 17
#define HGS_POSE_MAX_COLOURS 18
#define HGS_POSE_RECORD_INTS 8
#define HGS_POSE_MAX_DIM 4096
typedef struct hgs_pose_args {
  int32_t style;
  int32_t B, K, H, W;
  int32_t limb_width;
  int32_t uint8_out;
  int32_t num_limbs;
  const float* points;
  const float* mvp;
  const uint8_t* occlusion;
  void* image;
  float* kp;
  int32_t* records;
  int32_t limb[HGS_POSE_MAX_LIMBS][3];
// ... 91 lines not shown
```

Before: 661.2 million.

## Add entry-indexed pair table and gather-based backward reduction for single view

Adds an opt-in row-gather mode, used for single-view, SH-degree-0 inputs. The sort writes entry pairs indexed by entry id, and a new preprocess-backward kernel gathers each Gaussian's per-pair gradient rows directly through LDS windows. This replaces the separate pair-reduce kernel and its intermediate rows buffer. It adds LDS staging, block scans and extra barriers, and it runs only when the caller sets the new HGS_ROW_GATHER flag.

```diff
diff --git a/humangaussian_amd/csrc/api.hip b/humangaussian_amd/csrc/api.hip
--- a/humangaussian_amd/csrc/api.hip
+++ b/humangaussian_amd/csrc/api.hip
@@ -148,10 +148,12 @@
   return L;
 }
 
-View make_view(const hgs_settings* s, int B, int P, int M, int64_t cap, int max_tile_hint = 0, int act = 0) {
+View make_view(const hgs_settings* s, int B, int P, int M, int64_t cap, bool has_shs, bool row_gather, int max_tile_hint = 0, int act = 0) {
   View v;
   v.act = act;
   v.pairchunks = B >= HGS_CHUNK_ROWS_MIN_VIEWS ? 1 : 0;
+  v.enttab = (row_gather && B == 1 && (!has_shs || s->sh_degree == 0)) ? 1 : 0;
+  v.pair_cap = 0;
   for (int b = 0; b < HGS_MAX_VIEWS; ++b) {
     const hgs_settings& sb = s[b < B ? b : 0];
     Cam& c = v.cam[b];
@@ -463,7 +465,7 @@
                                int32_t store_bwd_state, int32_t max_tile_entries_hint, hgs_status* status_host,
                                int32_t status_host_mapped, void* status_event, void* const* stage_events,
                                int32_t activation_flags, float* means2D_leaf, void* stream_) {
-  if (activation_flags & ~(7 | HGS_GRAD_SCALE_TRUE_DERIVATIVE | HGS_ANTIALIAS)) return HGS_EINVAL;
+  if (activation_flags & ~(7 | HGS_GRAD_SCALE_TRUE_DERIVATIVE | HGS_ANTIALIAS | HGS_ROW_GATHER)) return HGS_EINVAL;
   if (!batch_ok(s, B) || P < 0 || !out_color || !out_depth || !out_alpha || !geom || !img ||
       entry_capacity < 0)
     return HGS_EINVAL;
@@ -482,8 +484,8 @@
   DeviceState* const ds = device_state(stream);
   const int ncu = cu_count(ds);
   const bool aa = (activation_flags & HGS_ANTIALIAS) != 0;
-  const View v = make_view(s, B, P, M, entry_capacity, max_tile_entries_hint > 0 ? max_tile_entries_hint : 0,
-                           activation_flags & 7);
+  const View v = make_view(s, B, P, M, entry_capacity, shs != nullptr, (activation_flags & HGS_ROW_GATHER) != 0,
+                           max_tile_entries_hint > 0 ? max_tile_entries_hint : 0, activation_flags & 7);
   const Layout L = make_layout(geom, bin, img, B, P, v.H, v.W, entry_capacity);
   hgs_status* status_dev =
       reinterpret_cast<hgs_status*>(static_cast<char*>(geom) + carve_geom(B, P, v.H, v.W).status);
@@ -566,8 +568,8 @@
         if (e != hipSuccess) return hip_rc(e);
       }
       const unsigned sort_wgs = std::min<unsigned>(class_grid(1), (unsigned)(hgs_knob("HGS_SORT_WGS_PER_CU", 3) * ncu));
-      hipLaunchKernelGGL(v.pairchunks ? hgs_k_sort_lds_ch : hgs_k_sort_lds, dim3(sort_wgs), dim3(HGS_SORT_NT), 0, stream, v, L,
-                         status_dev);
+      hipLaunchKernelGGL(v.pairchunks ? hgs_k_sort_lds_ch : (v.enttab ? hgs_k_sort_lds_et : hgs_k_sort_lds), dim3(sort_wgs),
+                         dim3(HGS_SORT_NT), 0, stream, v, L, status_dev);
       HGS_LAUNCH_CHECK();
       if (side) {
         e = hipStreamWaitEvent(stream, side->join, 0);
@@ -635,7 +637,7 @@
                            float* dL_drotations, float* dL_dcov3D_precomp, void* const* stage_events,
                            int32_t activation_flags, float* pack, int32_t pack_F, void* stream_) {
   (void)radii;
-  if (activation_flags & ~(7 | HGS_GRAD_SCALE_TRUE_DERIVATIVE | HGS_ANTIALIAS)) return HGS_EINVAL;
+  if (activation_flags & ~(7 | HGS_GRAD_SCALE_TRUE_DERIVATIVE | HGS_ANTIALIAS | HGS_ROW_GATHER)) return HGS_EINVAL;
   if ((activation_flags & (HGS_ACT_OPACITY_SIGMOID | HGS_ANTIALIAS)) && P > 0 && !opacities) return HGS_EINVAL;
   if (!batch_ok(s, B) || P < 0 || !geom || !img || entry_capacity < 0 || entry_capacity > HGS_MAX_ENTRY_CAPACITY) return HGS_EINVAL;
   if (status && status->overflow) return HGS_EINVAL;
@@ -651,7 +653,7 @@
   hipStream_t stream = static_cast<hipStream_t>(stream_);
   DeviceState* const ds = device_state(stream);
   const int64_t cap = entry_capacity;
-  const View v = make_view(s, B, P, M, cap, 0, activation_flags);
+  View v = make_view(s, B, P, M, cap, shs != nullptr, (activation_flags & HGS_ROW_GATHER) != 0, 0, activation_flags & ~HGS_ROW_GATHER);
   const Layout L = make_layout(const_cast<void*>(geom), const_cast<void*>(bin),
                                const_cast<void*>(img), B, P, v.H, v.W, cap);
   const hgs_status* status_dev = reinterpret_cast<const hgs_status*>(
@@ -662,6 +664,7 @@
   const uint32_t pair_cap = (uint32_t)(pc > 0xffffffffll ? 0xffffffffll : pc);
   float* rows = static_cast<float*>(bwd_scratch);
   float* pair_rows = rows + (size_t)X * HGS_ROW_FLOATS;
+  v.pair_cap = pair_cap;
   HGS_STAGE(0);
   if (maybe_entries) {
     const int resident = hgs_knob("HGS_BWD_WAVES_PER_CU", 12) * cu_count(ds);
@@ -669,7 +672,7 @@
                        out_color, out_depth, out_alpha, dL_dout_color, dL_dout_depth, dL_dout_alpha, pair_rows, pair_cap);
     HGS_LAUNCH_CHECK();
     HGS_STAGE(1);
-    if (X > 0) {
+    if (X > 0 && !v.enttab) {
       const uint32_t R_host = status ? status->num_rendered : 0xffffffffu;
       hipLaunchKernelGGL(v.pairchunks ? hgs_k_pair_reduce_ch : hgs_k_pair_reduce_em, dim3((unsigned)((X + 255) / 256)), dim3(256), 0,
                          stream, v, L, status_dev, L.recs, pair_rows, rows, pair_cap, R_host);
@@ -686,11 +689,12 @@
   const int row_p = hgs_pre_bwd_row(aa, 2, deg);
   const bool vpar_ok = v.B >= HGS_PRE_BWD_VPAR_MIN_VIEWS && thr_p <= (unsigned)hgs_pre_bwd_forms.row[row_p].threads &&
                        (lds_p <= 65536 || pre_bwd_lds_raised(ds, row_p));
-  const int mode = v.B == 1 ? 1 : (vpar_ok ? 2 : 0);
+  const int mode = v.enttab ? 3 : (v.B == 1 ? 1 : (vpar_ok ? 2 : 0));
   const PreBwdForm& form = hgs_pre_bwd_forms.row[hgs_pre_bwd_row(aa, mode, deg)];
-  const unsigned grid = mode == 2 ? (unsigned)((v.P + 63) / 64) : (unsigned)v.nblk, threads = mode == 2 ? thr_p : HGS_BLOCK;
+  const unsigned grid = mode >= 2 ? (unsigned)((v.P + 63) / 64) : (unsigned)v.nblk;
+  const unsigned threads = mode == 2 ? thr_p : (mode == 3 ? (unsigned)form.threads : HGS_BLOCK);
   const size_t lds = mode == 2 ? lds_p : (mode == 1 ? hgs_pre_bwd_stage_bytes(M, deg, shs != nullptr && dL_dshs != nullptr) : 0);
-  hipLaunchKernelGGL(form.kernel, dim3(grid), dim3(threads), lds, stream, v, L, status_dev, rows, means3D, shs,
+  hipLaunchKernelGGL(form.kernel, dim3(grid), dim3(threads), lds, stream, v, L, status_dev, mode == 3 ? pair_rows : rows, means3D, shs,
                      colors_precomp, opacities, scales, rotations, cov3D_precomp, dL_dmeans3D, dL_dmeans2D,
                      dL_dshs, dL_dcolors_precomp, dL_dopacities, dL_dscales, dL_drotations,
                      dL_dcov3D_precomp, pack, (int)pack_F);
diff --git a/humangaussian_amd/csrc/binning.hip b/humangaussian_amd/csrc/binning.hip
--- a/humangaussian_amd/csrc/binning.hip
+++ b/humangaussian_amd/csrc/binning.hip
@@ -98,6 +98,7 @@
     st.reserved[1] = L.ctr->max_n;
     st.reserved[2] = 1;
     *status = st;
+    L.ctr->enttab = v.enttab ? 1u : 0u;
     if (status_host) {
       volatile uint32_t* hs = reinterpret_cast<volatile uint32_t*>(status_host);
       const uint32_t* sw = reinterpret_cast<const uint32_t*>(&st);
@@ -205,7 +206,7 @@
 
 namespace {
 
-#define HGS_EMIT_RECORD(MASK, G0, G1, G2, OFFSET, CHUNK_BASE, K, TAGGED, CHUNK_ROWS)                                     \
+#define HGS_EMIT_RECORD(MASK, ENTRY, G0, G1, G2, OFFSET, CHUNK_BASE, K, TAGGED, CHUNK_ROWS, ET)                          \
   {                                                                                                                      \
     const uint4 g0 = (G0), g1 = (G1), g2 = (G2);                                                                         \
     const int minx = g2.z & 0xffffu, miny = g2.z >> 16, maxx = g2.w & 0xffffu;                                           \
@@ -218,7 +219,8 @@
     dst[0] = make_uint4(g0.x, g0.y, __float_as_uint(qa), __float_as_uint(qb));                                           \
     dst[1] = make_uint4(__float_as_uint(qc), g1.y, g1.z, g1.w);                                                          \
     dst[2] = make_uint4(g2.x, g2.y, entry, (TAGGED) ? hgs_rec_tag(MASK, (K), n, (CHUNK_ROWS)) : 0u);                     \
-    L.entpair[start + (K)].x = hgs_entpair_x(entry, (uint32_t)__popc(MASK));                                             \
+    L.entpair[(ET) ? entry : start + (K)].x = hgs_entpair_x(entry, (uint32_t)__popc(MASK));                              \
+    ENTRY = entry;                                                                                                       \
   }
 
 struct CellAlloc {
@@ -351,10 +353,10 @@
 #pragma unroll
     for (int u = 0; u < GU; ++u) {
       const uint32_t k = kb + (uint32_t)u * nt;
-      uint32_t mask = 0;
+      uint32_t mask = 0, eid = 0;
       if (k < n) {
-        HGS_EMIT_RECORD(mask, q0[u], q1[u], q2[u], q3[u], cbase[idxv[u] >> 8], k, v.pairchunks, false)
-        sorted[k] = (unsigned long long)mask;
+        HGS_EMIT_RECORD(mask, eid, q0[u], q1[u], q2[u], q3[u], cbase[idxv[u] >> 8], k, v.pairchunks, false, v.enttab != 0)
+        sorted[k] = hgs_mask_slot(mask, eid);
       }
 #pragma unroll
       for (int c = 0; c < 16; ++c) {
@@ -372,7 +374,7 @@
     const uint32_t nch = min((uint32_t)MAXCH, (n - sc0 + 63u) / 64u);
     for (uint32_t ch = wv; ch < nch; ch += nwaves) {
       const uint32_t k = sc0 + ch * 64u + lane;
-      const uint32_t mask = (k < n) ? (uint32_t)sorted[k] : 0u;
+      const uint32_t mask = (k < n) ? hgs_mask_slot_mask(sorted[k]) : 0u;
       uint32_t mine = 0;
 #pragma unroll
       for (int c = 0; c < 16; ++c) {
@@ -403,10 +405,11 @@
     for (uint32_t ch = wv; ch < nch; ch += nwaves) {
       const uint32_t k = sc0 + ch * 64u + lane;
       const bool in = k < n;
-      const uint32_t mask = in ? (uint32_t)sorted[k] : 0u;
+      const unsigned long long slot_k = in ? sorted[k] : 0ull;
+      const uint32_t mask = hgs_mask_slot_mask(slot_k);
       const uint32_t cnt = (uint32_t)__popc(mask);
       const uint32_t rel = S.tab[ch][16] + hgs_wave_incl_scan(cnt) - cnt;
-      if (in) L.entpair[start + k].y = pair_base + rel;
+      if (in) L.entpair[v.enttab ? hgs_mask_slot_entry(slot_k) : start + k].y = pair_base + rel;
 #pragma unroll
       for (int c = 0; c < 16; ++c) {
         const bool bit = (mask >> c) & 1u;
@@ -468,10 +471,10 @@
     for (int u = 0; u < GU; ++u) {
       const uint32_t k = kb + (uint32_t)u * nt;
       if (kb0 + (uint32_t)u * nt + (uint32_t)(wv * 64) >= n) continue;
-      uint32_t mask = 0;
+      uint32_t mask = 0, eid = 0;
       if (k < n) {
-        HGS_EMIT_RECORD(mask, q0[u], q1[u], q2[u], q3[u], cbase[idxv[u] >> 8], k, v.pairchunks, false)
-        sorted[k] = (unsigned long long)mask;
+        HGS_EMIT_RECORD(mask, eid, q0[u], q1[u], q2[u], q3[u], cbase[idxv[u] >> 8], k, v.pairchunks, false, v.enttab != 0)
+        sorted[k] = hgs_mask_slot(mask, eid);
       }
       const uint32_t ch = k >> 6;
       uint32_t tot[4];
@@ -527,7 +530,8 @@
   for (uint32_t ch = wv; ch < nch; ch += nwaves) {
     const uint32_t k = ch * 64u + lane;
     const bool in = k < n;
-    uint32_t mask = in ? (uint32_t)sorted[k] : 0u;
+    const unsigned long long slot_k = in ? sorted[k] : 0ull;
+    uint32_t mask = hgs_mask_slot_mask(slot_k);
     uint32_t ex[4], before = 0;
 #pragma unroll
     for (int wd = 0; wd < 4; ++wd) {
@@ -536,7 +540,7 @@
       before += hgs_bytesum(ex[wd]);
     }
     const uint32_t rel = S.tab[ch][16] + before;
-    if (in) L.entpair[start + k].y = pair_base + rel;
+    if (in) L.entpair[v.enttab ? hgs_mask_slot_entry(slot_k) : start + k].y = pair_base + rel;
     uint32_t r = 0;
     while (mask) {
       const int c = __builtin_ctz(mask);
@@ -669,9 +673,9 @@
   }
 }
 
-template <int NT, bool CH>
+template <int NT, bool CH, bool ET>
 __device__ __forceinline__ void cell_lists_from_masks(const View& v, const Layout& L, uint32_t order_pos, uint32_t start, uint32_t n,
-                                                      const uint16_t* __restrict__ masks, GatherLds<64>& S, const CellAlloc& ca,
+                                                      uint16_t* __restrict__ masks, GatherLds<64>& S, const CellAlloc& ca,
                                                       unsigned long long* tp) {
   const int tid = (int)threadIdx.x, lane = tid & 63, wv = tid >> 6;
   constexpr int nwaves = NT / 64;
@@ -735,7 +739,7 @@
     }
     const uint32_t rel_chunk = pair_base + S.tab[ch][16];
     const uint32_t rel = rel_chunk + before;
-    if (in) L.entpair[start + k].y = CH ? rel_chunk : rel;
+    if (!ET && in) L.entpair[start + k].y = CH ? rel_chunk : rel;
     const uint32_t cb = lane < 16 ? S.cell_base[lane] + S.tab[ch][lane] : 0u;
     uint32_t cp = 0;
 #pragma unroll
@@ -748,8 +752,10 @@
       }
       if (CH) cp += (tot[c >> 2] >> (8 * (c & 3))) & 0xffu;
     }
-  }
-}
+    if (ET && in) masks[k] = (uint16_t)(rel - pair_base);
+  }
+}
+static_assert(HGS_PAIRS_PER_ENTRY * (HGS_SORT_LDS_MAX - 1) < 65536, "an entry's first pair row, relative to its tile's, fits the mask's 16 bits");
 
 template <int E, int NT>
 __device__ __forceinline__ bool rank_keys(const Layout& L, uint32_t start, uint32_t n, uint32_t NB, const u64 (&keyp)[HGS_RANK_GU],
@@ -959,7 +965,7 @@
   return degenerate;
 }
 
-template <int NT, bool CH>
+template <int NT, bool CH, bool ET>
 __device__ __forceinline__ void rank_sort_tile(const View& v, const Layout& L, uint32_t order_pos, int g, uint32_t start, uint32_t n,
                                                unsigned long long* pairs, RankLds& R, GatherLds<64>& S, bool& degenerate_out,
                                                unsigned long long* tp) {
@@ -1016,13 +1022,14 @@
     const uint32_t k__ = ((r) * (uint32_t)GU + (uint32_t)u) * NT + (uint32_t)tid;             \
     HGS_RANK_ISSUE(X, u, (k__ < n) ? pairs[k__] : ~0ull);                                     \
   }
-#define HGS_RANK_CONSUME(X)                                                                   \
+#define HGS_RANK_CONSUME(X, r)      \
   _Pragma("unroll") for (int u = 0; u < GU; ++u) {                                            \
     if (X##pr[u] != ~0ull) {                                                                  \
       const uint32_t k = (uint32_t)(X##pr[u] >> 32);                                          \
-      uint32_t mask;                                                                          \
-      HGS_EMIT_RECORD(mask, X##a[u], X##b[u], X##c[u], X##off[u], X##cb[u], k, CH, true)    \
+      uint32_t mask, eid;                                                                     \
+      HGS_EMIT_RECORD(mask, eid, X##a[u], X##b[u], X##c[u], X##off[u], X##cb[u], k, CH, true, ET)    \
       masks[k] = (uint16_t)mask;                                                              \
+      if (ET) pairs[((r) * (uint32_t)GU + (uint32_t)u) * NT + (uint32_t)tid] = hgs_rank_slot(eid, k); \
       _Pragma("unroll") for (int wd = 0; wd < 4; ++wd) acc[wd] += hgs_spread4((mask >> (4 * wd)) & 0xfu); \
     }                                                                                         \
   }
@@ -1039,10 +1046,10 @@
   for (uint32_t r = 0; r * per_round < n; r += 2u) {
     const bool hb = (r + 1u) * per_round < n, ha = (r + 2u) * per_round < n;
     if (hb) { HGS_RANK_ROUND(B, r + 1u) }
-    HGS_RANK_CONSUME(A)
+    HGS_RANK_CONSUME(A, r)
     if (r < 4u) HGS_TQ(4 + r)
     if (ha) { HGS_RANK_ROUND(A, r + 2u) }
-    if (hb) { HGS_RANK_CONSUME(B) }
+    if (hb) { HGS_RANK_CONSUME(B, r + 1u) }
     if (r < 3u) HGS_TQ(5 + r)
   }
 #undef HGS_RANK_ISSUE
@@ -1069,10 +1076,18 @@
     const uint32_t word = R.tot16[2 * (c >> 2) + (c & 1)];
     hgs_alloc_cell_ranges_issue(L, order_pos, (word >> (16 * ((c >> 1) & 1))) & 0xffffu, ca);
   }
-  cell_lists_from_masks<NT, CH>(v, L, order_pos, start, n, masks, S, ca, tp);
-}
-
-template <int NT, bool CH>
+  cell_lists_from_masks<NT, CH, ET>(v, L, order_pos, start, n, masks, S, ca, tp);
+  if (ET) {
+    lds_barrier();
+    const uint32_t pair_base = S.pair_base;
+    for (uint32_t k = tid; k < n; k += NT) {
+      const u64 sl = pairs[k];
+      L.entpair[hgs_rank_slot_entry(sl)].y = pair_base + (uint32_t)masks[hgs_rank_slot_rank(sl)];
+    }
+  }
+}
+
+template <int NT, bool CH, bool ET>
 __device__ __forceinline__ void sort_rank_body(const View& v, const Layout& L, const hgs_status* __restrict__ status,
                                                unsigned long long* pairs, RankLds& R, GatherLds<64>& S) {
   if (status->overflow) return;
@@ -1097,7 +1112,7 @@
 #endif
     bool degenerate;
     unsigned long long tp[4] = {0, 0, 0, 0};
-    rank_sort_tile<NT, CH>(v, L, b, g, start, n, pairs, R, S, degenerate, tp);
+    rank_sort_tile<NT, CH, ET>(v, L, b, g, start, n, pairs, R, S, degenerate, tp);
 #ifdef HGS_TIMELINE
     if (threadIdx.x == 0 && b < HGS_TL_SLOTS) {
       const unsigned long long tpe = wall_clock64();
@@ -1119,18 +1134,19 @@
 }
 
 static_assert(16 * HGS_SORT_NT >= 4096, "the rank sort takes every list of the LDS class");
-#define HGS_SORT_LDS_KERNEL(NAME, CH)                                                                                  \
+#define HGS_SORT_LDS_KERNEL(NAME, CH, ET)                                                                                \
   extern "C" __global__ void __launch_bounds__(HGS_SORT_NT) __attribute__((amdgpu_waves_per_eu(HGS_SORT_WAVES_PER_EU, HGS_SORT_WAVES_PER_EU))) \
   NAME(View v, Layout L, const hgs_status* __restrict__ status) {                                                      \
     __shared__ unsigned long long pairs[4096];                                                                         \
     __shared__ GatherLds<64> S;                                                                                        \
     __shared__ RankLds R;                                                                                              \
     HGS_TL_BEGIN();                                                                                                    \
-    sort_rank_body<HGS_SORT_NT, CH>(v, L, status, pairs, R, S);                                                        \
+    sort_rank_body<HGS_SORT_NT, CH, ET>(v, L, status, pairs, R, S);                                                       \
     HGS_TL_END(3, 0u);                                                                                                 \
   }
-HGS_SORT_LDS_KERNEL(hgs_k_sort_lds, false)
-HGS_SORT_LDS_KERNEL(hgs_k_sort_lds_ch, true)
+HGS_SORT_LDS_KERNEL(hgs_k_sort_lds, false, false)
+HGS_SORT_LDS_KERNEL(hgs_k_sort_lds_ch, true, false)
+HGS_SORT_LDS_KERNEL(hgs_k_sort_lds_et, false, true)
 
 extern "C" __global__ void __launch_bounds__(1024)
 hgs_k_sort_large(View v, Layout L, const hgs_status* __restrict__ status) {
diff --git a/humangaussian_amd/csrc/entryrec.h b/humangaussian_amd/csrc/entryrec.h
--- a/humangaussian_amd/csrc/entryrec.h
+++ b/humangaussian_amd/csrc/entryrec.h
@@ -52,6 +52,24 @@
 HGS_HD uint32_t hgs_entpair_entry(uint32_t x) { return x & HGS_ENTRY_MASK; }
 HGS_HD uint32_t hgs_entpair_pairs(uint32_t x) { return x >> HGS_ENTRY_BITS; }
 
+#define HGS_SLOT_ENTRY_SHIFT 16
+static_assert(HGS_SLOT_ENTRY_SHIFT >= HGS_TAG_MASK_BITS && HGS_SLOT_ENTRY_SHIFT + HGS_ENTRY_BITS <= 64, "mask and entry id share a 64-bit slot");
+HGS_HD uint64_t hgs_mask_slot(uint32_t mask, uint32_t entry) { return (uint64_t)(mask & 0xffffu) | ((uint64_t)entry << HGS_SLOT_ENTRY_SHIFT); }
+HGS_HD uint32_t hgs_mask_slot_mask(uint64_t s) { return (uint32_t)s & 0xffffu; }
+HGS_HD uint32_t hgs_mask_slot_entry(uint64_t s) { return (uint32_t)(s >> HGS_SLOT_ENTRY_SHIFT) & HGS_ENTRY_MASK; }
+HGS_HD uint64_t hgs_rank_slot(uint32_t entry, uint32_t rank) { return (uint64_t)entry | ((uint64_t)rank << 32); }
+HGS_HD uint32_t hgs_rank_slot_entry(uint64_t s) { return (uint32_t)s; }
+HGS_HD uint32_t hgs_rank_slot_rank(uint64_t s) { return (uint32_t)(s >> 32); }
+
+#define HGS_GATHER_WINDOW 128u
+#define HGS_GATHER_ROWS 352u
+HGS_HD void hgs_window_span(uint32_t first, uint32_t count, uint32_t w0, uint32_t wn, uint32_t& lo, uint32_t& hi) {
+  lo = first > w0 ? first : w0;
+  const uint32_t e1 = first + count, e2 = w0 + wn;
+  hi = e1 < e2 ? e1 : e2;
+  if (count == 0u) hi = lo;
+}
+
 #define HGS_CELL_KEY_BITS 4
 static_assert(HGS_CELLS_PER_TILE == 1 << HGS_CELL_KEY_BITS, "the cell index is the key's low bits");
 HGS_HD uint32_t hgs_cell_key(uint32_t g, uint32_t c) { return g * (uint32_t)HGS_CELLS_PER_TILE + c; }
diff --git a/humangaussian_amd/csrc/hgs_common.h b/humangaussian_amd/csrc/hgs_common.h
--- a/humangaussian_amd/csrc/hgs_common.h
+++ b/humangaussian_amd/csrc/hgs_common.h
@@ -57,6 +57,7 @@
   unsigned long long alloc_eb;
   __attribute__((aligned(128))) uint32_t entry_alloc;
   __attribute__((aligned(128))) uint32_t max_n;
+  uint32_t enttab;
   CounterLine cls_hist[HGS_NCLS];
   CounterLine cls_cur[HGS_NCLS];
   __attribute__((aligned(128))) unsigned long long alloc_ps;
@@ -119,6 +120,8 @@
   int32_t max_tile_hint;
   int32_t act;
   int32_t pairchunks;
+  int32_t enttab;
+  uint32_t pair_cap;
 };
 
 static inline size_t hgs_align_up(size_t v, size_t a) { return (v + a - 1) / a * a; }
diff --git a/humangaussian_amd/csrc/preprocess.hip b/humangaussian_amd/csrc/preprocess.hip
--- a/humangaussian_amd/csrc/preprocess.hip
+++ b/humangaussian_amd/csrc/preprocess.hip
@@ -436,6 +436,7 @@
   constexpr int NC = (DEG + 1) * (DEG + 1);
   constexpr bool SINGLE = MODE != 0;
   constexpr bool VPAR = MODE == 2;
+  constexpr bool GATHER = MODE == 3;
   constexpr int NV = 23 + 3 * NC;
   extern __shared__ float red[];
   int i = blockIdx.x * HGS_BLOCK + threadIdx.x, bview = 0, il = threadIdx.x;
@@ -444,6 +445,12 @@
     bview = __builtin_amdgcn_readfirstlane((int)threadIdx.x >> 6);
     i = blockIdx.x * 64 + il;
   }
+  int gwave = 0;
+  if (GATHER) {
+    il = (int)threadIdx.x & 63;
+    gwave = __builtin_amdgcn_readfirstlane((int)threadIdx.x >> 6);
+    i = blockIdx.x * 64 + il;
+  }
   const bool mine = (i < v.P) && (bview < v.B);
   const bool staged = MODE == 1 && DEG > 0 && dL_dshs != nullptr && shs != nullptr && hgs_sh_staged(v.M) &&
                       (int)(blockIdx.x + 1) * HGS_BLOCK <= v.P && pack == nullptr;
@@ -451,7 +458,7 @@
     stage_sh_chunk(shs, v.M, (int)blockIdx.x * HGS_BLOCK, HGS_BLOCK, red);
     __syncthreads();
   }
-  if (!VPAR && !mine) return;
+  if (!VPAR && !GATHER && !mine) return;
   if (!mine) i = 0;
   if (bview >= v.B) bview = 0;
   const bool ok = status->overflow == 0;
@@ -486,7 +493,92 @@
       }
     }
   };
-  if (SINGLE) load_inputs();
+  if (SINGLE && gwave == 0) load_inputs();
+
+  float gs0 = 0.f, gs1 = 0.f, gs2 = 0.f, gs3 = 0.f, gs4 = 0.f, gs5 = 0.f, gs6 = 0.f, gs7 = 0.f, gs8 = 0.f, gs9 = 0.f;
+  if constexpr (GATHER) {
+    constexpr uint32_t GT = 128;
+    constexpr uint32_t GW = HGS_GATHER_WINDOW;
+    constexpr uint32_t RC = HGS_GATHER_ROWS;
+    constexpr int NL = (int)((RC * HGS_PROW_F2 + GT - 1) / GT);
+    static_assert(GW == GT, "a window is one table slot per thread");
+    __shared__ uint2 s_ent[GW];
+    __shared__ __attribute__((aligned(8))) float s_esum[GW * HGS_PROW_FLOATS];
+    __shared__ uint32_t s_rowmap[RC];
+    __shared__ float2 s_rows[RC * HGS_PROW_F2];
+    __shared__ uint32_t s_wtot[GT / 64];
+    const uint32_t tid = threadIdx.x;
+    const uint4 gq2 = reinterpret_cast<const uint4*>(&L.geom[i])[2], gq3 = reinterpret_cast<const uint4*>(&L.geom[i])[3];
+    const uint32_t rect_n = ((gq2.w & 0xffffu) - (gq2.z & 0xffffu)) * ((gq2.w >> 16) - (gq2.z >> 16));
+    const uint32_t tt_me = (mine && ok && (int)gq3.y > 0) ? rect_n : 0u;
+    const uint32_t e_me = L.chunk_base[i >> 8] + gq3.x;
+    const uint32_t e_lo = ~hgs_wave_max_u32(tt_me ? ~e_me : 0u), e_hi = hgs_wave_max_u32(tt_me ? e_me + tt_me : 0u);
+    const uint32_t E = e_hi > e_lo ? e_hi - e_lo : 0u;
+    const uint32_t first_me = tt_me ? e_me - e_lo : 0u;
+    const bool poisoned = (uint32_t)L.ctr->alloc_ps > v.pair_cap || L.ctr->enttab != 1u;
+    const float2* __restrict__ prow = reinterpret_cast<const float2*>(grad_rows);
+    if (poisoned) {
+      if (tt_me) gs0 = gs1 = gs2 = gs3 = gs4 = gs5 = gs6 = gs7 = gs8 = gs9 = __builtin_nanf("");
+    } else {
+      for (uint32_t w0 = 0; w0 < E; w0 += GW) {
+        const uint32_t wn = min(GW, E - w0);
+        uint2 ep = make_uint2(0u, 0u);
+        if (tid < wn) ep = L.entpair[e_lo + w0 + tid];
+        const uint32_t cnt = min(hgs_entpair_pairs(ep.x), (uint32_t)HGS_PAIRS_PER_ENTRY);
+        uint32_t RT;
+        const uint32_t rb = hgs_block_excl_scan<(int)GT>(cnt, s_wtot, RT);
+        s_ent[tid] = make_uint2(rb, cnt);
+#pragma unroll
+        for (int k = 0; k < HGS_PROW_FLOATS; ++k) s_esum[tid + GT * k] = 0.f;
+        for (uint32_t c0 = 0; c0 < RT; c0 += RC) {
+          const uint32_t nrow = min(RC, RT - c0), npiece = nrow * HGS_PROW_F2;
+          {
+            const uint32_t lo = max(rb, c0), hi = min(rb + cnt, c0 + nrow);
+            for (uint32_t j = lo; j < hi; ++j) s_rowmap[j - c0] = ep.y + (j - rb);
+          }
+          __syncthreads();
+          float2 pc[NL];
+#pragma unroll
+          for (int q = 0; q < NL; ++q) {
+            const uint32_t s = tid + GT * (uint32_t)q, sc = s < npiece ? s : 0u;
+            const uint32_t row = sc / HGS_PROW_F2;
+            pc[q] = prow[(size_t)s_rowmap[row] * HGS_PROW_F2 + (sc - row * HGS_PROW_F2)];
+          }
+#pragma unroll
+          for (int q = 0; q < NL; ++q) {
+            const uint32_t s = tid + GT * (uint32_t)q;
+            if (s < npiece) s_rows[s] = pc[q];
+          }
+          __syncthreads();
+          const float* __restrict__ rf = reinterpret_cast<const float*>(s_rows);
+          for (uint32_t item = tid; item < wn * HGS_PROW_FLOATS; item += GT) {
+            const uint32_t e = item / HGS_PROW_FLOATS, c = item - e * HGS_PROW_FLOATS;
+            const uint2 en = s_ent[e];
+            const uint32_t lo = max(en.x, c0), hi = min(en.x + en.y, c0 + nrow);
+            if (hi > lo) {
+              float sum = s_esum[item];
+              const float* q = rf + (lo - c0) * HGS_PROW_FLOATS + c;
+#pragma unroll 4
+              for (uint32_t j = lo; j < hi; ++j, q += HGS_PROW_FLOATS) sum += *q;
+              s_esum[item] = sum;
+            }
+          }
+          __syncthreads();
+        }
+        if (RT == 0u) __syncthreads();
+        if (gwave == 0) {
+          uint32_t lo, hi;
+          hgs_window_span(first_me, tt_me, w0, wn, lo, hi);
+          for (uint32_t e = lo; e < hi; ++e) {
+            const float2* q = reinterpret_cast<const float2*>(s_esum + (e - w0) * HGS_PROW_FLOATS);
+            const float2 a0 = q[0], a1 = q[1], a2 = q[2], a3 = q[3], a4 = q[4];
+            gs0 += a0.x; gs1 += a0.y; gs2 += a1.x; gs3 += a1.y; gs4 += a2.x; gs5 += a2.y; gs6 += a3.x; gs7 += a3.y; gs8 += a4.x; gs9 += a4.y;
+          }
+        }
+      }
+    }
+    if (gwave != 0 || !mine) return;
+  }
 
   float a_mean[3] = {0.f, 0.f, 0.f}, a_sc[3] = {0.f, 0.f, 0.f}, a_rot[4] = {0.f, 0.f, 0.f, 0.f};
   float a_cov[6] = {0.f, 0.f, 0.f, 0.f, 0.f, 0.f}, a_col[3] = {0.f, 0.f, 0.f}, a_op = 0.f;
@@ -512,6 +604,9 @@
       const int rw = (int)(g.rect_hi & 0xffffu) - (int)(g.rect_lo & 0xffffu);
       const int rh = (int)(g.rect_hi >> 16) - (int)(g.rect_lo >> 16);
       const int tt = rw * rh;
+      if constexpr (GATHER) {
+        gmx = gs0; gmy = gs1; gA = gs2; gB = gs3; gC = gs4; gop = gs5; gr = gs6; gg = gs7; gb = gs8; gdep = gs9;
+      } else {
       const float4* rows = reinterpret_cast<const float4*>(grad_rows) +
                            HGS_GROW_F4 * (size_t)(L.chunk_base[(size_t)b * v.nblk + (i >> 8)] + g.offset);
 #define HGS_ROWS_UNROLL_MANY 4
@@ -531,6 +626,7 @@
             gb += r2[u].x; gdep += r2[u].y;
           }
         }
+      }
       }
       if (!aa) a_op += gop;
       a_col[0] += gr; a_col[1] += gg; a_col[2] += gb;
@@ -887,6 +983,8 @@
   X(1, 1, 0, hgs_k_preprocess_bwd_s1, HGS_BLOCK)                                                                          \
   X(2, 1, 0, hgs_k_preprocess_bwd_s2, HGS_BLOCK)                                                                          \
   X(3, 1, 0, hgs_k_preprocess_bwd_s3, HGS_BLOCK)                                                                          \
+  X(0, 3, 0, hgs_k_preprocess_bwd_g0, 128)             \
+  X(0, 3, 1, hgs_k_preprocess_bwd_g0_aa, 128)                                                                             \
   X(0, 2, 0, hgs_k_preprocess_bwd_p0, 1024)                \
   X(1, 2, 0, hgs_k_preprocess_bwd_p1, 1024)                 \
   X(2, 2, 0, hgs_k_preprocess_bwd_p2, 512)                                                                                \
@@ -926,8 +1024,8 @@
                               const float*, const float*, const float*, const float*, float*, float*, float*, float*,
                               float*, float*, float*, float*, float*, int);
 struct PreBwdForm { PreBwdKernel kernel; const char* name; int threads; };
-constexpr int HGS_PRE_BWD_ROWS = 24;
-constexpr int hgs_pre_bwd_row(int aa, int mode, int deg) { return deg + 4 * mode + 12 * aa; }
+constexpr int HGS_PRE_BWD_ROWS = 32;
+constexpr int hgs_pre_bwd_row(int aa, int mode, int deg) { return deg + 4 * mode + 16 * aa; }
 struct PreBwdForms { PreBwdForm row[HGS_PRE_BWD_ROWS]; };
 __host__ constexpr PreBwdForms hgs_make_pre_bwd_forms() {
   PreBwdForms t{};
@@ -940,8 +1038,10 @@
 }
 constexpr PreBwdForms hgs_pre_bwd_forms = hgs_make_pre_bwd_forms();
 __host__ constexpr bool hgs_pre_bwd_forms_complete() {
-  for (int r = 0; r < HGS_PRE_BWD_ROWS; ++r)
-    if (hgs_pre_bwd_forms.row[r].kernel == nullptr) return false;
+  for (int aa = 0; aa < 2; ++aa)
+    for (int mode = 0; mode < 4; ++mode)
+      for (int deg = 0; deg < (mode == 3 ? 1 : 4); ++deg)
+        if (hgs_pre_bwd_forms.row[hgs_pre_bwd_row(aa, mode, deg)].kernel == nullptr) return false;
   return true;
 }
 static_assert(hgs_pre_bwd_forms_complete(), "a (filter, mode, degree) combination without a kernel");
diff --git a/include/hgs_rast.h b/include/hgs_rast.h
--- a/include/hgs_rast.h
+++ b/include/hgs_rast.h
@@ -89,6 +89,7 @@
 #define HGS_ACT_ROTATION_NORMALIZE 4
 #define HGS_GRAD_SCALE_TRUE_DERIVATIVE 8
 #define HGS_ANTIALIAS 16
+#define HGS_ROW_GATHER 64
 int hgs_forward_batch_act(const hgs_settings* views, int32_t B, int32_t P, int32_t M,
                           const float* means3D, const float* shs, const float* colors_precomp,
                           const float* opacities, const float* scales, const float* rotations,
```

Result: slower. 649.5 million (-1.8%).
